# INK-USC/RE-Net

Measured on AMD Instinct MI355X. Metric: RGCN+GRU encoder triples/s at bs=1024 n_hidden=200 (full training step, both directions), higher is better.
Workload: dtype f32; 1 GPU; ICEWS18-shaped synthetic stream (seed 999), n_hidden=200, seq_len=10, batch=1024 per GPU, dropout=0.50, fwd+bwd both directions + clip + Adam; parallelism=dp1, global_batch=1024, nodes=99312, edges=288792

## Files before the change

include/renet_hip.h:

```cpp
#ifndef RENET_HIP_H
#define RENET_HIP_H

#include <stddef.h>
#include <stdint.h>

#ifdef __cplusplus
extern "C" {
#endif

#define RENET_OK 0
#define RENET_ERR_BADARG (-1)
#define RENET_ERR_UNSUPPORTED (-2)
#define RENET_ERR_WORKSPACE (-3)

#define RENET_ABI_VERSION 1
int renet_version(void);

int renet_gather_rows(const float* table, const int32_t* idx, int n, int D, float* out, void* stream);
int renet_segment_add(const float* src, const int32_t* order, const int32_t* seg_ptr,
                      const int32_t* seg_target, int U, int D, float* dst, void* stream);
int renet_segment_add2(const float* src0, const float* src1, const int32_t* order, const int32_t* seg_ptr,
                       const int32_t* seg_target, int U, int D, float* dst0, float* dst1, void* stream);

int renet_rgcn_gather(const float* x, int D, const int32_t* row_ptr, const int32_t* col,
                      const int32_t* etype, const float* scale, const float* W, int T, int type_shift,
                      int transpose_w, const float* addend, float drop_p, uint64_t seed, int relu,
                      float* out, int N, const int32_t* heavy_rows, int n_heavy, int heavy_thresh,
                      int src_limit, int addend_rows, void* stream);

int renet_rgcn_gather_items(const float* x, int D, const int32_t* it_src, const int32_t* it_type,
                            const int32_t* grp_ptr, int n_groups, const int32_t* row_ptr, const int32_t* col,
                            const int32_t* etype, const float* scale, const float* W, int T, int type_shift,
                            int transpose_w, const float* addend, float drop_p, uint64_t seed, int relu,
                            float* out, int N, const int32_t* heavy_rows, int n_heavy, int src_limit,
                            int addend_rows, int pruned, void* stream);

int renet_rgcn_gather_items_table(const float* table, int table_rows, int D, const int32_t* it_src_t,
                                  const int32_t* it_type_t, const int32_t* grp_ptr, int n_groups,
                                  const int32_t* row_ptr, const int32_t* col_t, const int32_t* etype,
                                  const int32_t* row_map, const float* scale, const float* W, int T, int type_shift,
                                  const float* addend_table, float drop_p, uint64_t seed, int relu, float* out, int N,
                                  const int32_t* heavy_rows, int n_heavy, void* stream);

int renet_rgcn_gather_items_bf16(const float* x, int D, const int32_t* it_src, const int32_t* it_type,
                                 const int32_t* grp_ptr, int n_groups, const int32_t* row_ptr, const int32_t* col,
                                 const int32_t* etype, const float* scale, const void* W_bf16, int w_ld, int T,
                                 int type_shift, int transpose_w, const float* addend, float drop_p, uint64_t seed,
                                 int relu, float* out, int N, const int32_t* heavy_rows, int n_heavy, int src_limit,
                                 int addend_rows, int pruned, void* stream);
int renet_rgcn_gather_items_table_bf16(const void* table_bf16, int table_ld, int table_rows, int D,
                                       const int32_t* it_src_t, const int32_t* it_type_t, const int32_t* grp_ptr,
                                       int n_groups, const int32_t* row_ptr, const int32_t* col_t, const int32_t* etype,
                                       const int32_t* row_map, const float* scale, const void* W_bf16, int w_ld, int T,
                                       int type_shift, const float* addend_table, float drop_p, uint64_t seed, int relu,
                                       float* out, int N, const int32_t* heavy_rows, int n_heavy, void* stream);
int renet_compose_table_items(const int32_t* row_map, const int32_t* it_src, const int32_t* it_type, int n_items,
                              const int32_t* col, const int32_t* e_src, int E, int32_t* it_src_t,
                              int32_t* it_type_t, int32_t* col_t, int32_t* e_src_t, void* stream);

int renet_rgcn_bwd_prep(const float* g_out, const float* out, const float* norm, int relu,
                        float drop_p, uint64_t seed, int N, int D, float* gn, float* g_loop,
                        void* stream);
int renet_rgcn_bwd_prep_bounds(const float* g_out, const float* out, const float* norm, int relu,
                               float drop_p, uint64_t seed, int N, int D, float* gn, float* g_loop,
                               float* bound_part, void* stream);

size_t renet_rgcn_bwd_w_workspace(int n_chunks, int D);
int renet_rgcn_bwd_w(const float* x, const float* gn, const int32_t* e_src, const int32_t* e_dst,
                     const int32_t* chunk_ptr, const int32_t* chunk_type, int n_chunks,
                     const int32_t* type_chunk_ptr, int T, int type_shift, int D, float* dW, float beta,
                     float* workspace, size_t workspace_bytes, void* stream);
int renet_rgcn_bwd_w64(const float* x, const float* gn, const int32_t* e_src, const int32_t* e_dst,
                       const int32_t* chunk_ptr, const int32_t* chunk_type, int n_chunks,
                       const int32_t* type_chunk_ptr, int T, int type_shift, int D, float* dW, float beta,
                       float* workspace, size_t workspace_bytes, void* stream);

size_t renet_gemm_workspace(int M, int N, int split_k);
int renet_gemm_f32(int ta, int tb, int M, int N, int K, float alpha, const float* A, int lda,
                   const float* B, int ldb, float beta, float* C, int ldc, const float* bias,
                   int split_k, float* workspace, size_t workspace_bytes, void* stream);

int renet_gemm_f32_split(int ta, int tb, int M, int N, int K, float alpha, const float* A, int lda,
                         const float* B, int ldb, float beta, float* C, int ldc, const float* bias,
                         int split_k, float* workspace, size_t workspace_bytes, void* stream);

int renet_gemm_split_plan(int ta, int tb, int M, int N, int K, const float* A, int lda, const float* B, int ldb,
                          int split_k, int* plan);

int renet_maxabs_blocks(int rows, int cols, int ld);
int renet_maxabs_partials(const float* x, int rows, int cols, int ld, float* part, void* stream);
int renet_maxabs_partials_multi(const void* jobs, int n_jobs, void* stream);
int renet_gemm_f32_h3(int ta, int tb, int M, int N, int K, float alpha, const float* A, int lda, const float* B,
                      int ldb, float beta, float* C, int ldc, const float* bias, int split_k, float* workspace,
                      size_t workspace_bytes, const float* maxA, int nA, const float* maxB, int nB, void* stream);

int renet_gemm_bf16(int ta, int tb, int M, int N, int K, float alpha, const float* A, int lda,
                    const float* B, int ldb, float beta, float* C, int ldc, const float* bias,
                    int split_k, float* workspace, size_t workspace_bytes, void* stream);

size_t renet_bf16_bytes(int R, int C);
int renet_pack_bf16(const float* X, int R, int C, int ldx, void* out, void* stream);
int renet_gemm_bf16s(int a_tr, int b_tr, int M, int N, int K, float alpha, const void* Ap, int lda, const void* Bp,
                     int ldb, float beta, float* C, int ldc, const float* bias, int split_k, float* workspace,
                     size_t workspace_bytes, void* stream);
int renet_bf16_zero_padding(void* P, int rows, int C, int ld, int rows_alloc, void* stream);
int renet_seq_assemble_fwd_bf16(const float* h2, const float* ent, const float* rel, const float* glob,
                                const int32_t* subj_row, const int32_t* row_ent, const int32_t* row_rel,
                                const int32_t* glob_row, int S, int D, float drop_p, uint64_t seed_x,
                                uint64_t seed_xr, void* X, int ldx, void* Xr, int ldxr, int rows_alloc,
                                void* stream);
int renet_softmax_ce_bf16(const float* logits, const int32_t* target, int B, int C, int ld, float grad_scale,
                          float* row_loss, void* dlogits_bf16, int ld16, int rows16, void* stream);
int renet_gru_bwd_layouts_bf16out(int n, const float* const* dh_last, const int32_t* const* step_off, const int* L,
                                  int H, const float* const* Whh, const float* const* saved, void* const* dGi16,
                                  void* const* dGh16, int out_ld, float* workspace, size_t workspace_bytes,
                                  void* stream);
int renet_colsum_bf16(const void* X, int M, int N, int ldx, float* out, float beta, float* workspace,
                      size_t workspace_bytes, void* stream);
int renet_scale_bf16_by_device_scalar(void* x, size_t n, const float* scale, void* stream);

size_t renet_planes_elems(int R, int C);
int renet_pack_planes(const float* X, int R, int C, int ldx, int ones_col, void* out, void* stream);
int renet_gemm_planes(int a_tr, int b_tr, int M, int N, int K, float alpha, const float* alpha_dev, const void* Ap,
                      int lda, size_t a_plane, const void* Bp, int ldb, size_t b_plane, float beta, float* C, int ldc,
                      const float* bias, float* col_out, int split_k, float* workspace, size_t workspace_bytes,
                      void* stream);
int renet_softmax_ce_planes(const float* logits, const int32_t* target, int B, int C, int ld, float grad_scale,
                            float* row_loss, void* dl_planes, size_t plane, int ld16, int rows16, void* stream);

size_t renet_colsum_workspace(int M, int N);
int renet_colsum(const float* X, int M, int N, int ldx, float* out, float beta, float* workspace,
                 size_t workspace_bytes, void* stream);

int renet_scale_by_device_scalar(float* x, size_t n, const float* scale, void* stream);
int renet_scale_by_device_scalar_bound(float* x, size_t n, const float* scale, float bound_in, float* bound_out,
                                       void* stream);

int renet_seq_assemble_fwd(const float* h2, const float* ent, const float* rel, const float* glob,
                           const int32_t* subj_row, const int32_t* row_ent, const int32_t* row_rel,
                           const int32_t* glob_row, int S, int D, float drop_p, uint64_t seed_x,
                           uint64_t seed_xr, float* X, float* Xr, void* stream);
int renet_bound_parts(size_t total4);
int renet_seq_assemble_fwd_bounds(const float* h2, const float* ent, const float* rel, const float* glob,
                                  const int32_t* subj_row, const int32_t* row_ent, const int32_t* row_rel,
                                  const int32_t* glob_row, int S, int D, float drop_p, uint64_t seed_x,
                                  uint64_t seed_xr, float* X, float* Xr, float* partX, float* partXr, void* stream);
int renet_seq_assemble_bwd(const float* dX, const float* dXr, const int32_t* step_off, int L, int S,
                           int B, int D, float drop_p, uint64_t seed_x, uint64_t seed_xr, float* dRows,
                           float* dEntSeq, float* dRelSeq, void* stream);

size_t renet_gru_workspace(int B, int H);
int renet_gru_fwd(const float* Gi, const int32_t* step_off, int L, int H, const float* Whh,
                  const float* bhh, float* h_last, int out_rows, float* saved, float* workspace,
                  size_t workspace_bytes, void* stream);
int renet_gru_bwd(const float* dh_last, const int32_t* step_off, int L, int H, const float* Whh,
                  const float* saved, float* dGi, float* dGh, float* workspace,
                  size_t workspace_bytes, void* stream);
int renet_gru_fwd_multi(int n, const float* const* Gi, const int32_t* step_off, int L, int H,
                        const float* const* Whh, const float* const* bhh, float* const* h_last, int out_rows,
                        float* const* saved, float* workspace, size_t workspace_bytes, void* stream);
int renet_gru_bwd_multi(int n, const float* const* dh_last, const int32_t* step_off, int L, int H,
                        const float* const* Whh, const float* const* saved, float* const* dGi,
                        float* const* dGh, float* workspace, size_t workspace_bytes, void* stream);
int renet_gru_fwd_layouts(int n, const float* const* Gi, const int32_t* const* step_off, const int* L, int H,
                          const float* const* Whh, const float* const* bhh, float* const* h_last,
                          const int* out_rows, float* const* saved, float* workspace, size_t workspace_bytes,
                          void* stream);
int renet_gru_bwd_layouts(int n, const float* const* dh_last, const int32_t* const* step_off, const int* L, int H,
                          const float* const* Whh, const float* const* saved, float* const* dGi,
                          float* const* dGh, float* workspace, size_t workspace_bytes, void* stream);
int renet_gru_bound_parts(int max_rows);
int renet_gru_bwd_layouts_bounds(int n, const float* const* dh_last, const int32_t* const* step_off, const int* L, int H,
                                 const float* const* Whh, const float* const* saved, float* const* dGi,
                                 float* const* dGh, float* const* bounds, float* workspace, size_t workspace_bytes,
                                 void* stream);
int renet_gru_fwd_layouts_f32(int n, const float* const* Gi, const int32_t* const* step_off, const int* L, int H,
                              const float* const* Whh, const float* const* bhh, float* const* h_last,
                              const int* out_rows, float* const* saved, float* workspace, size_t workspace_bytes,
                              void* stream);
int renet_gru_bwd_layouts_f32(int n, const float* const* dh_last, const int32_t* const* step_off, const int* L, int H,
                              const float* const* Whh, const float* const* saved, float* const* dGi,
                              float* const* dGh, float* workspace, size_t workspace_bytes, void* stream);
int renet_gru_fwd_layouts_bf16(int n, const float* const* Gi, const int32_t* const* step_off, const int* L, int H,
                               const float* const* Whh, const float* const* bhh, float* const* h_last,
                               const int* out_rows, float* const* saved, float* workspace, size_t workspace_bytes,
                               void* stream);
int renet_gru_bwd_layouts_bf16(int n, const float* const* dh_last, const int32_t* const* step_off, const int* L, int H,
                               const float* const* Whh, const float* const* saved, float* const* dGi,
                               float* const* dGh, float* workspace, size_t workspace_bytes, void* stream);

int renet_concat3_fwd(const float* a, const int32_t* ia, const float* hmid, const float* c,
                      const int32_t* ic, int B, int D, float drop_p, uint64_t seed, float* feat,
                      void* stream);
int renet_concat3_fwd_bounds(const float* a, const int32_t* ia, const float* hmid, const float* c,
                             const int32_t* ic, int B, int D, float drop_p, uint64_t seed, float* feat,
                             float* bound_part, void* stream);
int renet_concat3_bwd(const float* dfeat, int B, int D, int parts, float drop_p, uint64_t seed,
                      float* da_rows, float* dhmid, float* dc_rows, void* stream);
int renet_dropout(const float* x, size_t n, float drop_p, uint64_t seed, float* y, void* stream);
int renet_softmax_ce(const float* logits, const int32_t* target, int B, int C, int ld,
                     float grad_scale, float* row_loss, float* dlogits, void* stream);

int renet_segment_pool_fwd(const float* h, const int32_t* seg_ptr, int G, int D, int is_max,
                           float* out, int32_t* argmax, void* stream);
int renet_segment_pool_bwd(const float* dout, const int32_t* seg_ptr, const int32_t* argmax, int G,
                           int D, int is_max, int N, float* dh, void* stream);

size_t renet_adam_workspace(size_t n);
int renet_adam_step(float* p, float* g, float* m, float* v, size_t n, float lr, float beta1, float beta2,
                    float eps, float weight_decay, float max_norm, int step, int zero_grad, float* workspace,
                    size_t workspace_bytes, float* grad_norm_out, void* stream);
int renet_adam_step_scaled(float* p, float* g, float* m, float* v, size_t n, float lr, float beta1, float beta2,
                           float eps, float weight_decay, float max_norm, float grad_scale, int step,
                           int zero_grad, float* workspace, size_t workspace_bytes, float* grad_norm_out,
                           void* stream);

int renet_sumsq_partials(const float* g, size_t n, float* partial, int n_slots, void* stream);
int renet_adam_step_presummed(float* p, float* g, float* m, float* v, size_t n, float lr, float beta1, float beta2,
                              float eps, float weight_decay, float max_norm, float grad_scale, int step, int zero_grad,
                              const float* partial, int n_partial, float* grad_norm_out, void* stream);

int renet_joint_softmax(float* logits, int ld, int n, int R, int N, const float* logits_r, int ld_r,
                        const float* prob_e, void* stream);
size_t renet_topk_workspace(int n);
int renet_topk_positive(const float* x, size_t ldx, int n, int M, int k, float* out_val, int64_t* out_idx,
                        void* workspace, size_t workspace_bytes, void* stream);

typedef struct {
    const int32_t *q_s, *q_r, *q_o;
    const int32_t* h_first[2];
    const int32_t* h_count[2];
    const int32_t* snap_t[2];
    const int32_t* snap_ptr[2];
    const int32_t* nbr_o[2];
    const int32_t* times;
    const int32_t* trip_ptr;
    const int32_t *trip_s, *trip_r, *trip_o;
    const int32_t* glob_times;
    int T, n_glob, n_facts, num_ent, num_rels;
} RenetStoreDev;

typedef struct {
    int32_t *node_ent, *node_slot, *row_ptr, *col, *etype;
    float* norm;
    int32_t *heavy_rows, *e_src, *e_dst, *chunk_ptr, *chunk_type, *type_chunk_ptr;
    int32_t *e_src2, *e_dst2, *chunk_ptr2, *chunk_type2, *type_chunk_ptr2;
    int32_t *it_src, *it_type, *grp_ptr;
    int32_t *subj_row, *row_seq, *row_ent, *row_rel, *glob_row;
    int32_t *s_sorted, *r_sorted, *rel_label, *ent_label, *perm, *step_off;
    int32_t* plan_order[4];
    int32_t* plan_seg[4];
    int32_t* plan_target[4];
    int32_t* counts;
    int cap_nodes, cap_edges;
    int32_t* seg_ptr;
} RenetBatchOut;

enum {
    RENET_BB_NNZ = 0, RENET_BB_S, RENET_BB_L, RENET_BB_TB, RENET_BB_FACTS, RENET_BB_N, RENET_BB_NA, RENET_BB_E2,
    RENET_BB_E, RENET_BB_NHEAVY, RENET_BB_NHEAVY_OUT, RENET_BB_NCHUNKS, RENET_BB_NCHUNKS2, RENET_BB_NITEMS,
    RENET_BB_NGROUPS, RENET_BB_NGROUPS_OUT, RENET_BB_NSEG0, RENET_BB_NSEG1, RENET_BB_NSEG2, RENET_BB_NSEG3,
    RENET_BB_ERR, RENET_BB_EOUT,
    RENET_BB_STEP_OFF = 24,
    RENET_BB_NCOUNTS = 64
};
enum { RENET_BB_ERR_TIME = 1, RENET_BB_ERR_GLOB = 2, RENET_BB_ERR_NODES = 4, RENET_BB_ERR_EDGES = 8 };

size_t renet_build_batch_workspace(const RenetStoreDev* store, int B, int cap_nodes, int cap_edges);
int renet_build_batch_both(const RenetStoreDev* store, const int32_t* idx_dev, int B, int seq_len, int heavy_thresh,
                           int group_budget, int chunk, const RenetBatchOut* out, void* workspace,
                           size_t workspace_bytes, void* stream);

typedef struct {
    const int32_t* node_ptr;
    const int32_t* node_ent_all;
    const int32_t* trip_ptr;
    const int32_t *trip_ls, *trip_r, *trip_lo;
    int T, n_nodes, n_facts, num_ent, num_rels;
} RenetFullStoreDev;

size_t renet_build_full_graphs_workspace(const RenetFullStoreDev* store, int G, int cap_nodes, int cap_edges);
int renet_build_full_graphs(const RenetFullStoreDev* store, const int32_t* tidx_dev, int G, int heavy_thresh,
                            int group_items, int chunk, RenetBatchOut* out, void* workspace, size_t workspace_bytes,
                            void* stream);

typedef struct { const int32_t *order, *seg_ptr, *target; int num_segments; } RenetSegPlan;
typedef struct {
    int D, num_ent, T, C2;
    float drop_p;
    const float *ent, *rel;
    const float *w1, *loop1, *w2, *loop2;
    const float *wih, *whh, *bih, *bhh;
    const float *wih_r, *whh_r, *bih_r, *bhh_r;
    const float *lin_w, *lin_b;
    const float *linr_w, *linr_b;
    float *g_ent, *g_rel, *g_w1, *g_loop1, *g_w2, *g_loop2, *g_wih, *g_whh, *g_bih, *g_bhh, *g_wih_r, *g_whh_r, *g_bih_r,
          *g_bhh_r, *g_lin_w, *g_lin_b, *g_linr_w, *g_linr_b;
    const float* glob;
    const void* lin_w_planes;
    size_t lin_w_plane;
    int lin_w_ld;
} RenetStepModel;
// ... 62 lines not shown
```

re-net_amd/csrc/rgcn.hip:

```cpp
#include "common.h"
#include <stdlib.h>

namespace {

constexpr int kWaves = 4;
constexpr int kThreads = 64 * kWaves;

template <int SI, bool TR>
__device__ __forceinline__ void blockmul(const float4 x, const float4* __restrict__ w, float4& acc) {
    if constexpr (SI == 1) {
        const float4 w0 = w[0];
        acc.x = fmaf(x.x, w0.x, acc.x);
        acc.y = fmaf(x.y, w0.y, acc.y);
        acc.z = fmaf(x.z, w0.z, acc.z);
        acc.w = fmaf(x.w, w0.w, acc.w);
    } else if constexpr (SI == 2) {
        const float4 a = w[0], b = w[1];
        if constexpr (!TR) {
            acc.x = fmaf(x.x, a.x, fmaf(x.y, a.z, acc.x));
            acc.y = fmaf(x.x, a.y, fmaf(x.y, a.w, acc.y));
            acc.z = fmaf(x.z, b.x, fmaf(x.w, b.z, acc.z));
            acc.w = fmaf(x.z, b.y, fmaf(x.w, b.w, acc.w));
        } else {
            acc.x = fmaf(x.x, a.x, fmaf(x.y, a.y, acc.x));
// ... 611 lines not shown
#pragma unroll
    for (int q = 0; q < NCH; ++q) off[q] = (uint32_t)(lane + 64 * q) < (uint32_t)CH ? (uint32_t)(lane + 64 * q) * 16u : kOob;
    float4 acc[NCH][SI];
#pragma unroll
    for (int q = 0; q < NCH; ++q)
#pragma unroll
        for (int i = 0; i < SI; ++i) acc[q][i] = make_float4(0.f, 0.f, 0.f, 0.f);

    for (int eb = e0; eb < e1; eb += 64) {
        const int my_e = eb + lane;
        int my_s = 0, my_d = 0;
        if (my_e < e1) { my_s = e_src[my_e]; my_d = e_dst[my_e]; }
        asm volatile("" : "+v"(my_s), "+v"(my_d));
        const int cnt = min(64, e1 - eb);
        for (int k0 = 0; k0 < cnt; k0 += UNR) {
            float4 xv[UNR][NCH], gv[UNR][NCH];
#pragma unroll
            for (int u = 0; u < UNR; ++u) {
                const int kk = min(k0 + u, 63);
                const bool ok = (k0 + u) < cnt;
                const uint32_t so = ok ? (uint32_t)__builtin_amdgcn_readlane(my_s, kk) * ROWB : 0u;
                const uint32_t dof = ok ? (uint32_t)__builtin_amdgcn_readlane(my_d, kk) * ROWB : 0u;
#pragma unroll
                for (int q = 0; q < NCH; ++q) {
                    if constexpr (BIG) {
                        const int ch = lane + 64 * q;
                        const bool on = ok && ch < CH;
                        const size_t sr = (size_t)__builtin_amdgcn_readlane(my_s, kk) * CH + ch;
                        const size_t dr = (size_t)__builtin_amdgcn_readlane(my_d, kk) * CH + ch;
                        const float4 z = make_float4(0.f, 0.f, 0.f, 0.f);
                        xv[u][q] = on ? reinterpret_cast<const float4*>(x)[sr] : z;
                        gv[u][q] = on ? reinterpret_cast<const float4*>(gmat)[dr] : z;
                    } else {
                        xv[u][q] = buf_load4s(rx, ok ? off[q] : kOob, so);
                        gv[u][q] = buf_load4s(rg, ok ? off[q] : kOob, dof);
                    }
                }
            }
#pragma unroll
            for (int u = 0; u < UNR; ++u) {
#pragma unroll
                for (int q = 0; q < NCH; ++q) {
                    if constexpr (SI == 1) {
                        acc[q][0].x = fmaf(xv[u][q].x, gv[u][q].x, acc[q][0].x);
                        acc[q][0].y = fmaf(xv[u][q].y, gv[u][q].y, acc[q][0].y);
                        acc[q][0].z = fmaf(xv[u][q].z, gv[u][q].z, acc[q][0].z);
                        acc[q][0].w = fmaf(xv[u][q].w, gv[u][q].w, acc[q][0].w);
                    } else if constexpr (SI == 2) {
                        acc[q][0].x = fmaf(xv[u][q].x, gv[u][q].x, acc[q][0].x);
                        acc[q][0].y = fmaf(xv[u][q].x, gv[u][q].y, acc[q][0].y);
                        acc[q][0].z = fmaf(xv[u][q].y, gv[u][q].x, acc[q][0].z);
                        acc[q][0].w = fmaf(xv[u][q].y, gv[u][q].y, acc[q][0].w);
                        acc[q][1].x = fmaf(xv[u][q].z, gv[u][q].z, acc[q][1].x);
                        acc[q][1].y = fmaf(xv[u][q].z, gv[u][q].w, acc[q][1].y);
                        acc[q][1].z = fmaf(xv[u][q].w, gv[u][q].z, acc[q][1].z);
                        acc[q][1].w = fmaf(xv[u][q].w, gv[u][q].w, acc[q][1].w);
                    } else {
                        const float xs[4] = {xv[u][q].x, xv[u][q].y, xv[u][q].z, xv[u][q].w};
#pragma unroll
                        for (int i = 0; i < 4; ++i) {
                            acc[q][i].x = fmaf(xs[i], gv[u][q].x, acc[q][i].x);
                            acc[q][i].y = fmaf(xs[i], gv[u][q].y, acc[q][i].y);
                            acc[q][i].z = fmaf(xs[i], gv[u][q].z, acc[q][i].z);
                            acc[q][i].w = fmaf(xs[i], gv[u][q].w, acc[q][i].w);
                        }
                    }
                }
            }
        }
    }
#pragma unroll
    for (int q = 0; q < NCH; ++q) {
        const int ch = lane + 64 * q;
        if (ch < CH) {
#pragma unroll
            for (int i = 0; i < SI; ++i) red[wave][ch * SI + i] = acc[q][i];
        }
    }
    __syncthreads();
    if (!live) return;
    const int ty = chunk_type[c];
    if (wave != 0 && chunk_type[c - 1] == ty) return;
    int run = 1;
    while (wave + run < kBwdWGroup && c + run < n_chunks && chunk_type[c + run] == ty) ++run;
#pragma unroll
    for (int q = 0; q < NCH; ++q) {
        const int ch = lane + 64 * q;
        if (ch < CH) {
#pragma unroll
            for (int i = 0; i < SI; ++i) {
                float4 r = red[wave][ch * SI + i];
                for (int w = 1; w < run; ++w) r = f4_add(r, red[wave + w][ch * SI + i]);
                partial[(size_t)c * WROW4 + ch * SI + i] = r;
            }
        }
    }
}

constexpr int kRedWaves = 16;
__global__ __launch_bounds__(kRedWaves * 64) void rgcn_bwd_w_reduce_kernel(
    const float4* __restrict__ partial, const int32_t* __restrict__ type_chunk_ptr, int WROW4,
    int T, int shift, float beta, float4* __restrict__ dW) {
    __shared__ float4 red[kRedWaves][64];
    const int t = blockIdx.x;
    const int lane = threadIdx.x & 63, wave = threadIdx.x >> 6;
    const int colq = blockIdx.y * 64 + lane;
    const int c0 = type_chunk_ptr[t], c1 = type_chunk_ptr[t + 1];
    float4 s = make_float4(0.f, 0.f, 0.f, 0.f);
    if (colq < WROW4 && c1 > c0) {
        if (wave == 0) s = partial[(size_t)c0 * WROW4 + colq];
        const int g0 = c0 / kBwdWGroup + 1;
        const int g1 = (c1 + kBwdWGroup - 1) / kBwdWGroup;
        float4 s1 = make_float4(0.f, 0.f, 0.f, 0.f), s2 = s1, s3 = s1;
        int gq = g0 + wave;
        for (; gq + 3 * kRedWaves < g1; gq += 4 * kRedWaves) {
            const float4 v0 = partial[(size_t)gq * kBwdWGroup * WROW4 + colq];
            const float4 v1 = partial[(size_t)(gq + kRedWaves) * kBwdWGroup * WROW4 + colq];
            const float4 v2 = partial[(size_t)(gq + 2 * kRedWaves) * kBwdWGroup * WROW4 + colq];
            const float4 v3 = partial[(size_t)(gq + 3 * kRedWaves) * kBwdWGroup * WROW4 + colq];
            s = f4_add(s, v0); s1 = f4_add(s1, v1); s2 = f4_add(s2, v2); s3 = f4_add(s3, v3);
        }
        for (; gq < g1; gq += kRedWaves) s = f4_add(s, partial[(size_t)gq * kBwdWGroup * WROW4 + colq]);
        s = f4_add(f4_add(s, s1), f4_add(s2, s3));
    }
    red[wave][lane] = s;
    __syncthreads();
    if (wave == 0 && colq < WROW4) {
        float4 r = red[0][lane];
#pragma unroll
        for (int w = 1; w < kRedWaves; ++w) r = f4_add(r, red[w][lane]);
        int to = t + shift;
        if (to >= T) to -= T;
        float4* o = dW + (size_t)to * WROW4 + colq;
        if (beta != 0.f) {
            const float4 p = *o;
            r = make_float4(r.x + beta * p.x, r.y + beta * p.y, r.z + beta * p.z, r.w + beta * p.w);
        }
        *o = r;
    }
}

__global__ __launch_bounds__(256) void gather_rows_kernel(const float4* __restrict__ table,
                                                          const int32_t* __restrict__ idx, int n, int CH,
                                                          float4* __restrict__ out) {
    const size_t total = (size_t)n * CH;
    for (size_t i = (size_t)blockIdx.x * blockDim.x + threadIdx.x; i < total;
         i += (size_t)gridDim.x * blockDim.x) {
        const int r = (int)(i / CH), c = (int)(i % CH);
        out[i] = table[(size_t)idx[r] * CH + c];
    }
}

constexpr int kSegWaves = 16, kSegShort = 16, kSegUnr = 8;
__global__ __launch_bounds__(kSegWaves * 64) void segment_add_kernel(const float4* __restrict__ src0,
                                                                     const float4* __restrict__ src1,
                                                                     const int32_t* __restrict__ order,
                                                                     const int32_t* __restrict__ seg_ptr,
                                                                     const int32_t* __restrict__ seg_target,
                                                                     int U, int CH, float4* __restrict__ dst0,
                                                                     float4* __restrict__ dst1) {
    const float4* __restrict__ src = blockIdx.y ? src1 : src0;
    float4* __restrict__ dst = blockIdx.y ? dst1 : dst0;
    __shared__ float4 red[kSegWaves][128];
    const int lane = threadIdx.x & 63;
    const int wave = __builtin_amdgcn_readfirstlane(threadIdx.x >> 6);
    const int nwg = gridDim.x;
    {
        const int u = blockIdx.x + wave * nwg;
        const int k0 = u < U ? seg_ptr[u] : 0, k1 = u < U ? seg_ptr[u + 1] : 0;
        const int len = k1 - k0;
        if (len > 0 && len <= kSegShort) {
            const size_t tgt = (size_t)seg_target[u] * CH;
            for (int ch = lane; ch < CH; ch += 64) {
                float4 s = make_float4(0.f, 0.f, 0.f, 0.f);
                for (int k = k0; k < k1; k += kSegUnr) {
                    float4 v[kSegUnr];
#pragma unroll
                    for (int j = 0; j < kSegUnr; ++j) v[j] = src[(size_t)order[min(k + j, k1 - 1)] * CH + ch];
#pragma unroll
                    for (int j = 0; j < kSegUnr; ++j)
                        if (k + j < k1) s = f4_add(s, v[j]);
                }
                dst[tgt + ch] = f4_add(dst[tgt + ch], s);
            }
        }
    }
    for (int j = 0; j < kSegWaves; ++j) {
        const int u = blockIdx.x + j * nwg;
        if (u >= U) break;
        const int k0 = seg_ptr[u], k1 = seg_ptr[u + 1];
        if (k1 - k0 <= kSegShort) continue;
        const size_t tgt = (size_t)seg_target[u] * CH;
        for (int ch = lane; ch < CH; ch += 64) {
            float4 s = make_float4(0.f, 0.f, 0.f, 0.f);
            for (int k = k0 + wave * kSegUnr; k < k1; k += kSegWaves * kSegUnr) {
                float4 v[kSegUnr];
#pragma unroll
                for (int q = 0; q < kSegUnr; ++q) v[q] = src[(size_t)order[min(k + q, k1 - 1)] * CH + ch];
#pragma unroll
                for (int q = 0; q < kSegUnr; ++q)
                    if (k + q < k1) s = f4_add(s, v[q]);
            }
            red[wave][ch] = s;
        }
        __syncthreads();
        if (wave == 0) {
            for (int ch = lane; ch < CH; ch += 64) {
                float4 r = red[0][ch];
#pragma unroll
                for (int w = 1; w < kSegWaves; ++w) r = f4_add(r, red[w][ch]);
                dst[tgt + ch] = f4_add(dst[tgt + ch], r);
            }
        }
        __syncthreads();
    }
}

__global__ __launch_bounds__(256) void compose_table_items_kernel(const int32_t* __restrict__ row_map,
                                                                  const int32_t* __restrict__ it_src,
                                                                  const int32_t* __restrict__ it_type, int n_items,
                                                                  const int32_t* __restrict__ col,
                                                                  const int32_t* __restrict__ e_src, int E,
                                                                  int32_t* __restrict__ it_src_t,
                                                                  int32_t* __restrict__ it_type_t,
                                                                  int32_t* __restrict__ col_t,
                                                                  int32_t* __restrict__ e_src_t) {
    const int total = n_items + 2 * E;
    for (int i = blockIdx.x * blockDim.x + threadIdx.x; i < total; i += gridDim.x * blockDim.x) {
        if (i < n_items) {
            const int s = it_src[i], t = it_type[i];
            if (t >= 0) { it_src_t[i] = row_map[s]; it_type_t[i] = t; }
            else if (t == -1) { it_src_t[i] = s; it_type_t[i] = -3 - row_map[s]; }
            else { it_src_t[i] = s; it_type_t[i] = t; }
        } else if (i < n_items + E) {
            col_t[i - n_items] = row_map[col[i - n_items]];
        } else {
            e_src_t[i - n_items - E] = row_map[e_src[i - n_items - E]];
        }
    }
}

}

extern "C" {

int renet_version(void) { return RENET_ABI_VERSION; }

int renet_gather_rows(const float* table, const int32_t* idx, int n, int D, float* out, void* stream) {
    if (n < 0 || D <= 0 || (D & 3)) return RENET_ERR_BADARG;
    if (n == 0) return RENET_OK;
    const int CH = D / 4;
    const size_t total = (size_t)n * CH;
    int blocks = (int)min((size_t)2048, (total + 255) / 256);
    RENET_LAUNCH(gather_rows_kernel, dim3(blocks), dim3(256), 0, (hipStream_t)stream,
                       (const float4*)table, idx, n, CH, (float4*)out);
    RENET_LAUNCH_CHECK();
    return RENET_OK;
}

static int seg_grid(int U) { return U <= 512 ? U : max(512, (U + kSegWaves - 1) / kSegWaves); }

int renet_segment_add(const float* src, const int32_t* order, const int32_t* seg_ptr,
                      const int32_t* seg_target, int U, int D, float* dst, void* stream) {
    if (U < 0 || D <= 0 || (D & 3)) return RENET_ERR_BADARG;
    if (U == 0) return RENET_OK;
    if (D > 512) return RENET_ERR_UNSUPPORTED;
    RENET_LAUNCH(segment_add_kernel, dim3(seg_grid(U)), dim3(kSegWaves * 64), 0,
                       (hipStream_t)stream, (const float4*)src, (const float4*)src, order, seg_ptr, seg_target, U, D / 4,
                       (float4*)dst, (float4*)dst);
    RENET_LAUNCH_CHECK();
    return RENET_OK;
}

int renet_segment_add2(const float* src0, const float* src1, const int32_t* order, const int32_t* seg_ptr,
                       const int32_t* seg_target, int U, int D, float* dst0, float* dst1, void* stream) {
    if (U < 0 || D <= 0 || (D & 3)) return RENET_ERR_BADARG;
    if (U == 0) return RENET_OK;
    if (D > 512) return RENET_ERR_UNSUPPORTED;
    RENET_LAUNCH(segment_add_kernel, dim3(seg_grid(U), 2), dim3(kSegWaves * 64), 0,
                       (hipStream_t)stream, (const float4*)src0, (const float4*)src1, order, seg_ptr, seg_target, U, D / 4,
                       (float4*)dst0, (float4*)dst1);
    RENET_LAUNCH_CHECK();
    return RENET_OK;
}

int renet_rgcn_gather(const float* x, int D, const int32_t* row_ptr, const int32_t* col,
                      const int32_t* etype, const float* scale, const float* W, int T, int type_shift,
                      int transpose_w, const float* addend, float drop_p, uint64_t seed, int relu,
                      float* out, int N, const int32_t* heavy_rows, int n_heavy, int heavy_thresh,
                      int src_limit, int addend_rows, void* stream) {
    if (!renet_dim_ok(D)) return RENET_ERR_UNSUPPORTED;
    if (n_heavy < 0 || (n_heavy > 0 && (!heavy_rows || heavy_thresh < 1))) return RENET_ERR_BADARG;
    if (N < 0 || T <= 0 || type_shift < 0 || type_shift >= T || drop_p < 0.f || drop_p >= 1.f)
        return RENET_ERR_BADARG;
    if (N == 0) return RENET_OK;
    GatherArgs a;
    a.x = x; a.row_ptr = row_ptr; a.col = col; a.etype = etype; a.scale = scale; a.W = W;
    a.addend = addend; a.out = out; a.N = N; a.T = T; a.shift = type_shift; a.relu = relu;
    a.heavy = heavy_rows; a.n_heavy = n_heavy;
    a.src_limit = src_limit > 0 ? src_limit : 0x7fffffff;
    a.addend_rows = addend_rows > 0 ? addend_rows : 0x7fffffff;
    a.heavy_thresh = n_heavy > 0 ? heavy_thresh : 0x7fffffff;
    a.drop = make_drop(drop_p, seed);
    hipStream_t st = (hipStream_t)stream;
    switch (D) {
        case 100: return launch_gather<1, 1, 4>(a, transpose_w != 0, st);
        case 200: return launch_gather<2, 1, 4>(a, transpose_w != 0, st);
        default: return launch_gather<4, 2, 2>(a, transpose_w != 0, st);
    }
}

static int gather_items_impl(int mx, int x_ld, int w_ld, const float* x, int x_rows, int D, const int32_t* it_src, const int32_t* it_type,
                             const int32_t* grp_ptr, int n_groups, const int32_t* row_ptr, const int32_t* col,
                             const int32_t* etype, const float* scale, const float* W, int T, int type_shift,
                             int transpose_w, const float* addend, float drop_p, uint64_t seed, int relu,
                             float* out, int N, const int32_t* heavy_rows, int n_heavy, int src_limit,
                             int addend_rows, int pruned, const int32_t* row_map, void* stream) {
    if (!renet_dim_ok(D)) return RENET_ERR_UNSUPPORTED;
    if (n_heavy < 0 || (n_heavy > 0 && !heavy_rows) || n_groups < 0) return RENET_ERR_BADARG;
    if (N < 0 || T <= 0 || type_shift < 0 || type_shift >= T || drop_p < 0.f || drop_p >= 1.f)
        return RENET_ERR_BADARG;
    if (N == 0 || (n_groups == 0 && n_heavy == 0)) return RENET_OK;
    if ((size_t)max(N, x_rows) * D * sizeof(float) >= ((size_t)1 << 31) ||
        (size_t)T * D * (D / 100) * sizeof(float) >= ((size_t)1 << 31))
        return RENET_ERR_UNSUPPORTED;
    ItemArgs a;
    a.g.x = x; a.g.row_ptr = row_ptr; a.g.col = col; a.g.etype = etype; a.g.scale = scale; a.g.W = W;
    a.g.addend = addend; a.g.out = out; a.g.N = N; a.g.T = T; a.g.shift = type_shift; a.g.relu = relu;
    a.g.heavy = heavy_rows; a.g.n_heavy = n_heavy; a.g.heavy_thresh = 0;
    a.g.src_limit = src_limit > 0 ? src_limit : 0x7fffffff;
    a.g.addend_rows = addend_rows > 0 ? addend_rows : 0x7fffffff;
    a.g.row_map = row_map;
    a.g.drop = make_drop(drop_p, seed);
    a.it_src = it_src; a.it_type = it_type; a.grp_ptr = grp_ptr; a.n_groups = n_groups;
    hipStream_t st = (hipStream_t)stream;
    const bool tr = transpose_w != 0, pr = pruned != 0;
    a.g.x_rowb = mx == 2 ? (uint32_t)x_ld * 2u : (uint32_t)D * 4u;
    a.g.w_rowb = mx >= 1 ? (uint32_t)w_ld * 2u : (uint32_t)D * (D / 100) * 4u;
    if (mx < 0 || mx > 2 || (mx >= 1 && w_ld < D * (D / 100)) || (mx == 2 && x_ld < D)) return RENET_ERR_BADARG;
    if (mx == 1) {
        switch (D) {
            case 100: return launch_gather_items<1, 1, 6, 1>(a, tr, pr, st);
            case 200: return launch_gather_items<2, 1, 3, 1>(a, tr, pr, st);
            default: return launch_gather_items<4, 2, 2, 1>(a, tr, pr, st);
        }
    }
    if (mx == 2) {
        switch (D) {
            case 100: return launch_gather_items<1, 1, 6, 2>(a, tr, pr, st);
            case 200: return launch_gather_items<2, 1, 3, 2>(a, tr, pr, st);
            default: return launch_gather_items<4, 2, 2, 2>(a, tr, pr, st);
        }
    }
    const int unr = gather_unr();
    switch (D) {
        case 100:
            if (unr == 8) return launch_gather_items<1, 1, 8>(a, tr, pr, st);
            if (unr == 4) return launch_gather_items<1, 1, 4>(a, tr, pr, st);
            return launch_gather_items<1, 1, 6>(a, tr, pr, st);
        case 200:
            if (unr == 2) return launch_gather_items<2, 1, 2>(a, tr, pr, st);
            if (unr == 4) return launch_gather_items<2, 1, 4>(a, tr, pr, st);
            if (unr == 6) return launch_gather_items<2, 1, 6>(a, tr, pr, st);
            if (unr == 8) return launch_gather_items<2, 1, 8>(a, tr, pr, st);
            return launch_gather_items<2, 1, 3>(a, tr, pr, st);
        default:
            if (unr == 3) return launch_gather_items<4, 2, 3>(a, tr, pr, st);
            if (unr == 4) return launch_gather_items<4, 2, 4>(a, tr, pr, st);
            return launch_gather_items<4, 2, 2>(a, tr, pr, st);
    }
}

int renet_rgcn_gather_items(const float* x, int D, const int32_t* it_src, const int32_t* it_type,
                            const int32_t* grp_ptr, int n_groups, const int32_t* row_ptr, const int32_t* col,
                            const int32_t* etype, const float* scale, const float* W, int T, int type_shift,
                            int transpose_w, const float* addend, float drop_p, uint64_t seed, int relu,
                            float* out, int N, const int32_t* heavy_rows, int n_heavy, int src_limit,
                            int addend_rows, int pruned, void* stream) {
    return gather_items_impl(0, 0, 0, x, N, D, it_src, it_type, grp_ptr, n_groups, row_ptr, col, etype, scale, W, T,
                             type_shift, transpose_w, addend, drop_p, seed, relu, out, N, heavy_rows, n_heavy, src_limit,
                             addend_rows, pruned, nullptr, stream);
}

int renet_rgcn_gather_items_bf16(const float* x, int D, const int32_t* it_src, const int32_t* it_type,
                                 const int32_t* grp_ptr, int n_groups, const int32_t* row_ptr, const int32_t* col,
                                 const int32_t* etype, const float* scale, const void* W_bf16, int w_ld, int T,
                                 int type_shift, int transpose_w, const float* addend, float drop_p, uint64_t seed,
                                 int relu, float* out, int N, const int32_t* heavy_rows, int n_heavy, int src_limit,
                                 int addend_rows, int pruned, void* stream) {
    return gather_items_impl(1, 0, w_ld, x, N, D, it_src, it_type, grp_ptr, n_groups, row_ptr, col, etype, scale,
                             (const float*)W_bf16, T, type_shift, transpose_w, addend, drop_p, seed, relu, out, N,
                             heavy_rows, n_heavy, src_limit, addend_rows, pruned, nullptr, stream);
}

int renet_rgcn_gather_items_table(const float* table, int table_rows, int D, const int32_t* it_src_t,
                                  const int32_t* it_type_t, const int32_t* grp_ptr, int n_groups,
                                  const int32_t* row_ptr, const int32_t* col_t, const int32_t* etype,
                                  const int32_t* row_map, const float* scale, const float* W, int T, int type_shift,
                                  const float* addend_table, float drop_p, uint64_t seed, int relu, float* out, int N,
                                  const int32_t* heavy_rows, int n_heavy, void* stream) {
    if (!row_map || table_rows <= 0) return RENET_ERR_BADARG;
    return gather_items_impl(0, 0, 0, table, table_rows, D, it_src_t, it_type_t, grp_ptr, n_groups, row_ptr, col_t, etype,
                             scale, W, T, type_shift, 0, addend_table, drop_p, seed, relu, out, N, heavy_rows, n_heavy, 0, 0,
                             0, row_map, stream);
}

int renet_rgcn_gather_items_table_bf16(const void* table_bf16, int table_ld, int table_rows, int D,
                                       const int32_t* it_src_t, const int32_t* it_type_t, const int32_t* grp_ptr,
                                       int n_groups, const int32_t* row_ptr, const int32_t* col_t, const int32_t* etype,
                                       const int32_t* row_map, const float* scale, const void* W_bf16, int w_ld, int T,
                                       int type_shift, const float* addend_table, float drop_p, uint64_t seed, int relu,
                                       float* out, int N, const int32_t* heavy_rows, int n_heavy, void* stream) {
    if (!row_map || table_rows <= 0) return RENET_ERR_BADARG;
    return gather_items_impl(2, table_ld, w_ld, (const float*)table_bf16, table_rows, D, it_src_t, it_type_t, grp_ptr,
                             n_groups, row_ptr, col_t, etype, scale, (const float*)W_bf16, T, type_shift, 0, addend_table,
                             drop_p, seed, relu, out, N, heavy_rows, n_heavy, 0, 0, 0, row_map, stream);
}

int renet_compose_table_items(const int32_t* row_map, const int32_t* it_src, const int32_t* it_type, int n_items,
                              const int32_t* col, const int32_t* e_src, int E, int32_t* it_src_t,
                              int32_t* it_type_t, int32_t* col_t, int32_t* e_src_t, void* stream) {
    if (n_items < 0 || E < 0 || !row_map) return RENET_ERR_BADARG;
    const int total = n_items + 2 * E;
    if (total == 0) return RENET_OK;
    RENET_LAUNCH(compose_table_items_kernel, dim3(min(2048, (total + 255) / 256)), dim3(256), 0, (hipStream_t)stream,
                 row_map, it_src, it_type, n_items, col, e_src, E, it_src_t, it_type_t, col_t, e_src_t);
    RENET_LAUNCH_CHECK();
    return RENET_OK;
}

static int bwd_prep_impl(const float* g_out, const float* out, const float* norm, int relu, float drop_p,
                         uint64_t seed, int N, int D, float* gn, float* g_loop, float* bound_part, void* stream) {
    if (N < 0 || D <= 0 || (D & 3) || drop_p < 0.f || drop_p >= 1.f) return RENET_ERR_BADARG;
    if (N == 0) return bound_part ? RENET_ERR_BADARG : RENET_OK;
// ... 88 lines not shown
```

re-net_amd/csrc/seq.hip:

```cpp
#include "common.h"

namespace {

__device__ __forceinline__ float sq_max4(float m, const float4& v) {
    return fmaxf(fmaxf(m, fmaxf(fabsf(v.x), fabsf(v.y))), fmaxf(fabsf(v.z), fabsf(v.w)));
}
__device__ __forceinline__ void sq_block_max_write(float m, float* __restrict__ part, float* red ) {
#pragma unroll
    for (int off = 32; off >= 1; off >>= 1) m = fmaxf(m, __shfl_xor(m, off));
    if ((threadIdx.x & 63) == 0) red[threadIdx.x >> 6] = m;
    __syncthreads();
    if (threadIdx.x == 0) part[blockIdx.x] = fmaxf(fmaxf(red[0], red[1]), fmaxf(red[2], red[3]));
    __syncthreads();
}

__global__ __launch_bounds__(256) void seq_assemble_fwd_kernel(
    const float4* __restrict__ h2, const float4* __restrict__ ent, const float4* __restrict__ rel,
    const float4* __restrict__ glob, const int32_t* __restrict__ subj_row,
    const int32_t* __restrict__ row_ent, const int32_t* __restrict__ row_rel,
    const int32_t* __restrict__ glob_row, int S, int CH, DropCfg dx, DropCfg dxr,
    float4* __restrict__ X, float4* __restrict__ Xr, float* __restrict__ partX, float* __restrict__ partXr) {
    __shared__ float red[4];
    float mx = 0.f, mxr = 0.f;
    const size_t total = (size_t)S * 4 * CH;
    for (size_t i = (size_t)blockIdx.x * blockDim.x + threadIdx.x; i < total;
         i += (size_t)gridDim.x * blockDim.x) {
        const int p = (int)(i / (4 * CH));
        const int c = (int)(i - (size_t)p * 4 * CH);
        const int part = c / CH, cc = c - part * CH;
        float4 v;
        if (part == 0) v = h2[(size_t)subj_row[p] * CH + cc];
        else if (part == 1) v = ent[(size_t)row_ent[p] * CH + cc];
        else if (part == 2) v = rel[(size_t)row_rel[p] * CH + cc];
        else v = glob[(size_t)glob_row[p] * CH + cc];
        const float4 o = f4_mul(v, renet_drop4(dx, i));
        X[i] = o;
        mx = sq_max4(mx, o);
        if (part != 2) {
            const int cr = (part == 3 ? 2 : part) * CH + cc;
            const size_t ir = (size_t)p * 3 * CH + cr;
            const float4 orr = f4_mul(v, renet_drop4(dxr, ir));
            Xr[ir] = orr;
            mxr = sq_max4(mxr, orr);
        }
    }
    if (partX) {
        sq_block_max_write(mx, partX, red);
        sq_block_max_write(mxr, partXr, red);
    }
}

typedef float sq_f32x2 __attribute__((ext_vector_type(2)));
typedef __bf16 sq_bf16x2 __attribute__((ext_vector_type(2)));
__device__ __forceinline__ uint2 sq_pack4(float4 v) {
    const sq_bf16x2 lo = __builtin_convertvector(sq_f32x2{v.x, v.y}, sq_bf16x2);
    const sq_bf16x2 hi = __builtin_convertvector(sq_f32x2{v.z, v.w}, sq_bf16x2);
    uint2 u;
    u.x = __builtin_bit_cast(unsigned, lo);
    u.y = __builtin_bit_cast(unsigned, hi);
    return u;
}
__global__ __launch_bounds__(256) void seq_assemble_fwd_bf16_kernel(
    const float4* __restrict__ h2, const float4* __restrict__ ent, const float4* __restrict__ rel,
    const float4* __restrict__ glob, const int32_t* __restrict__ subj_row,
    const int32_t* __restrict__ row_ent, const int32_t* __restrict__ row_rel,
    const int32_t* __restrict__ glob_row, int S, int CH, DropCfg dx, DropCfg dxr,
    __bf16* __restrict__ X, int ldx, __bf16* __restrict__ Xr, int ldxr) {
    const size_t total = (size_t)S * 4 * CH;
    for (size_t i = (size_t)blockIdx.x * blockDim.x + threadIdx.x; i < total;
         i += (size_t)gridDim.x * blockDim.x) {
        const int p = (int)(i / (4 * CH));
        const int c = (int)(i - (size_t)p * 4 * CH);
        const int part = c / CH, cc = c - part * CH;
        float4 v;
        if (part == 0) v = h2[(size_t)subj_row[p] * CH + cc];
        else if (part == 1) v = ent[(size_t)row_ent[p] * CH + cc];
        else if (part == 2) v = rel[(size_t)row_rel[p] * CH + cc];
        else v = glob[(size_t)glob_row[p] * CH + cc];
        *reinterpret_cast<uint2*>(X + (size_t)p * ldx + c * 4) = sq_pack4(f4_mul(v, renet_drop4(dx, i)));
        if (part != 2) {
            const int cr = (part == 3 ? 2 : part) * CH + cc;
            const size_t ir = (size_t)p * 3 * CH + cr;
            *reinterpret_cast<uint2*>(Xr + (size_t)p * ldxr + cr * 4) = sq_pack4(f4_mul(v, renet_drop4(dxr, ir)));
        }
    }
}

__global__ __launch_bounds__(256) void seq_assemble_bwd_rows_kernel(const float4* __restrict__ dX,
                                                                    const float4* __restrict__ dXr, int S,
                                                                    int CH, DropCfg dx, DropCfg dxr,
                                                                    float4* __restrict__ dRows) {
    const size_t total = (size_t)S * CH;
    for (size_t i = (size_t)blockIdx.x * blockDim.x + threadIdx.x; i < total;
         i += (size_t)gridDim.x * blockDim.x) {
        const int p = (int)(i / CH), cc = (int)(i - (size_t)p * CH);
        const size_t bx = (size_t)p * 4 * CH, br = (size_t)p * 3 * CH;
        const float4 a = f4_mul(dX[bx + cc], renet_drop4(dx, bx + cc));
        const float4 b = f4_mul(dXr[br + cc], renet_drop4(dxr, br + cc));
        dRows[i] = f4_add(a, b);
    }
}

__global__ __launch_bounds__(256) void seq_assemble_bwd_seq_kernel(const float4* __restrict__ dX,
                                                                   const float4* __restrict__ dXr,
                                                                   const int32_t* __restrict__ off, int L,
                                                                   int B, int CH, DropCfg dx, DropCfg dxr,
                                                                   float4* __restrict__ dEntSeq,
                                                                   float4* __restrict__ dRelSeq) {
    const size_t total = (size_t)B * CH;
    for (size_t t = (size_t)blockIdx.x * blockDim.x + threadIdx.x; t < total;
         t += (size_t)gridDim.x * blockDim.x) {
        const int i = (int)(t / CH), cc = (int)(t - (size_t)i * CH);
        float4 se = make_float4(0.f, 0.f, 0.f, 0.f), sr = se;
        for (int j = 0; j < L; ++j) {
            const int o0 = off[j], o1 = off[j + 1];
            if (i >= o1 - o0) break;
            const size_t p = (size_t)(o0 + i);
            const size_t bx = p * 4 * CH, br = p * 3 * CH;
            se = f4_add(se, f4_mul(dX[bx + CH + cc], renet_drop4(dx, bx + CH + cc)));
            se = f4_add(se, f4_mul(dXr[br + CH + cc], renet_drop4(dxr, br + CH + cc)));
            sr = f4_add(sr, f4_mul(dX[bx + 2 * CH + cc], renet_drop4(dx, bx + 2 * CH + cc)));
        }
        dEntSeq[t] = se;
        dRelSeq[t] = sr;
    }
}

__global__ __launch_bounds__(256) void concat3_fwd_kernel(const float4* __restrict__ a,
                                                          const int32_t* __restrict__ ia,
                                                          const float4* __restrict__ hmid,
                                                          const float4* __restrict__ c,
                                                          const int32_t* __restrict__ ic, int B, int CH,
                                                          int parts, DropCfg d, float4* __restrict__ feat,
                                                          float* __restrict__ bound_part) {
    __shared__ float red[4];
    float mx = 0.f;
    const size_t total = (size_t)B * parts * CH;
    for (size_t i = (size_t)blockIdx.x * blockDim.x + threadIdx.x; i < total;
         i += (size_t)gridDim.x * blockDim.x) {
        const int b = (int)(i / (parts * CH));
        const int q = (int)(i - (size_t)b * parts * CH);
        const int part = q / CH, cc = q - part * CH;
        float4 v;
        if (part == 0) v = a[(size_t)ia[b] * CH + cc];
        else if (part == 1) v = hmid[(size_t)b * CH + cc];
        else v = c[(size_t)ic[b] * CH + cc];
        const float4 o = f4_mul(v, renet_drop4(d, i));
        feat[i] = o;
        mx = sq_max4(mx, o);
    }
    if (bound_part) sq_block_max_write(mx, bound_part, red);
}

__global__ __launch_bounds__(256) void concat3_bwd_kernel(const float4* __restrict__ dfeat, int B, int CH,
                                                          int parts, DropCfg d, float4* __restrict__ da,
                                                          float4* __restrict__ dh, float4* __restrict__ dc) {
    const size_t total = (size_t)B * parts * CH;
    for (size_t i = (size_t)blockIdx.x * blockDim.x + threadIdx.x; i < total;
         i += (size_t)gridDim.x * blockDim.x) {
        const int b = (int)(i / (parts * CH));
        const int q = (int)(i - (size_t)b * parts * CH);
        const int part = q / CH, cc = q - part * CH;
        const float4 v = f4_mul(dfeat[i], renet_drop4(d, i));
        const size_t o = (size_t)b * CH + cc;
        if (part == 0) da[o] = v;
        else if (part == 1) dh[o] = v;
        else dc[o] = v;
    }
}

__device__ __forceinline__ float wave_max(float v) {
#pragma unroll
    for (int o = 32; o > 0; o >>= 1) v = fmaxf(v, __shfl_xor(v, o));
    return v;
}
__device__ __forceinline__ float wave_sum(float v) {
#pragma unroll
    for (int o = 32; o > 0; o >>= 1) v += __shfl_xor(v, o);
    return v;
}

__global__ __launch_bounds__(256) void softmax_ce_kernel(const float* logits,
                                                         const int32_t* __restrict__ target, int C, int ld,
                                                         float grad_scale, float* __restrict__ row_loss,
                                                         float* dlogits, __bf16* __restrict__ dl16, int ld16) {
    __shared__ float red[4];
    const int b = blockIdx.x;
    const int lane = threadIdx.x & 63, wave = threadIdx.x >> 6;
    const float* x = logits + (size_t)b * ld;
    float m = -INFINITY;
    for (int c = threadIdx.x; c < C; c += 256) m = fmaxf(m, x[c]);
    m = wave_max(m);
    if (lane == 0) red[wave] = m;
    __syncthreads();
    m = fmaxf(fmaxf(red[0], red[1]), fmaxf(red[2], red[3]));
    __syncthreads();
    float s = 0.f;
    for (int c = threadIdx.x; c < C; c += 256) s += expf(x[c] - m);
    s = wave_sum(s);
    if (lane == 0) red[wave] = s;
    __syncthreads();
    s = (red[0] + red[1]) + (red[2] + red[3]);
    const int t = target[b];
    float xt = x[t];
    asm volatile("" : "+v"(xt) :: "memory");
    __syncthreads();
    if (threadIdx.x == 0) row_loss[b] = logf(s) + m - xt;
    if (dlogits) {
        float* dx = dlogits + (size_t)b * ld;
        const float inv = 1.f / s;
        for (int c = threadIdx.x; c < C; c += 256) {
            const float p = expf(x[c] - m) * inv;
            dx[c] = (p - (c == t ? 1.f : 0.f)) * grad_scale;
        }
    }
    if (dl16) {
        __bf16* dx = dl16 + (size_t)b * ld16;
        const float inv = 1.f / s;
        const int C16 = min((C + 63) & ~63, ld16);
        for (int c = threadIdx.x; c < C16; c += 256)
            dx[c] = c < C ? (__bf16)((expf(x[c] - m) * inv - (c == t ? 1.f : 0.f)) * grad_scale) : (__bf16)0.f;
    }
}

template <int NQ>
__global__ __launch_bounds__(512, 4) void softmax_ce_reg_kernel(const float* logits, const int32_t* __restrict__ target,
                                                                int C, int ld, float grad_scale,
                                                                float* __restrict__ row_loss, float* dlogits) {
    __shared__ float red_m[8], red_s[8];
    const int b = blockIdx.x;
    const int lane = threadIdx.x & 63, wave = threadIdx.x >> 6;
    const int t = target[b];
    const __amdgpu_buffer_rsrc_t rin = __builtin_amdgcn_make_buffer_rsrc(
        const_cast<float*>(logits + (size_t)b * ld), (short)0, C * 4, 0x00020000);
    const int voff = (int)threadIdx.x * 4;
    float v[NQ];
#pragma unroll
    for (int q = 0; q < NQ; ++q)
        v[q] = __uint_as_float(__builtin_amdgcn_raw_buffer_load_b32(rin, voff, 2048 * q, 0));
    float m = -INFINITY, xt = 0.f;
    const int tq = t >> 9;
    const bool mine = (int)threadIdx.x == (t & 511);
#pragma unroll
    for (int q = 0; q < NQ; ++q) {
        v[q] = (int)threadIdx.x < C - 512 * q ? v[q] : -INFINITY;
        m = fmaxf(m, v[q]);
        xt = (mine && q == tq) ? v[q] : xt;
    }
    m = wave_max(m);
    if (lane == 0) red_m[wave] = m;
    __syncthreads();
    m = red_m[0];
#pragma unroll
    for (int w = 1; w < 8; ++w) m = fmaxf(m, red_m[w]);
    float s = 0.f;
#pragma unroll
    for (int q = 0; q < NQ; ++q) {
        v[q] = expf(v[q] - m);
        s += v[q];
        if ((q & 7) == 7) __builtin_amdgcn_sched_barrier(0);
    }
    s = wave_sum(s);
    if (lane == 0) red_s[wave] = s;
    __syncthreads();
    s = 0.f;
#pragma unroll
    for (int w = 0; w < 8; ++w) s += red_s[w];
    if (mine) row_loss[b] = logf(s) + m - xt;
    if (dlogits) {
        const __amdgpu_buffer_rsrc_t rout = __builtin_amdgcn_make_buffer_rsrc(dlogits + (size_t)b * ld, (short)0, C * 4,
                                                                             0x00020000);
        const float inv = 1.f / s;
#pragma unroll
        for (int q = 0; q < NQ; ++q) {
            const float o = (v[q] * inv - ((mine && q == tq) ? 1.f : 0.f)) * grad_scale;
            __builtin_amdgcn_raw_buffer_store_b32(__float_as_uint(o), rout, voff, 2048 * q, 0);
        }
    }
}

// ... 327 lines not shown

__global__ __launch_bounds__(256) void zero_kernel(float4* __restrict__ x, size_t n4, float* __restrict__ xt, int tail) {
    const float4 z = make_float4(0.f, 0.f, 0.f, 0.f);
    for (size_t i = (size_t)blockIdx.x * 256 + threadIdx.x; i < n4; i += (size_t)gridDim.x * 256) x[i] = z;
    if (blockIdx.x == 0 && (int)threadIdx.x < tail) xt[threadIdx.x] = 0.f;
}

__global__ __launch_bounds__(256) void add_inplace_kernel(float4* __restrict__ x, const float4* __restrict__ y, size_t n4,
                                                          float* __restrict__ xt, const float* __restrict__ yt, int tail) {
    for (size_t i = (size_t)blockIdx.x * 256 + threadIdx.x; i < n4; i += (size_t)gridDim.x * 256) x[i] = f4_add(x[i], y[i]);
    if (blockIdx.x == 0 && (int)threadIdx.x < tail) xt[threadIdx.x] += yt[threadIdx.x];
}

__global__ __launch_bounds__(256) void segment_pool_fwd_kernel(const float* __restrict__ h,
                                                               const int32_t* __restrict__ seg_ptr, int D,
                                                               int is_max, float* __restrict__ out,
                                                               int32_t* __restrict__ argmax) {
    __shared__ float rv[4][64];
    __shared__ int ri[4][64];
    const int g = blockIdx.x;
    const int lane = threadIdx.x & 63, wave = threadIdx.x >> 6;
    const int c = blockIdx.y * 64 + lane;
    const int r0 = seg_ptr[g], r1 = seg_ptr[g + 1];
    float best = is_max ? -INFINITY : 0.f;
    int bi = r0;
    if (c < D) {
        for (int r = r0 + wave; r < r1; r += 4) {
            const float v = h[(size_t)r * D + c];
            if (is_max) { if (v > best) { best = v; bi = r; } }
            else best += v;
        }
    }
    rv[wave][lane] = best; ri[wave][lane] = bi;
    __syncthreads();
    if (wave == 0 && c < D) {
        if (is_max) {
            for (int w = 1; w < 4; ++w) {
                const float v = rv[w][lane];
                const int i = ri[w][lane];
                if (v > best || (v == best && i < bi)) { best = v; bi = i; }
            }
            out[(size_t)g * D + c] = best;
            argmax[(size_t)g * D + c] = bi;
        } else {
            const float s = (rv[0][lane] + rv[1][lane]) + (rv[2][lane] + rv[3][lane]);
            out[(size_t)g * D + c] = s / (float)max(r1 - r0, 1);
        }
    }
}

__global__ __launch_bounds__(256) void segment_pool_bwd_kernel(const float* __restrict__ dout,
                                                               const int32_t* __restrict__ seg_ptr,
                                                               const int32_t* __restrict__ argmax, int D,
                                                               int is_max, float* __restrict__ dh) {
    const int g = blockIdx.x;
    const int r0 = seg_ptr[g], r1 = seg_ptr[g + 1];
    const int n = (r1 - r0) * D;
    for (int i = threadIdx.x; i < n; i += 256) {
        const int r = r0 + i / D, c = i % D;
        const float go = dout[(size_t)g * D + c];
        float v;
        if (is_max) v = (argmax[(size_t)g * D + c] == r) ? go : 0.f;
        else v = go / (float)(r1 - r0);
        dh[(size_t)r * D + c] = v;
    }
}

__global__ __launch_bounds__(256) void dropout_kernel(const float4* __restrict__ x, size_t n4, DropCfg d,
                                                      float4* __restrict__ y) {
    for (size_t i = (size_t)blockIdx.x * blockDim.x + threadIdx.x; i < n4; i += (size_t)gridDim.x * blockDim.x)
        y[i] = f4_mul(x[i], renet_drop4(d, i));
}

inline int grid_for(size_t total) { return (int)max((size_t)1, min((size_t)2048, (total + 255) / 256)); }

}

extern "C" {

int renet_seq_assemble_fwd(const float* h2, const float* ent, const float* rel, const float* glob,
                           const int32_t* subj_row, const int32_t* row_ent, const int32_t* row_rel,
                           const int32_t* glob_row, int S, int D, float drop_p, uint64_t seed_x,
                           uint64_t seed_xr, float* X, float* Xr, void* stream) {
    if (S < 0 || D <= 0 || (D & 3) || drop_p < 0.f || drop_p >= 1.f) return RENET_ERR_BADARG;
    if (S == 0) return RENET_OK;
    const int CH = D / 4;
    RENET_LAUNCH(seq_assemble_fwd_kernel, dim3(grid_for((size_t)S * 4 * CH)), dim3(256), 0,
                       (hipStream_t)stream, (const float4*)h2, (const float4*)ent, (const float4*)rel,
                       (const float4*)glob, subj_row, row_ent, row_rel, glob_row, S, CH,
                       make_drop(drop_p, seed_x), make_drop(drop_p, seed_xr), (float4*)X, (float4*)Xr,
                       (float*)nullptr, (float*)nullptr);
    RENET_LAUNCH_CHECK();
    return RENET_OK;
}

int renet_bound_parts(size_t total4) { return (int)max((size_t)1, min((size_t)1024, (total4 + 255) / 256)); }

int renet_seq_assemble_fwd_bounds(const float* h2, const float* ent, const float* rel, const float* glob,
                                  const int32_t* subj_row, const int32_t* row_ent, const int32_t* row_rel,
                                  const int32_t* glob_row, int S, int D, float drop_p, uint64_t seed_x,
                                  uint64_t seed_xr, float* X, float* Xr, float* partX, float* partXr, void* stream) {
    if (S <= 0 || D <= 0 || (D & 3) || drop_p < 0.f || drop_p >= 1.f || !partX || !partXr) return RENET_ERR_BADARG;
    const int CH = D / 4;
    RENET_LAUNCH(seq_assemble_fwd_kernel, dim3(renet_bound_parts((size_t)S * 4 * CH)), dim3(256), 0,
                       (hipStream_t)stream, (const float4*)h2, (const float4*)ent, (const float4*)rel,
                       (const float4*)glob, subj_row, row_ent, row_rel, glob_row, S, CH,
                       make_drop(drop_p, seed_x), make_drop(drop_p, seed_xr), (float4*)X, (float4*)Xr, partX, partXr);
    RENET_LAUNCH_CHECK();
    return RENET_OK;
}

static int zero_bf16_padding(__bf16* P, int rows, int C, int ld, int rows_alloc, hipStream_t st) {
    const int c16 = min((C + 63) & ~63, ld), r16 = min((rows + 63) & ~63, rows_alloc);
    if (c16 > C && rows > 0) {
        hipError_t e = hipMemset2DAsync(P + C, (size_t)ld * sizeof(__bf16), 0, (size_t)(c16 - C) * sizeof(__bf16),
                                        (size_t)rows, st);
        if (e != hipSuccess) return (int)e;
    }
    if (r16 > rows) {
        hipError_t e = hipMemsetAsync(P + (size_t)rows * ld, 0, (size_t)(r16 - rows) * ld * sizeof(__bf16), st);
        if (e != hipSuccess) return (int)e;
    }
    return RENET_OK;
}

int renet_seq_assemble_fwd_bf16(const float* h2, const float* ent, const float* rel, const float* glob,
                                const int32_t* subj_row, const int32_t* row_ent, const int32_t* row_rel,
                                const int32_t* glob_row, int S, int D, float drop_p, uint64_t seed_x,
                                uint64_t seed_xr, void* X, int ldx, void* Xr, int ldxr, int rows_alloc,
                                void* stream) {
    if (S < 0 || D <= 0 || (D & 3) || drop_p < 0.f || drop_p >= 1.f || ldx < 4 * D || ldxr < 3 * D || (ldx & 3) ||
        (ldxr & 3) || rows_alloc < S) return RENET_ERR_BADARG;
    hipStream_t st = (hipStream_t)stream;
    int e = zero_bf16_padding((__bf16*)X, S, 4 * D, ldx, rows_alloc, st);
    if (e != RENET_OK) return e;
    e = zero_bf16_padding((__bf16*)Xr, S, 3 * D, ldxr, rows_alloc, st);
    if (e != RENET_OK) return e;
    if (S == 0) return RENET_OK;
    const int CH = D / 4;
    RENET_LAUNCH(seq_assemble_fwd_bf16_kernel, dim3(grid_for((size_t)S * 4 * CH)), dim3(256), 0, st,
                       (const float4*)h2, (const float4*)ent, (const float4*)rel, (const float4*)glob, subj_row,
                       row_ent, row_rel, glob_row, S, CH, make_drop(drop_p, seed_x), make_drop(drop_p, seed_xr),
                       (__bf16*)X, ldx, (__bf16*)Xr, ldxr);
    RENET_LAUNCH_CHECK();
    return RENET_OK;
}

int renet_seq_assemble_bwd(const float* dX, const float* dXr, const int32_t* step_off, int L, int S,
                           int B, int D, float drop_p, uint64_t seed_x, uint64_t seed_xr, float* dRows,
                           float* dEntSeq, float* dRelSeq, void* stream) {
    if (S < 0 || B < 0 || L < 0 || D <= 0 || (D & 3) || drop_p < 0.f || drop_p >= 1.f) return RENET_ERR_BADARG;
    const int CH = D / 4;
    const DropCfg dx = make_drop(drop_p, seed_x), dxr = make_drop(drop_p, seed_xr);
    if (S > 0) {
        RENET_LAUNCH(seq_assemble_bwd_rows_kernel, dim3(grid_for((size_t)S * CH)), dim3(256), 0,
                           (hipStream_t)stream, (const float4*)dX, (const float4*)dXr, S, CH, dx, dxr,
                           (float4*)dRows);
        RENET_LAUNCH_CHECK();
    }
    if (B > 0) {
        RENET_LAUNCH(seq_assemble_bwd_seq_kernel, dim3(grid_for((size_t)B * CH)), dim3(256), 0,
                           (hipStream_t)stream, (const float4*)dX, (const float4*)dXr, step_off, L, B, CH, dx,
                           dxr, (float4*)dEntSeq, (float4*)dRelSeq);
        RENET_LAUNCH_CHECK();
    }
    return RENET_OK;
}

static int concat3_fwd_impl(const float* a, const int32_t* ia, const float* hmid, const float* c,
                            const int32_t* ic, int B, int D, float drop_p, uint64_t seed, float* feat,
                            float* bound_part, void* stream) {
    if (B < 0 || D <= 0 || (D & 3) || drop_p < 0.f || drop_p >= 1.f) return RENET_ERR_BADARG;
    if (B == 0) return bound_part ? RENET_ERR_BADARG : RENET_OK;
    const int CH = D / 4, parts = c ? 3 : 2;
    RENET_LAUNCH(concat3_fwd_kernel, dim3(bound_part ? renet_bound_parts((size_t)B * parts * CH)
                                                     : grid_for((size_t)B * parts * CH)), dim3(256), 0,
                       (hipStream_t)stream, (const float4*)a, ia, (const float4*)hmid, (const float4*)c, ic,
                       B, CH, parts, make_drop(drop_p, seed), (float4*)feat, bound_part);
    RENET_LAUNCH_CHECK();
    return RENET_OK;
}

int renet_concat3_fwd(const float* a, const int32_t* ia, const float* hmid, const float* c,
                      const int32_t* ic, int B, int D, float drop_p, uint64_t seed, float* feat,
                      void* stream) {
    return concat3_fwd_impl(a, ia, hmid, c, ic, B, D, drop_p, seed, feat, nullptr, stream);
}

int renet_concat3_fwd_bounds(const float* a, const int32_t* ia, const float* hmid, const float* c,
                             const int32_t* ic, int B, int D, float drop_p, uint64_t seed, float* feat,
                             float* bound_part, void* stream) {
    if (!bound_part) return RENET_ERR_BADARG;
    return concat3_fwd_impl(a, ia, hmid, c, ic, B, D, drop_p, seed, feat, bound_part, stream);
}

int renet_concat3_bwd(const float* dfeat, int B, int D, int parts, float drop_p, uint64_t seed,
                      float* da_rows, float* dhmid, float* dc_rows, void* stream) {
    if (B < 0 || D <= 0 || (D & 3) || (parts != 2 && parts != 3) || drop_p < 0.f || drop_p >= 1.f)
        return RENET_ERR_BADARG;
    if (B == 0) return RENET_OK;
    const int CH = D / 4;
    RENET_LAUNCH(concat3_bwd_kernel, dim3(grid_for((size_t)B * parts * CH)), dim3(256), 0,
                       (hipStream_t)stream, (const float4*)dfeat, B, CH, parts, make_drop(drop_p, seed),
                       (float4*)da_rows, (float4*)dhmid, (float4*)dc_rows);
    RENET_LAUNCH_CHECK();
    return RENET_OK;
}

int renet_dropout(const float* x, size_t n, float drop_p, uint64_t seed, float* y, void* stream) {
    if ((n & 3) || drop_p < 0.f || drop_p >= 1.f) return RENET_ERR_BADARG;
    if (n == 0) return RENET_OK;
    RENET_LAUNCH(dropout_kernel, dim3(grid_for(n / 4)), dim3(256), 0, (hipStream_t)stream,
                       (const float4*)x, n / 4, make_drop(drop_p, seed), (float4*)y);
    RENET_LAUNCH_CHECK();
    return RENET_OK;
}

static int softmax_ce_impl(const float* logits, const int32_t* target, int B, int C, int ld, float grad_scale,
                           float* row_loss, float* dlogits, __bf16* dl16, int ld16, void* stream);

int renet_softmax_ce(const float* logits, const int32_t* target, int B, int C, int ld,
                     float grad_scale, float* row_loss, float* dlogits, void* stream) {
    return softmax_ce_impl(logits, target, B, C, ld, grad_scale, row_loss, dlogits, nullptr, 0, stream);
}

int renet_softmax_ce_bf16(const float* logits, const int32_t* target, int B, int C, int ld, float grad_scale,
                          float* row_loss, void* dlogits_bf16, int ld16, int rows16, void* stream) {
    if (!dlogits_bf16 || ld16 < C || (ld16 & 1) || rows16 < B) return RENET_ERR_BADARG;
    if (rows16 > B) {
        hipError_t e = hipMemsetAsync((__bf16*)dlogits_bf16 + (size_t)B * ld16, 0,
                                      (size_t)(rows16 - B) * ld16 * sizeof(__bf16), (hipStream_t)stream);
        if (e != hipSuccess) return (int)e;
    }
    return softmax_ce_impl(logits, target, B, C, ld, grad_scale, row_loss, nullptr, (__bf16*)dlogits_bf16, ld16, stream);
}

static int softmax_ce_impl(const float* logits, const int32_t* target, int B, int C, int ld, float grad_scale,
                           float* row_loss, float* dlogits, __bf16* dl16, int ld16, void* stream) {
    if (B < 0 || C <= 0 || ld < C) return RENET_ERR_BADARG;
    if (B == 0) return RENET_OK;
    const size_t lds = (size_t)C * sizeof(float);
    if (!dl16 && C >= 4096 && C <= 48 * 512) {
        const dim3 grid(B), blk(512);
        hipStream_t st = (hipStream_t)stream;
        if (C <= 16 * 512) RENET_LAUNCH((softmax_ce_reg_kernel<16>), grid, blk, 0, st, logits, target, C, ld, grad_scale, row_loss, dlogits);
        else if (C <= 32 * 512) RENET_LAUNCH((softmax_ce_reg_kernel<32>), grid, blk, 0, st, logits, target, C, ld, grad_scale, row_loss, dlogits);
        else RENET_LAUNCH((softmax_ce_reg_kernel<48>), grid, blk, 0, st, logits, target, C, ld, grad_scale, row_loss, dlogits);
    } else if (lds <= 128 * 1024 && C >= 4096) {
        static bool attr_set = false;
        if (!attr_set) {
            hipError_t e = hipFuncSetAttribute((const void*)softmax_ce_lds_kernel,
                                               hipFuncAttributeMaxDynamicSharedMemorySize, 128 * 1024);
            if (e != hipSuccess) return (int)e;
            attr_set = true;
        }
        RENET_LAUNCH(softmax_ce_lds_kernel, dim3(B), dim3(1024), lds, (hipStream_t)stream, logits, target, C, ld,
                     grad_scale, row_loss, dlogits, dl16, ld16);
    } else {
        RENET_LAUNCH(softmax_ce_kernel, dim3(B), dim3(256), 0, (hipStream_t)stream, logits, target, C, ld,
                     grad_scale, row_loss, dlogits, dl16, ld16);
    }
    RENET_LAUNCH_CHECK();
    return RENET_OK;
}

int renet_softmax_ce_planes(const float* logits, const int32_t* target, int B, int C, int ld, float grad_scale,
                            float* row_loss, void* dl_planes, size_t plane, int ld16, int rows16, void* stream) {
    if (B < 0 || C <= 0 || ld < C || !dl_planes || ld16 < C || (ld16 & 15) || rows16 < ((B + 15) & ~15)) return RENET_ERR_BADARG;
    if (plane < (size_t)rows16 * ld16) return RENET_ERR_BADARG;
    if (B == 0) return RENET_OK;
    hipStream_t st = (hipStream_t)stream;
    __bf16* P = (__bf16*)dl_planes;
    if ((B & 15) != 0) {
        for (int p = 0; p < 3; ++p) {
            hipError_t e = hipMemsetAsync(P + (size_t)p * plane + (size_t)(B >> 4) * ld16 * 16, 0,
                                          (size_t)ld16 * 16 * sizeof(__bf16), st);
            if (e != hipSuccess) return (int)e;
        }
    }
    const bool aligned = (ld & 3) == 0 && (reinterpret_cast<uintptr_t>(logits) & 15) == 0 &&
                         (reinterpret_cast<uintptr_t>(dl_planes) & 7) == 0 && (plane & 3) == 0;
    static const bool rows4 = !renet_env_flag("RENET_SOFTMAX_ROWS", false);
    if (aligned && rows4 && C >= 2048 && ld16 <= 12 * 2048 && (reinterpret_cast<uintptr_t>(dl_planes) & 15) == 0 &&
        (plane & 7) == 0) {
        const int quads = (B + 3) / 4;
        const dim3 grid((unsigned)((quads + 31) & ~31)), blk(512);
        if (ld16 <= 4 * 2048) RENET_LAUNCH((softmax_ce_planes4_kernel<4>), grid, blk, 0, st, logits, target, B, C, ld, grad_scale, row_loss, P, plane, ld16);
        else if (ld16 <= 8 * 2048) RENET_LAUNCH((softmax_ce_planes4_kernel<8>), grid, blk, 0, st, logits, target, B, C, ld, grad_scale, row_loss, P, plane, ld16);
        else RENET_LAUNCH((softmax_ce_planes4_kernel<12>), grid, blk, 0, st, logits, target, B, C, ld, grad_scale, row_loss, P, plane, ld16);
    } else if (aligned && C >= 2048 && ld16 <= 12 * 2048) {
        const dim3 grid((unsigned)((B + 127) & ~127)), blk(512);
        if (ld16 <= 4 * 2048) RENET_LAUNCH((softmax_ce_planes_kernel<4>), grid, blk, 0, st, logits, target, B, C, ld, grad_scale, row_loss, P, plane, ld16);
        else if (ld16 <= 8 * 2048) RENET_LAUNCH((softmax_ce_planes_kernel<8>), grid, blk, 0, st, logits, target, B, C, ld, grad_scale, row_loss, P, plane, ld16);
        else RENET_LAUNCH((softmax_ce_planes_kernel<12>), grid, blk, 0, st, logits, target, B, C, ld, grad_scale, row_loss, P, plane, ld16);
    } else {
        RENET_LAUNCH(softmax_ce_planes_generic_kernel, dim3(B), dim3(256), 0, st, logits, target, C, ld, grad_scale,
                     row_loss, P, plane, ld16);
    }
    RENET_LAUNCH_CHECK();
    return RENET_OK;
}

int renet_zero(float* x, size_t n, void* stream) {
    if (n == 0) return RENET_OK;
    if (!x || (reinterpret_cast<uintptr_t>(x) & 15)) return RENET_ERR_BADARG;
    const size_t n4 = n / 4;
    const int blocks = (int)max((size_t)1, min((size_t)2048, (n4 + 255) / 256));
    RENET_LAUNCH(zero_kernel, dim3(blocks), dim3(256), 0, (hipStream_t)stream, (float4*)x, n4, x + n4 * 4, (int)(n & 3));
    RENET_LAUNCH_CHECK();
    return RENET_OK;
}

int renet_add_inplace(float* x, const float* y, size_t n, void* stream) {
    if (n == 0) return RENET_OK;
    if (!x || !y || ((reinterpret_cast<uintptr_t>(x) | reinterpret_cast<uintptr_t>(y)) & 15)) return RENET_ERR_BADARG;
    const size_t n4 = n / 4;
// ... 30 lines not shown
```

re-net_amd/csrc/step.cpp:

```cpp
#include <hip/hip_runtime.h>
#include <algorithm>
#include <cstdint>
#include <cstdlib>
#include <vector>
#include "../../include/renet_hip.h"

namespace {

int auto_split_k(int m, int n, int k) {
    const long tiles = (long)((m + 127) / 128) * ((n + 127) / 128);
    const int ktiles = (k + 31) / 32;
    if (tiles >= 256 || ktiles < 8) return 1;
    const int smax = std::max(1, std::min(128, ktiles / 4));
    const double per_slice = (double)m * (double)n * 2.7e-6;
    int best = 1;
    double best_t = -1.0;
    for (int s = 1; s <= smax; ++s) {
        const long rounds = (tiles * s + 511) / 512;
        const double t = (double)rounds * ((double)ktiles / (double)s + 6.0) + (s > 1 ? per_slice * s : 0.0);
        if (best_t < 0.0 || t < best_t - 1e-9) { best = s; best_t = t; }
    }
    return best;
}

int auto_split_k_planes(int m, int n, int k) {
    const long tiles = (long)((m + 255) / 256) * ((n + 127) / 128);
    const int ktiles = (k + 31) / 32;
    if (tiles >= 128 || ktiles < 8) return 1;
    const int smax = std::max(1, std::min(64, ktiles / 4));
    const double per_slice = (double)m * (double)n * 2.7e-6;
    int best = 1;
    double best_t = -1.0;
    for (int s = 1; s <= smax; ++s) {
        const long rounds = (tiles * s + 255) / 256;
        const double t = (double)rounds * ((double)ktiles / (double)s + 6.0) + (s > 1 ? per_slice * s : 0.0);
        if (best_t < 0.0 || t < best_t - 1e-9) { best = s; best_t = t; }
    }
    return best;
}

inline size_t up(size_t x) { return (x + 255) & ~(size_t)255; }
inline size_t fbytes(size_t rows, size_t cols) { return up(rows * cols * sizeof(float)); }

struct Lay {
    size_t out1, out2, X, Xr, sv0, sv1, feat1, feat2, dl1, dl2, featp1;
    size_t ew, gi0, gi1, hs0, hs1, logits, featp;
    size_t dfeat1, dfeat2, da1, da2, dh1, dh2, dc1, dgi0, dgi1, dgh0, dgh1, dX, dXr, d_rows, d_ent_seq, d_rel_seq, d_h2, gn2,
        gl2, dhN, gn1, gl1, dh1N, gs;
    size_t gru_ws, gemm_ws_main, gemm_ws_side, bwdw_ws, colsum_ws;
    size_t gru_ws_bytes, gemm_ws_bytes, bwdw_ws_bytes, colsum_ws_bytes;
    size_t dl_plane, dl_ld, dl_rows, featp_plane, featp_ld, featp1_plane, featp1_ld, logits_ld;
    size_t total;
};

bool use_planes(const RenetStepModel& m) { return m.lin_w_planes != nullptr; }

Lay layout(const RenetStepModel& m, const RenetStepBatch& b) {
    Lay L{};
    size_t o = 0;
    auto take = [&](size_t bytes) { const size_t at = o; o += up(bytes); return at; };
    const size_t D = m.D, N = b.N, nA = b.nA, S = b.S, B = b.B, NE = m.num_ent, C2 = m.C2;
    const bool pl = use_planes(m);
    L.out1 = take(fbytes(N, D));
    L.out2 = take(fbytes(nA, D));
    L.X = take(fbytes(S, 4 * D));
    L.Xr = take(fbytes(S, 3 * D));
    L.sv0 = take(fbytes(S, 5 * D));
    L.sv1 = take(fbytes(S, 5 * D));
    L.feat1 = take(fbytes(B, 3 * D));
    L.feat2 = take(fbytes(B, 2 * D));
    L.dl2 = take(fbytes(B, C2));
    if (pl) {
        L.dl_rows = (B + 255) & ~(size_t)255;
        L.dl_ld = (NE + 255) & ~(size_t)255;
        L.dl_plane = L.dl_rows * L.dl_ld;
        L.dl1 = take(3 * L.dl_plane * 2);
        L.featp_ld = (3 * D + 255) & ~(size_t)255;
        L.featp_plane = L.dl_rows * L.featp_ld;
        L.featp1_ld = (3 * D + 1 + 255) & ~(size_t)255;
        L.featp1_plane = L.dl_rows * L.featp1_ld;
        L.featp1 = take(3 * L.featp1_plane * 2);
        L.logits_ld = (NE + 3) & ~(size_t)3;
        L.logits = take(fbytes(B, L.logits_ld));
    } else {
        L.dl1 = take(fbytes(B, NE));
        L.logits_ld = NE;
    }
    L.ew = take(fbytes(NE, D));
    L.gi0 = take(fbytes(S, 3 * D));
    L.gi1 = take(fbytes(S, 3 * D));
    L.hs0 = take(fbytes(B, D));
    L.hs1 = take(fbytes(B, D));
    L.dfeat1 = take(fbytes(B, 3 * D));
    L.dfeat2 = take(fbytes(B, 2 * D));
    L.da1 = take(fbytes(B, D));
    L.da2 = take(fbytes(B, D));
    L.dh1 = take(fbytes(B, D));
    L.dh2 = take(fbytes(B, D));
    L.dc1 = take(fbytes(B, D));
    L.dgi0 = take(fbytes(S, 3 * D));
    L.dgi1 = take(fbytes(S, 3 * D));
    L.dgh0 = take(fbytes(S, 3 * D));
    L.dgh1 = take(fbytes(S, 3 * D));
    L.dX = take(fbytes(S, 4 * D));
    L.dXr = take(fbytes(S, 3 * D));
    L.d_rows = take(fbytes(S, D));
    L.d_ent_seq = take(fbytes(B, D));
    L.d_rel_seq = take(fbytes(B, D));
    L.d_h2 = take(fbytes(nA, D));
    L.gn2 = take(fbytes(nA, D));
    L.gl2 = take(fbytes(nA, D));
    L.dhN = take(fbytes(N, D));
    L.gn1 = take(fbytes(N, D));
    L.gl1 = take(fbytes(N, D));
    L.dh1N = take(fbytes(N, D));
    L.gs = take(fbytes(NE, D));
    const int bmax = b.L > 0 ? b.step_off_host[1] - b.step_off_host[0] : 0;
    L.gru_ws_bytes = 2 * renet_gru_workspace(bmax, m.D);
    L.gru_ws = take(std::max<size_t>(L.gru_ws_bytes, 4));
    size_t need = 4;
    auto g_ = [&](int mm, int nn, int kk) { need = std::max(need, renet_gemm_workspace(mm, nn, auto_split_k(mm, nn, kk))); };
    const int Di = m.D, Si = b.S, Bi = b.B, NEi = m.num_ent, nAi = b.nA, C2i = m.C2;
    g_(NEi, Di, Di); g_(nAi, Di, Di); g_(Si, 3 * Di, 4 * Di); g_(Si, 3 * Di, 3 * Di); g_(Bi, NEi, 3 * Di); g_(Bi, C2i, 2 * Di);
    g_(Bi, 3 * Di, NEi); g_(NEi, 3 * Di, Bi); g_(Bi, 2 * Di, C2i); g_(C2i, 2 * Di, Bi);
    g_(3 * Di, 4 * Di, Si); g_(3 * Di, 3 * Di, Si); g_(3 * Di, Di, Si); g_(Si, 3 * Di, 3 * Di); g_(Si, 2 * Di, 3 * Di);
    g_(Di, Di, nAi); g_(Di, Di, NEi);
    if (pl) {
        need = std::max(need, renet_gemm_workspace(Bi, 3 * Di, auto_split_k_planes(Bi, 3 * Di, NEi)));
        need = std::max(need, renet_gemm_workspace(NEi, 3 * Di + 1, auto_split_k_planes(NEi, 3 * Di + 1, Bi)));
        need = std::max(need, renet_gemm_workspace(Bi, NEi, auto_split_k_planes(Bi, NEi, 3 * Di)));
    }
    L.gemm_ws_bytes = need;
    L.gemm_ws_main = take(need);
    L.gemm_ws_side = take(need);
    L.bwdw_ws_bytes = std::max<size_t>(renet_rgcn_bwd_w_workspace(std::max(b.n_chunks, b.n_chunks2), m.D), 4);
    L.bwdw_ws = take(L.bwdw_ws_bytes);
    size_t cs = 4;
    cs = std::max(cs, renet_colsum_workspace(Bi, NEi));
    cs = std::max(cs, renet_colsum_workspace(Bi, C2i));
    cs = std::max(cs, renet_colsum_workspace(Si, 3 * Di));
    L.colsum_ws_bytes = cs;
    L.colsum_ws = take(cs);
    L.total = o;
    return L;
}

bool args_ok(const RenetStepModel* m, const RenetStepBatch* b) {
    if (!m || !b) return false;
    if (!(m->D == 100 || m->D == 200 || m->D == 400) || m->num_ent < 1 || m->T < 2 || m->C2 < 1) return false;
    if (b->N < 1 || b->nA < 1 || b->nA > b->N || b->S < 1 || b->B < 1 || b->L < 1 || !b->step_off_host) return false;
    const size_t big = (size_t)std::max(b->N, m->num_ent) * m->D * 4;
    return big < ((size_t)1 << 31);
}

hipEvent_t step_event(int i) {
    thread_local std::vector<hipEvent_t> ev;
    while ((int)ev.size() <= i) {
        hipEvent_t e = nullptr;
        if (hipEventCreateWithFlags(&e, hipEventDisableTiming) != hipSuccess) return nullptr;
        ev.push_back(e);
    }
    return ev[i];
}

struct Streams {
    hipStream_t main, side;
    int next_ev = 0, rc = 0;
    bool two() const { return side != main; }
    void order(hipStream_t first, hipStream_t then) {
        if (!two() || rc) return;
        hipEvent_t e = step_event(next_ev++ & 7);
        if (!e) { rc = (int)hipErrorOutOfMemory; return; }
        hipError_t x = hipEventRecord(e, first);
        if (x == hipSuccess) x = hipStreamWaitEvent(then, e, 0);
        if (x != hipSuccess) rc = (int)x;
    }
    void fork() { order(main, side); }
    void join() { order(side, main); }
};

#define CK(call)                      \
    do {                              \
        const int rc__ = (call);      \
        ++launches;                   \
        if (rc__ != 0) return rc__;   \
    } while (0)

int gemm(hipStream_t st, float* ws, size_t ws_bytes, int ta, int tb, int M, int N, int K, const float* A, int lda, const float* B,
         int ldb, float beta, float* C, int ldc, const float* bias) {
    const int sk = auto_split_k(M, N, K);
    return renet_gemm_f32_split(ta, tb, M, N, K, 1.f, A, lda, B, ldb, beta, C, ldc, bias, sk, sk > 1 ? ws : nullptr,
                                sk > 1 ? ws_bytes : 0, st);
}

}

extern "C" {

size_t renet_step_workspace(const RenetStepModel* m, const RenetStepBatch* b) {
    if (!args_ok(m, b)) return 0;
    return layout(*m, *b).total;
}

int renet_step_forward(const RenetStepModel* mp, const RenetStepBatch* bp, const RenetStepRun* r, float* row_loss,
                       int* n_launches) {
    if (!args_ok(mp, bp) || !r || !r->workspace || !row_loss) return RENET_ERR_BADARG;
    const RenetStepModel& m = *mp;
    const RenetStepBatch& b = *bp;
    const Lay L = layout(m, b);
    if (r->workspace_bytes < L.total) return RENET_ERR_WORKSPACE;
    char* W = (char*)r->workspace;
    auto F = [&](size_t off) { return (float*)(W + off); };
    Streams s{(hipStream_t)r->stream, (hipStream_t)(r->side_stream ? r->side_stream : r->stream)};
    int launches = 0;
    const int D = m.D, N = b.N, nA = b.nA, S = b.S, B = b.B, NE = m.num_ent, T = m.T;
    const float p = m.drop_p;
    const bool pruned = nA < N;
    float* wsm = F(L.gemm_ws_main);
    float* wss = F(L.gemm_ws_side);

    CK(gemm(s.main, wsm, L.gemm_ws_bytes, 0, 0, NE, D, D, m.ent, D, m.loop1, D, 0.f, F(L.ew), D, nullptr));
    CK(renet_rgcn_gather_items_table(m.ent, NE, D, b.it_src_t, b.it_type_t, b.grp_ptr, b.n_groups, b.row_ptr, b.col_t, b.etype,
                                     b.node_ent, b.norm, m.w1, T, 0, F(L.ew), p, r->seed_rgcn1, 1, F(L.out1), N,
                                     b.n_heavy ? b.heavy_rows : nullptr, b.n_heavy, s.main));
    CK(gemm(s.main, wsm, L.gemm_ws_bytes, 0, 0, nA, D, D, F(L.out1), D, m.loop2, D, 0.f, F(L.out2), D, nullptr));
    CK(renet_rgcn_gather_items(F(L.out1), D, b.it_src, b.it_type, b.grp_ptr, pruned ? b.n_groups_out : b.n_groups, b.row_ptr,
                               b.col, b.etype, b.norm, m.w2, T, 0, 0, F(L.out2), p, r->seed_rgcn2, 0, F(L.out2), nA,
                               pruned ? (b.n_heavy_out ? b.heavy_rows_out : nullptr) : (b.n_heavy ? b.heavy_rows : nullptr),
                               pruned ? b.n_heavy_out : b.n_heavy, 0, 0, pruned ? 1 : 0, s.main));
    CK(renet_seq_assemble_fwd(F(L.out2), m.ent, m.rel, m.glob, b.subj_row, b.row_ent, b.row_rel, b.glob_row, S, D, p, r->seed_x,
                              r->seed_xr, F(L.X), F(L.Xr), s.main));
    s.fork();
    CK(gemm(s.side, wss, L.gemm_ws_bytes, 0, 1, S, 3 * D, 3 * D, F(L.Xr), 3 * D, m.wih_r, 3 * D, 0.f, F(L.gi1), 3 * D, m.bih_r));
    CK(gemm(s.main, wsm, L.gemm_ws_bytes, 0, 1, S, 3 * D, 4 * D, F(L.X), 4 * D, m.wih, 4 * D, 0.f, F(L.gi0), 3 * D, m.bih));
    s.join();
    {
        const float* gi[2] = {F(L.gi0), F(L.gi1)};
        const int32_t* so[2] = {b.step_off_host, b.step_off_host};
        const int ls[2] = {b.L, b.L};
        const float* whh[2] = {m.whh, m.whh_r};
        const float* bhh[2] = {m.bhh, m.bhh_r};
        float* hl[2] = {F(L.hs0), F(L.hs1)};
        const int bmax = b.step_off_host[1] - b.step_off_host[0];
        const int rows[2] = {std::max(B, bmax), std::max(B, bmax)};
        float* sv[2] = {F(L.sv0), F(L.sv1)};
        if (rows[0] != B) return RENET_ERR_BADARG;
        CK(renet_gru_fwd_layouts(2, gi, so, ls, D, whh, bhh, hl, rows, sv, F(L.gru_ws), L.gru_ws_bytes, s.main));
    }
    s.fork();
    CK(renet_concat3_fwd(m.ent, b.s_idx, F(L.hs1), nullptr, nullptr, B, D, p, r->seed_head2, F(L.feat2), s.side));
    CK(gemm(s.side, wss, L.gemm_ws_bytes, 0, 1, B, m.C2, 2 * D, F(L.feat2), 2 * D, m.linr_w, 2 * D, 0.f, F(L.dl2), m.C2, m.linr_b));
    CK(renet_softmax_ce(F(L.dl2), b.rel_label, B, m.C2, m.C2, r->scale_rel, row_loss + B, F(L.dl2), s.side));
    CK(renet_concat3_fwd(m.ent, b.s_idx, F(L.hs0), m.rel, b.r_idx, B, D, p, r->seed_head1, F(L.feat1), s.main));
    if (use_planes(m)) {
        CK(renet_pack_planes(F(L.feat1), B, 3 * D, 3 * D, 1, W + L.featp1, s.main));
        const int sk = auto_split_k_planes(B, NE, 3 * D);
        CK(renet_gemm_planes(0, 0, B, NE, 3 * D, 1.f, nullptr, W + L.featp1, (int)L.featp1_ld, L.featp1_plane, m.lin_w_planes,
                             m.lin_w_ld, m.lin_w_plane, 0.f, F(L.logits), (int)L.logits_ld, m.lin_b, nullptr, sk,
                             sk > 1 ? wsm : nullptr, sk > 1 ? L.gemm_ws_bytes : 0, s.main));
        CK(renet_softmax_ce_planes(F(L.logits), b.ent_label, B, NE, (int)L.logits_ld, r->scale_ent, row_loss, W + L.dl1, L.dl_plane,
                                   (int)L.dl_ld, (int)L.dl_rows, s.main));
    } else {
        CK(gemm(s.main, wsm, L.gemm_ws_bytes, 0, 1, B, NE, 3 * D, F(L.feat1), 3 * D, m.lin_w, 3 * D, 0.f, F(L.dl1), NE, m.lin_b));
        CK(renet_softmax_ce(F(L.dl1), b.ent_label, B, NE, NE, r->scale_ent, row_loss, F(L.dl1), s.main));
    }
    s.join();
    if (n_launches) *n_launches = launches;
    return s.rc;
}

int renet_step_backward(const RenetStepModel* mp, const RenetStepBatch* bp, const RenetStepRun* r, const float* g,
                        int defer_side, void* ev_head_done, void* ev_gru_done, int* n_launches) {
    if (!args_ok(mp, bp) || !r || !r->workspace || !g) return RENET_ERR_BADARG;
    const RenetStepModel& m = *mp;
    const RenetStepBatch& b = *bp;
    const Lay L = layout(m, b);
    if (r->workspace_bytes < L.total) return RENET_ERR_WORKSPACE;
    char* W = (char*)r->workspace;
    auto F = [&](size_t off) { return (float*)(W + off); };
    Streams s{(hipStream_t)r->stream, (hipStream_t)(r->side_stream ? r->side_stream : r->stream)};
    int launches = 0;
    const int D = m.D, N = b.N, nA = b.nA, S = b.S, B = b.B, NE = m.num_ent, T = m.T, C2 = m.C2;
    const float p = m.drop_p;
    const bool pruned = nA < N;
    const bool pl = use_planes(m);
    float* wsm = F(L.gemm_ws_main);
    float* wss = F(L.gemm_ws_side);
    float* csw = L.colsum_ws_bytes > 4 ? F(L.colsum_ws) : nullptr;
    auto colsum = [&](const float* X, int M_, int N_, float* out, hipStream_t st) {
        const size_t need = renet_colsum_workspace(M_, N_);
        return renet_colsum(X, M_, N_, N_, out, 1.f, need ? csw : nullptr, need, st);
    };

    if (!pl) CK(renet_scale_by_device_scalar(F(L.dl1), (size_t)B * NE, g, s.main));
    s.fork();
    CK(renet_scale_by_device_scalar(F(L.dl2), (size_t)B * C2, g, s.side));
    CK(gemm(s.side, wss, L.gemm_ws_bytes, 0, 0, B, 2 * D, C2, F(L.dl2), C2, m.linr_w, 2 * D, 0.f, F(L.dfeat2), 2 * D, nullptr));
    CK(gemm(s.side, wss, L.gemm_ws_bytes, 1, 0, C2, 2 * D, B, F(L.dl2), C2, F(L.feat2), 2 * D, 1.f, m.g_linr_w, 2 * D, nullptr));
    CK(colsum(F(L.dl2), B, C2, m.g_linr_b, s.side));
    CK(renet_concat3_bwd(F(L.dfeat2), B, D, 2, p, r->seed_head2, F(L.da2), F(L.dh2), nullptr, s.side));
    if (pl) {
        const int sk1 = auto_split_k_planes(B, 3 * D, NE);
        CK(renet_gemm_planes(0, 1, B, 3 * D, NE, 1.f, g, W + L.dl1, (int)L.dl_ld, L.dl_plane, m.lin_w_planes, m.lin_w_ld,
                             m.lin_w_plane, 0.f, F(L.dfeat1), 3 * D, nullptr, nullptr, sk1, sk1 > 1 ? wsm : nullptr,
                             sk1 > 1 ? L.gemm_ws_bytes : 0, s.main));
        const int sk2 = auto_split_k_planes(NE, 3 * D + 1, B);
        CK(renet_gemm_planes(1, 1, NE, 3 * D + 1, B, 1.f, g, W + L.dl1, (int)L.dl_ld, L.dl_plane, W + L.featp1, (int)L.featp1_ld,
                             L.featp1_plane, 1.f, m.g_lin_w, 3 * D, nullptr, m.g_lin_b, sk2, sk2 > 1 ? wsm : nullptr,
                             sk2 > 1 ? L.gemm_ws_bytes : 0, s.main));
    } else {
        CK(colsum(F(L.dl1), B, NE, m.g_lin_b, s.side));
        CK(gemm(s.main, wsm, L.gemm_ws_bytes, 0, 0, B, 3 * D, NE, F(L.dl1), NE, m.lin_w, 3 * D, 0.f, F(L.dfeat1), 3 * D, nullptr));
        CK(gemm(s.main, wsm, L.gemm_ws_bytes, 1, 0, NE, 3 * D, B, F(L.dl1), NE, F(L.feat1), 3 * D, 1.f, m.g_lin_w, 3 * D, nullptr));
    }
    CK(renet_concat3_bwd(F(L.dfeat1), B, D, 3, p, r->seed_head1, F(L.da1), F(L.dh1), F(L.dc1), s.main));
    s.join();
    if (ev_head_done) {
        const hipError_t e = hipEventRecord((hipEvent_t)ev_head_done, s.main);
        if (e != hipSuccess) return (int)e;
    }
    CK(renet_add_inplace(F(L.da1), F(L.da2), (size_t)B * D, s.main));
    CK(renet_segment_add(F(L.da1), b.plan_s.order, b.plan_s.seg_ptr, b.plan_s.target, b.plan_s.num_segments, D, m.g_ent, s.main));
    CK(renet_segment_add(F(L.dc1), b.plan_r.order, b.plan_r.seg_ptr, b.plan_r.target, b.plan_r.num_segments, D, m.g_rel, s.main));

    {
        const float* dhl[2] = {F(L.dh1), F(L.dh2)};
        const int32_t* so[2] = {b.step_off_host, b.step_off_host};
        const int ls[2] = {b.L, b.L};
        const float* whh[2] = {m.whh, m.whh_r};
        const float* sv[2] = {F(L.sv0), F(L.sv1)};
        float* dgi[2] = {F(L.dgi0), F(L.dgi1)};
        float* dgh[2] = {F(L.dgh0), F(L.dgh1)};
        CK(renet_gru_bwd_layouts(2, dhl, so, ls, D, whh, sv, dgi, dgh, F(L.gru_ws), L.gru_ws_bytes, s.main));
    }
    auto gru_param_grads = [&]() -> int {
        const float* xs[2] = {F(L.X), F(L.Xr)};
        const int in[2] = {4 * D, 3 * D};
        const size_t dgi[2] = {L.dgi0, L.dgi1}, dgh[2] = {L.dgh0, L.dgh1}, sv[2] = {L.sv0, L.sv1};
        float* gwih[2] = {m.g_wih, m.g_wih_r};
        float* gwhh[2] = {m.g_whh, m.g_whh_r};
        float* gbih[2] = {m.g_bih, m.g_bih_r};
        float* gbhh[2] = {m.g_bhh, m.g_bhh_r};
        for (int k = 0; k < 2; ++k) {
            CK(gemm(s.side, wss, L.gemm_ws_bytes, 1, 0, 3 * D, in[k], S, F(dgi[k]), 3 * D, xs[k], in[k], 1.f, gwih[k], in[k], nullptr));
            CK(gemm(s.side, wss, L.gemm_ws_bytes, 1, 0, 3 * D, D, S, F(dgh[k]), 3 * D, F(sv[k]) + 4 * D, 5 * D, 1.f, gwhh[k], D, nullptr));
            CK(colsum(F(dgi[k]), S, 3 * D, gbih[k], s.side));
            CK(colsum(F(dgh[k]), S, 3 * D, gbhh[k], s.side));
        }
        return 0;
    };
    auto gru_done = [&]() -> int {
        if (!ev_gru_done) return 0;
        return (int)hipEventRecord((hipEvent_t)ev_gru_done, s.side);
    };
    {
        s.fork();
        int rc_ = gru_param_grads();
        if (!rc_) rc_ = gru_done();
        if (rc_) return rc_;
    }
    CK(gemm(s.main, wsm, L.gemm_ws_bytes, 0, 0, S, 3 * D, 3 * D, F(L.dgi0), 3 * D, m.wih, 4 * D, 0.f, F(L.dX), 4 * D, nullptr));
    CK(gemm(s.main, wsm, L.gemm_ws_bytes, 0, 0, S, 2 * D, 3 * D, F(L.dgi1), 3 * D, m.wih_r, 3 * D, 0.f, F(L.dXr), 3 * D, nullptr));

    CK(renet_seq_assemble_bwd(F(L.dX), F(L.dXr), b.step_off, b.L, S, B, D, p, r->seed_x, r->seed_xr, F(L.d_rows), F(L.d_ent_seq),
                              F(L.d_rel_seq), s.main));
    CK(renet_zero(F(L.d_h2), (size_t)nA * D, s.main));
    CK(renet_segment_add(F(L.d_rows), b.plan_subj_row.order, b.plan_subj_row.seg_ptr, b.plan_subj_row.target,
                         b.plan_subj_row.num_segments, D, F(L.d_h2), s.main));
    CK(renet_segment_add(F(L.d_ent_seq), b.plan_s.order, b.plan_s.seg_ptr, b.plan_s.target, b.plan_s.num_segments, D, m.g_ent, s.main));
    CK(renet_segment_add(F(L.d_rel_seq), b.plan_r.order, b.plan_r.seg_ptr, b.plan_r.target, b.plan_r.num_segments, D, m.g_rel, s.main));

    const int pair_shift = (T / 2) % T;
    CK(renet_rgcn_bwd_prep(F(L.d_h2), F(L.out2), b.norm, 0, p, r->seed_rgcn2, nA, D, F(L.gn2), F(L.gl2), s.main));
    CK(renet_rgcn_gather_items(F(L.gn2), D, b.it_src, b.it_type, b.grp_ptr, b.n_groups, b.row_ptr, b.col, b.etype, nullptr, m.w2, T,
                               pair_shift, 1, nullptr, 0.f, 0, 0, F(L.dhN), N, b.n_heavy ? b.heavy_rows : nullptr, b.n_heavy,
                               pruned ? nA : 0, 0, pruned ? 1 : 0, s.main));
    CK(gemm(s.main, wsm, L.gemm_ws_bytes, 0, 1, nA, D, D, F(L.gl2), D, m.loop2, D, 1.f, F(L.dhN), D, nullptr));
    s.fork();
    if (pruned)
        CK(renet_rgcn_bwd_w(F(L.out1), F(L.gn2), b.e_src2, b.e_dst2, b.chunk_ptr2, b.chunk_type2, b.n_chunks2, b.type_chunk_ptr2, T,
                            0, D, m.g_w2, 1.f, F(L.bwdw_ws), renet_rgcn_bwd_w_workspace(b.n_chunks2, D), s.side));
    else
        CK(renet_rgcn_bwd_w(F(L.out1), F(L.gn2), b.e_src, b.e_dst, b.chunk_ptr, b.chunk_type, b.n_chunks, b.type_chunk_ptr, T, 0, D,
                            m.g_w2, 1.f, F(L.bwdw_ws), renet_rgcn_bwd_w_workspace(b.n_chunks, D), s.side));
    CK(gemm(s.side, wss, L.gemm_ws_bytes, 1, 0, D, D, nA, F(L.out1), D, F(L.gl2), D, 1.f, m.g_loop2, D, nullptr));

    CK(renet_rgcn_bwd_prep(F(L.dhN), F(L.out1), b.norm, 1, p, r->seed_rgcn1, N, D, F(L.gn1), F(L.gl1), s.main));
    CK(renet_rgcn_gather_items(F(L.gn1), D, b.it_src, b.it_type, b.grp_ptr, b.n_groups, b.row_ptr, b.col, b.etype, nullptr, m.w1, T,
                               pair_shift, 1, nullptr, 0.f, 0, 0, F(L.dh1N), N, b.n_heavy ? b.heavy_rows : nullptr, b.n_heavy, 0, 0,
                               0, s.main));
    s.fork();
    CK(renet_rgcn_bwd_w(m.ent, F(L.gn1), b.e_src_t, b.e_dst, b.chunk_ptr, b.chunk_type, b.n_chunks, b.type_chunk_ptr, T, 0, D,
                        m.g_w1, 1.f, F(L.bwdw_ws), renet_rgcn_bwd_w_workspace(b.n_chunks, D), s.side));
    CK(renet_zero(F(L.gs), (size_t)NE * D, s.main));
    CK(renet_segment_add2(F(L.dh1N), F(L.gl1), b.plan_node_ent.order, b.plan_node_ent.seg_ptr, b.plan_node_ent.target,
                          b.plan_node_ent.num_segments, D, m.g_ent, F(L.gs), s.main));
    CK(gemm(s.main, wsm, L.gemm_ws_bytes, 0, 1, NE, D, D, F(L.gs), D, m.loop1, D, 1.f, m.g_ent, D, nullptr));
    CK(gemm(s.main, wsm, L.gemm_ws_bytes, 1, 0, D, D, NE, m.ent, D, F(L.gs), D, 1.f, m.g_loop1, D, nullptr));
    if (!defer_side) s.join();
    if (n_launches) *n_launches = launches;
    return s.rc;
}

}
```

re-net_amd/ops.py:

```python
import contextlib
import threading
import functools
import ctypes
import os

import numpy as np
import torch
from torch.autograd import Function

import renet_hip as K

_seed_state = {'counter': 0}

SIDE_STREAM = os.environ.get('RENET_SIDE_STREAM', '1') != '0'
_side_streams = {}


class _Side(object):
    def __init__(self, device):
        self.on = SIDE_STREAM and device.type == 'cuda' and K._timer is None
        if self.on:
            key = device.index if device.index is not None else torch.cuda.current_device()
            if key not in _side_streams:
                _side_streams[key] = torch.cuda.Stream(device=device)
# ... 20 lines not shown
    if not sd.on:
        return None
    for t in tensors:
        if isinstance(t, torch.Tensor) and t.is_cuda:
            t.record_stream(sd.side)
    _deferred.append((sd.main, sd.side, (list(tensors), list(keep))))
    return sd


def join_deferred():
    while _deferred:
        main, side, keep = _deferred.pop()
        main.wait_stream(side)
        del keep


def _rank():
    import torch.distributed as dist
    return dist.get_rank() if (dist.is_available() and dist.is_initialized()) else 0


SHARED_GRAPH_SEEDS = False
_shared_tls = threading.local()


@contextlib.contextmanager
def shared_graph_seeds(flag):
    old = getattr(_shared_tls, 'flag', None)
    _shared_tls.flag = bool(flag)
    try:
        yield
    finally:
        _shared_tls.flag = old


def next_seed(graph_site=False):
    _seed_state['counter'] += 1
    scoped = getattr(_shared_tls, 'flag', None)
    shared = SHARED_GRAPH_SEEDS if scoped is None else scoped
    rank = 0 if (graph_site and shared) else _rank()
    x = torch.initial_seed() * 0x9E3779B1 + (rank + 1) * 0xC2B2AE3D27D4EB4F + _seed_state['counter'] * 0x85EBCA77
    return x & 0x7FFFFFFFFFFFFFFF


def reset_seed_counter(value=0):
    _seed_state['counter'] = int(value)


def _c(t):
    return t if t.is_contiguous() else t.contiguous()


INPLACE_GRADS = True

_grad_done_hooks = {}
_hook_tokens = {'next': 0}


_hook_wanted = {}


def register_grad_done_hook(params, callback, wanted=None):
    _hook_tokens['next'] += 1
    token = _hook_tokens['next']
    for p in params:
        _grad_done_hooks.setdefault(id(p), {})[token] = callback
    _hook_wanted[token] = wanted
    return token


def hooks_wanted(param):
    cbs = _grad_done_hooks.get(id(param))
    if not cbs:
        return False
    for token in cbs:
        w = _hook_wanted.get(token)
        if w is None or w():
            return True
    return False


def unregister_grad_done_hook(token):
    _hook_wanted.pop(token, None)
    for pid in list(_grad_done_hooks):
        _grad_done_hooks[pid].pop(token, None)
        if not _grad_done_hooks[pid]:
            del _grad_done_hooks[pid]


def grad_done(param):
    cbs = _grad_done_hooks.get(id(param))
    if cbs:
        for cb in list(cbs.values()):
            cb(param)

debug_tap = None


def _fwd_mode(fwd):
    @functools.wraps(fwd)
    def forward(ctx, *a, **k):
        ctx.gemm_mode = K.current_mode()
        return fwd(ctx, *a, **k)
    return forward


def _bwd_mode(bwd):
    @functools.wraps(bwd)
    def backward(ctx, *g):
        with K.gemm_mode(getattr(ctx, 'gemm_mode', None)):
            return bwd(ctx, *g)
    return backward


def grad_target(t):
    if not INPLACE_GRADS or t is None:
        return None
    base = t if t.is_leaf else getattr(t, '_base', None)
    if base is None or not base.is_leaf or not base.requires_grad or base.grad is None:
        return None
    if not base.grad.is_contiguous() or base.grad.shape != base.shape:
        return None
    if t is base:
        return base.grad
    if t.dim() == 2 and base.dim() == 2 and t.is_contiguous() and t.shape[1] == base.shape[1]:
        off = t.storage_offset() - base.storage_offset()
        if off >= 0 and off % base.shape[1] == 0:
            r0 = off // base.shape[1]
            return base.grad[r0:r0 + t.shape[0]]
    return None


def _gemm_grad(a, b, tgt):
    if tgt is not None:
        K.gemm(a, b, ta=True, out=tgt, beta=1.0)
        return None
    return K.gemm(a, b, ta=True)


def _colsum_grad(x, tgt):
    if tgt is not None:
        K.colsum(x, out=tgt, beta=1.0)
        return None
    return K.colsum(x)


def _segment_grad(src, plan, tgt, shape):
    if tgt is not None:
        K.segment_add(src, plan, tgt)
        return None
    d = torch.zeros(shape, device=src.device, dtype=torch.float32)
    K.segment_add(src, plan, d)
    return d


class GatherRowsFn(Function):

    @staticmethod
    @_fwd_mode
    def forward(ctx, table, idx, plan):
        ctx.plan, ctx.shape, ctx.src = plan, table.shape, table
        return K.gather_rows(_c(table), idx)

    @staticmethod
    @_bwd_mode
    def backward(ctx, g):
        return _segment_grad(_c(g), ctx.plan, grad_target(ctx.src), ctx.shape), None, None


class RGCNLayerFn(Function):

    @staticmethod
    @_fwd_mode
    def forward(ctx, h, weight, loop_weight, g, reverse, relu, drop_p, seed, n_out):
        ctx.src_w, ctx.src_loop = weight, loop_weight
        h, weight, loop_weight = _c(h), _c(weight), _c(loop_weight)
        n = h.shape[0]
        n_out = n if (n_out is None or n_out >= n) else int(n_out)
        pruned = n_out < n
        shift = g.num_types // 2 if reverse else 0
        h_op = K.operand(h[:n_out])
        out = K.gemm(h_op, loop_weight)
        K.rgcn_gather_items(h, g, weight, shift, False, out, drop_p, seed, relu, out, use_norm=True, pruned=pruned,
                            w16=K.gather_weight_bf16(weight))
        ctx.g, ctx.relu, ctx.drop_p, ctx.seed, ctx.shift, ctx.n_out = g, relu, drop_p, seed, shift, n_out
        ctx.h_op = h_op if K.is_handle(h_op) else None
        ctx.save_for_backward(h, weight, loop_weight, out)
        return out

    @staticmethod
    @_bwd_mode
    def backward(ctx, g_out):
        h, weight, loop_weight, out = ctx.saved_tensors
        g, n_out = ctx.g, ctx.n_out
        tgt_loop, tgt_w = grad_target(ctx.src_loop), grad_target(ctx.src_w)
        g_out = _c(g_out)
        n, d = h.shape
        pruned = n_out < n
        gn = torch.empty(n_out, d, device=h.device, dtype=torch.float32)
        g_loop = torch.empty(n_out, d, device=h.device, dtype=torch.float32)
        K.rgcn_bwd_prep(g_out, out, g.norm, ctx.relu, ctx.drop_p, ctx.seed, gn, g_loop)
        dh = torch.empty(n, d, device=h.device, dtype=torch.float32)
        pair_shift = (ctx.shift + g.num_types // 2) % g.num_types
        K.rgcn_gather_items(gn, g, weight, pair_shift, True, None, 0.0, 0, False, dh, use_norm=False, pruned=pruned,
                            src_limit=n_out if pruned else 0, w16=K.gather_weight_bf16(weight))
        gl_op = K.operand(g_loop)
        h_op = ctx.h_op if ctx.h_op is not None else h[:n_out]
        K.gemm(gl_op, loop_weight, tb=True, out=dh[:n_out], beta=1.0)
        acc = tgt_w is not None
        d_w = tgt_w if acc else torch.empty_like(weight)

        def weight_grads():
            if pruned:
                K.rgcn_bwd_w(h, gn, g.e_src2, g.e_dst2, g.chunk_ptr2, g.chunk_type2, g.n_chunks2, g.type_chunk_ptr2,
                             g.num_types, ctx.shift, d_w, beta=1.0 if acc else 0.0)
            else:
                K.rgcn_bwd_w(h, gn, g.e_src, g.e_dst, g.chunk_ptr, g.chunk_type, g.n_chunks, g.type_chunk_ptr,
                             g.num_types, ctx.shift, d_w, beta=1.0 if acc else 0.0)
            return _gemm_grad(h_op, gl_op, tgt_loop)
        sd = _deferred_scope(h.device, (h, gn, g_loop, getattr(gl_op, 'p', None), getattr(gl_op, 'part', None),
                                        getattr(h_op, 'p', None), getattr(h_op, 'part', None), getattr(h_op, 't', None),
                                        getattr(gl_op, 't', None)), keep=(g, h_op, gl_op, weight_grads)) \
            if (acc and tgt_loop is not None and K.current_mode() != 'bf16s') else None
        if sd is not None:
            if isinstance(gl_op, K.F32Op):
                gl_op.bound()
            if isinstance(h_op, K.F32Op):
                h_op.bound()
            sd.side.wait_stream(sd.main)
            with sd():
                weight_grads()
            d_loop = None
        else:
            d_loop = weight_grads()
        return dh, None if acc else d_w, d_loop, None, None, None, None, None, None


class TableRows(object):
    __slots__ = ('table', 'idx', 'plan')

    def __init__(self, table, idx, plan):
        self.table, self.idx, self.plan = table, idx, plan

    def materialise(self):
        return GatherRowsFn.apply(self.table, self.idx, self.plan)


class RGCNTableLayerFn(Function):

    @staticmethod
    @_fwd_mode
    def forward(ctx, table, weight, loop_weight, g, reverse, relu, drop_p, seed):
        ctx.src_tab, ctx.src_w, ctx.src_loop = table, weight, loop_weight
        table, weight, loop_weight = _c(table), _c(weight), _c(loop_weight)
        shift = g.num_types // 2 if reverse else 0
        ew = K.gemm(table, loop_weight)
        out = torch.empty(g.N, table.shape[1], device=table.device, dtype=torch.float32)
        K.rgcn_gather_items_table(table, g, weight, shift, ew, drop_p, seed, relu, out,
                                  table16=K.gather_weight_bf16(table), w16=K.gather_weight_bf16(weight))
        ctx.g, ctx.relu, ctx.drop_p, ctx.seed, ctx.shift = g, relu, drop_p, seed, shift
        ctx.save_for_backward(table, weight, loop_weight, out)
        return out

    @staticmethod
    @_bwd_mode
    def backward(ctx, g_out):
        table, weight, loop_weight, out = ctx.saved_tensors
        g = ctx.g
        tgt_tab, tgt_loop, tgt_w = grad_target(ctx.src_tab), grad_target(ctx.src_loop), grad_target(ctx.src_w)
        g_out = _c(g_out)
        n, d = out.shape
        dev = out.device
        gn = torch.empty(n, d, device=dev, dtype=torch.float32)
        g_loop = torch.empty(n, d, device=dev, dtype=torch.float32)
        K.rgcn_bwd_prep(g_out, out, g.norm, ctx.relu, ctx.drop_p, ctx.seed, gn, g_loop)
        dh = torch.empty(n, d, device=dev, dtype=torch.float32)
        pair_shift = (ctx.shift + g.num_types // 2) % g.num_types
        K.rgcn_gather_items(gn, g, weight, pair_shift, True, None, 0.0, 0, False, dh, use_norm=False,
                            w16=K.gather_weight_bf16(weight))
        acc = tgt_w is not None
        d_w = tgt_w if acc else torch.empty_like(weight)
        e_src_t = g.table_items()[3]
        sd = _deferred_scope(dev, (gn, e_src_t), keep=(g, table)) if acc else None
        with (sd() if sd is not None else contextlib.nullcontext()):
            K.rgcn_bwd_w(table, gn, e_src_t, g.e_dst, g.chunk_ptr, g.chunk_type, g.n_chunks, g.type_chunk_ptr,
                         g.num_types, ctx.shift, d_w, beta=1.0 if acc else 0.0)
        gs = torch.zeros(table.shape, device=dev, dtype=torch.float32)
        d_tab = tgt_tab if tgt_tab is not None else torch.zeros(table.shape, device=dev, dtype=torch.float32)
        K.segment_add2(dh, g_loop, g.plan_node_ent, d_tab, gs)
        gs_op = K.operand(gs)
        K.gemm(gs_op, loop_weight, tb=True, out=d_tab, beta=1.0)
        d_loop = _gemm_grad(table, gs_op, tgt_loop)
        return (None if tgt_tab is not None else d_tab), None if acc else d_w, d_loop, None, None, None, None, None


class SeqAssembleFn(Function):

    @staticmethod
    @_fwd_mode
    def forward(ctx, h2, ent, rel, glob, g, drop_p, seed_x, seed_xr, _lazy_bf16=False):
        ctx.src_ent, ctx.src_rel = ent, rel
        h2, ent, rel, glob = _c(h2), _c(ent), _c(rel), _c(glob)
        if _lazy_bf16 and K.current_mode() == 'bf16s':
            mx, mxr = K.seq_assemble_fwd_bf16(h2, ent, rel, glob, g.subj_row, g.row_ent, g.row_rel, g.glob_row,
                                              drop_p, seed_x, seed_xr)
            x, xr = K.lazy_shell(mx, h2.device), K.lazy_shell(mxr, h2.device)
        else:
            x, xr = K.seq_assemble_fwd(h2, ent, rel, glob, g.subj_row, g.row_ent, g.row_rel, g.glob_row,
                                       drop_p, seed_x, seed_xr)
        ctx.g, ctx.drop_p, ctx.seeds = g, drop_p, (seed_x, seed_xr)
        ctx.shapes = (h2.shape, ent.shape, rel.shape)
        return x, xr

    @staticmethod
    @_bwd_mode
    def backward(ctx, dx, dxr):
        g = ctx.g
        d = ctx.shapes[0][1]
        tgt_ent, tgt_rel = grad_target(ctx.src_ent), grad_target(ctx.src_rel)
        d_rows, d_ent_seq, d_rel_seq = K.seq_assemble_bwd(_c(dx), _c(dxr), g.step_off, g.L, g.B, d, ctx.drop_p,
                                                          *ctx.seeds)
        d_h2 = _segment_grad(d_rows, g.plan_subj_row, None, ctx.shapes[0])
        d_ent = _segment_grad(d_ent_seq, g.plan_s, tgt_ent, ctx.shapes[1])
        d_rel = _segment_grad(d_rel_seq, g.plan_r, tgt_rel, ctx.shapes[2])
        return d_h2, d_ent, d_rel, None, None, None, None, None, None


class GRUFn(Function):

    @staticmethod
    @_fwd_mode
    def forward(ctx, x, w_ih, w_hh, b_ih, b_hh, step_off, total_rows):
        x, w_ih, w_hh, b_ih, b_hh = _c(x), _c(w_ih), _c(w_hh), _c(b_ih), _c(b_hh)
        hdim = w_hh.shape[1]
        gi = K.gemm(x, w_ih, tb=True, bias=b_ih)
        full, saved = K.gru_fwd(gi, step_off, hdim, w_hh, b_hh, out_rows=total_rows)
        nnz = int(step_off[1] - step_off[0]) if len(step_off) > 1 else 0
        ctx.step_off, ctx.nnz, ctx.hdim = step_off, nnz, hdim
        ctx.save_for_backward(x, w_ih, w_hh, saved)
        return full.unsqueeze(0)

    @staticmethod
    @_bwd_mode
    def backward(ctx, dh):
        x, w_ih, w_hh, saved = ctx.saved_tensors
        hdim, nnz = ctx.hdim, ctx.nnz
        dh_last = _c(dh[0, :nnz])
        d_gi, d_gh = K.gru_bwd(dh_last, ctx.step_off, hdim, w_hh, saved)
        s = x.shape[0]
        dx = K.gemm(d_gi, w_ih)
        d_wih = K.gemm(d_gi, x, ta=True)
        d_bih = K.colsum(d_gi)
        h_prev = saved[:, 4 * hdim:]
        d_whh = K.gemm(d_gh, h_prev, ta=True)
        d_bhh = K.colsum(d_gh)
        return dx, d_wih, d_whh, d_bih, d_bhh, None, None


class MultiGRUFn(Function):

    @staticmethod
    @_fwd_mode
    def forward(ctx, step_offs, total_rows, live_cols, *ts):
        n = len(ts) // 5
        ctx.live_cols = live_cols
        ctx.src_w = [(ts[5 * k + 1], ts[5 * k + 2]) for k in range(n)]
        ctx.src_b = [(ts[5 * k + 3], ts[5 * k + 4]) for k in range(n)]
        ts = [_c(t) for t in ts]
        xs, w_ihs, w_hhs = ts[0::5], ts[1::5], ts[2::5]
        b_ihs, b_hhs = ts[3::5], ts[4::5]
        hdim = w_hhs[0].shape[1]
        x_ops = [K.operand(x) for x in xs]
        sd = _Side(xs[0].device)
        gis = [None] * n
        with sd():
            for k in range(1, n, 2):
                gis[k] = K.gemm(x_ops[k], w_ihs[k], tb=True, bias=b_ihs[k])
        for k in range(0, n, 2):
            gis[k] = K.gemm(x_ops[k], w_ihs[k], tb=True, bias=b_ihs[k])
        sd.join()
        ctx.x_ops = x_ops if any(K.is_handle(x) for x in x_ops) else None
        hs, svs = K.gru_fwd_layouts(gis, step_offs, hdim, w_hhs, b_hhs, total_rows)
        ctx.step_offs, ctx.hdim, ctx.n = step_offs, hdim, n
        ctx.nnz = [int(o[1] - o[0]) if len(o) > 1 else 0 for o in step_offs]
        ctx.save_for_backward(*(list(xs) + list(w_ihs) + list(w_hhs) + list(svs)))
        if debug_tap is not None:
            for k, h in enumerate(hs):
                debug_tap('h_n' if k % 2 == 0 else 'q_n', h)
        return tuple(h.unsqueeze(0) for h in hs)

    @staticmethod
    @_bwd_mode
    def backward(ctx, *dhs):
        n, hdim = ctx.n, ctx.hdim
        sv_ = ctx.saved_tensors
        xs, w_ihs, w_hhs, svs = sv_[:n], sv_[n:2 * n], sv_[2 * n:3 * n], sv_[3 * n:4 * n]
        d_gis, d_ghs = K.gru_bwd_layouts([_c(dh[0, :nz]) for dh, nz in zip(dhs, ctx.nnz)], ctx.step_offs, hdim,
                                         list(w_hhs), list(svs), out_bf16=(K.current_mode() == 'bf16s'))
        def param_grads(k, dgi_op):
            t_ih, t_hh = (grad_target(t) for t in ctx.src_w[k])
            t_bi, t_bh = (grad_target(t) for t in ctx.src_b[k])
            dgi, dgh, xx, s_ = d_gis[k], d_ghs[k], xs[k], svs[k]
            x_op = ctx.x_ops[k] if ctx.x_ops is not None else xx
            dwi = _gemm_grad(dgi_op, x_op, t_ih)
            dgh_op = K.operand_like(dgh, dgi_op)
            hp_op = K.operand(s_[:, 4 * hdim:], bound=K.const_bound(1.0, s_.device))
            return [dwi, _gemm_grad(dgh_op, hp_op, t_hh), _colsum_grad(dgi, t_bi), _colsum_grad(dgh, t_bh)]

        def input_grad(k, dgi_op):
            xx = xs[k]
            live = ctx.live_cols[k] if ctx.live_cols is not None else None
            if live is not None and live < xx.shape[1]:
                dxx = torch.empty_like(xx)
                K.gemm(dgi_op, w_ihs[k][:, :live], out=dxx[:, :live])
                dxx[:, live:].zero_()
                return dxx
            return K.gemm(dgi_op, w_ihs[k])

        def problem(k):
            dgi_op = K.operand(d_gis[k])
            return [input_grad(k, dgi_op)] + param_grads(k, dgi_op)

        all_in_place = all(grad_target(t) is not None for k in range(n) for t in ctx.src_w[k] + ctx.src_b[k])
        sd0 = _Side(d_gis[0].device if not isinstance(d_gis[0], K.BF16Mat) else d_gis[0].p.device)
        if DEFER_WEIGHT_GRADS and sd0.on and all_in_place and K.current_mode() != 'bf16s':
            ops_ = [K.operand(d_gis[k]) for k in range(n)]
            if K.current_mode() == 'f16x3':
                for o in ops_:
                    o.bound()
            sd = _Side(sd0.main.device)
            res = [None] * n
            with sd():
                for k in range(n):
                    param_grads(k, ops_[k])
                _gru_grads_done(ctx)
            live_ops = ops_ + (list(ctx.x_ops) if ctx.x_ops is not None else [])
            for t in list(d_gis) + list(d_ghs) + list(xs) + list(svs) + \
                    [getattr(o, 'part', None) for o in live_ops] + [getattr(o, 't', None) for o in live_ops]:
                if isinstance(t, torch.Tensor) and t.is_cuda:
                    t.record_stream(sd.side)
            for k in range(n):
                res[k] = [input_grad(k, ops_[k]), None, None, None, None]
            _deferred.append((sd.main, sd.side, (list(d_gis), list(d_ghs), list(xs), list(svs), live_ops)))
            out = [None, None, None]
            for k in range(n):
                out += res[k]
            return tuple(out)

        keys = [id(ctx.src_w[k][0]) for k in range(n)]
        uniq = list(dict.fromkeys(keys))
        on_side = [len(uniq) > 1 and keys[k] == uniq[1] for k in range(n)]
        res = [None] * n
        sd = sd0
        with sd():
            for k in range(n):
                if on_side[k]:
                    res[k] = problem(k)
        for k in range(n):
            if not on_side[k]:
                res[k] = problem(k)
        sd.join()
        if all_in_place:
            _gru_grads_done(ctx)
        out = [None, None, None]
        for k in range(n):
            out += res[k]
        return tuple(out)


def _gru_grads_done(ctx):
    if not _grad_done_hooks:
        return
    for k in range(len(ctx.src_w)):
        for t in list(ctx.src_w[k]) + list(ctx.src_b[k]):
            grad_done(t)


# ... 34 lines not shown
        return K.scale_by_device_scalar(dlogits, g, bound_in=float(grad_scale))
    K.scale_by_device_scalar(dlogits, g)
    return None


def _head_backward(dlogits, feat, feat_op, weight, t_w, t_b, bias_side=None, bound=None, g=None):
    if isinstance(dlogits, K.PlanesMat):
        w_pl = K.weight_planes(weight)
        dfeat = K.gemm_planes(dlogits, w_pl, alpha_dev=g)
        acc = t_w is not None and t_b is not None
        d_w = t_w if acc else torch.empty_like(weight)
        d_b = t_b if acc else torch.empty(weight.shape[0], device=weight.device, dtype=torch.float32)
        K.gemm_planes(dlogits, feat_op, ta=True, out=d_w, col_out=d_b, alpha_dev=g, beta=1.0 if acc else 0.0)
        return dfeat, (None if acc else d_w), (None if acc else d_b)
    dl_op = K.operand(dlogits, bound=bound)
    f_op = feat_op if feat_op is not None else feat

    if bias_side is not None:
        with bias_side():
            d_b = _colsum_grad(dlogits, t_b)
    dfeat = K.gemm(dl_op, weight)
    d_w = _gemm_grad(dl_op, f_op, t_w)
    if bias_side is None:
        d_b = _colsum_grad(dlogits, t_b)
    return dfeat, d_w, d_b


def _consume_ce_gradient(ctx):
    if ctx.consumed:
        raise RuntimeError('%s: the saved (softmax - onehot) buffers were scaled in place by the first backward pass; a '
                           'second pass over the same graph is not supported' % type(ctx).__name__)
    ctx.consumed = True


def _scatter_head_rows(da_rows, dc_rows, plan_a, plan_c, t_a, t_c, a_shape, c_shape):
    d_a = _segment_grad(da_rows, plan_a, t_a, a_shape)
    return d_a, (_segment_grad(dc_rows, plan_c, t_c, c_shape) if dc_rows is not None else None)


class HeadCEFn(Function):

    @staticmethod
    @_fwd_mode
    def forward(ctx, a, ia, hmid, c, ic, weight, bias, target, plan_a, plan_c, drop_p, seed, loss_scale=1.0):
        ctx.srcs = (a, c, weight, bias)
        a, hmid, weight, bias = _c(a), _c(hmid), _c(weight), _c(bias)
        c = _c(c) if c is not None else None
        b, d = hmid.shape
        need_grad = any(ctx.needs_input_grad)
        ctx.grad_scale = float(loss_scale) / b
        row_loss, feat, logits, ctx.dl_bf16, feat_op = _head_forward(a, ia, hmid, c, ic, weight, bias, target, drop_p,
                                                                     seed, ctx.grad_scale, need_grad)
        ctx.meta = (d, 3 if c is not None else 2, drop_p, seed, plan_a, plan_c, a.shape,
                    c.shape if c is not None else None)
        if need_grad:
            ctx.save_for_backward(feat, logits, weight)
            ctx.consumed = False
            ctx.feat_op = feat_op
        return row_loss.mean() if loss_scale == 1.0 else row_loss.mean() * float(loss_scale)

    @staticmethod
    @_bwd_mode
    def backward(ctx, g):
        feat, dlogits, weight = ctx.saved_tensors
        d, parts, drop_p, seed, plan_a, plan_c, a_shape, c_shape = ctx.meta
        t_a, t_c, t_w, t_b = [grad_target(t) for t in ctx.srcs]
        _consume_ce_gradient(ctx)
        if ctx.dl_bf16 is not None:
            dlogits = ctx.dl_bf16
        bound = _scale_ce_gradient(dlogits, g, ctx.grad_scale)
        sd = _Side(feat.device)
        dfeat, d_w, d_b = _head_backward(dlogits, feat, ctx.feat_op, weight, t_w, t_b, bias_side=sd, bound=bound, g=g)
        sd.join()
        if t_w is not None and t_b is not None:
            grad_done(ctx.srcs[2])
            grad_done(ctx.srcs[3])
        da_rows, dh, dc_rows = K.concat3_bwd(dfeat, d, parts, drop_p, seed)
        d_a, d_c = _scatter_head_rows(da_rows, dc_rows, plan_a, plan_c, t_a, t_c, a_shape, c_shape)
        return d_a, None, dh, d_c, None, d_w, d_b, None, None, None, None, None, None


_loss_weights = {}


def _loss_weight_vector(b, w1, w2, device):
    key = (b, float(w1), float(w2), str(device))
    v = _loss_weights.get(key)
    if v is None:
        if len(_loss_weights) > 16:
            _loss_weights.clear()
        v = torch.cat((torch.full((b,), float(w1)), torch.full((b,), float(w2)))).to(device)
        _loss_weights[key] = v
    return v


class DualHeadCEFn(Function):

    @staticmethod
    @_fwd_mode
    def forward(ctx, a, ia, h1, c, ic, w1, b1, target1, h2, w2, b2, target2, plan_a, plan_c, drop_p, seed1, seed2,
                loss_scale=1.0, rel_weight=0.1, row_tap=None):
        ctx.srcs = (a, c, w1, b1, w2, b2)
        a, h1, h2, c, w1, b1, w2, b2 = (_c(t) for t in (a, h1, h2, c, w1, b1, w2, b2))
        b, d = h1.shape
        need_grad = any(ctx.needs_input_grad)
        s1, s2 = float(loss_scale) / b, float(loss_scale) * float(rel_weight) / b
        rl = torch.empty(2 * b, device=h1.device, dtype=torch.float32)
        def head2():
            return _head_forward(a, ia, h2, None, None, w2, b2, target2, drop_p, seed2, s2, need_grad, row_loss=rl[b:])
        sd = _Side(h1.device)
        if debug_tap is None:
            with sd():
                _, feat2, lg2, dl2, fop2 = head2()
        _, feat1, lg1, dl1, fop1 = _head_forward(a, ia, h1, c, ic, w1, b1, target1, drop_p, seed1, s1, need_grad,
                                                 row_loss=rl[:b])
        if debug_tap is not None:
            _, feat2, lg2, dl2, fop2 = head2()
        sd.join()
        ctx.meta = (d, drop_p, seed1, seed2, plan_a, plan_c, a.shape, c.shape)
        ctx.grad_scales = (s1, s2)
        if need_grad:
            ctx.save_for_backward(feat1, lg1, w1, feat2, lg2, w2)
            ctx.consumed = False
            ctx.bf16 = (dl1, fop1, dl2, fop2)
        if row_tap is not None:
            row_tap.append((rl.detach(), s1, s2))
        return torch.dot(rl, _loss_weight_vector(b, s1, s2, h1.device))

    @staticmethod
    @_bwd_mode
    def backward(ctx, g):
        feat1, dl1, w1, feat2, dl2, w2 = ctx.saved_tensors
        d, drop_p, seed1, seed2, plan_a, plan_c, a_shape, c_shape = ctx.meta
        t_a, t_c, t_w1, t_b1, t_w2, t_b2 = [grad_target(t) for t in ctx.srcs]
        _consume_ce_gradient(ctx)
        b1_, fop1, b2_, fop2 = ctx.bf16
        dl1 = b1_ if b1_ is not None else dl1
        dl2 = b2_ if b2_ is not None else dl2
        bound1 = _scale_ce_gradient(dl1, g, ctx.grad_scales[0])
        sd = _Side(feat1.device)
        with sd():
            bound2 = _scale_ce_gradient(dl2, g, ctx.grad_scales[1])
            dfeat2, d_w2, d_b2 = _head_backward(dl2, feat2, fop2, w2, t_w2, t_b2, bound=bound2, g=g)
            da2, dh2, _ = K.concat3_bwd(dfeat2, d, 2, drop_p, seed2)
        dfeat1, d_w1, d_b1 = _head_backward(dl1, feat1, fop1, w1, t_w1, t_b1, bias_side=sd, bound=bound1, g=g)
        da1, dh1, dc1 = K.concat3_bwd(dfeat1, d, 3, drop_p, seed1)
        sd.join()
        if t_w1 is not None and t_b1 is not None:
            grad_done(ctx.srcs[2])
            grad_done(ctx.srcs[3])
        if t_w2 is not None and t_b2 is not None:
            grad_done(ctx.srcs[4])
            grad_done(ctx.srcs[5])
        da1.add_(da2)
        d_a, d_c = _scatter_head_rows(da1, dc1, plan_a, plan_c, t_a, t_c, a_shape, c_shape)
        return (d_a, None, dh1, d_c, None, d_w1, d_b1, None, dh2, d_w2, d_b2, None) + (None,) * 8


class SegmentPoolFn(Function):

    @staticmethod
    @_fwd_mode
    def forward(ctx, h, seg_ptr, num_graphs, is_max):
        h = _c(h)
        out, arg = K.segment_pool_fwd(h, seg_ptr, num_graphs, is_max)
        ctx.meta = (seg_ptr, arg, num_graphs, is_max, h.shape[0])
        return out

    @staticmethod
    @_bwd_mode
    def backward(ctx, dout):
        seg_ptr, arg, num_graphs, is_max, n = ctx.meta
        return K.segment_pool_bwd(_c(dout), seg_ptr, arg, num_graphs, is_max, n), None, None, None


class DropoutFn(Function):

    @staticmethod
    @_fwd_mode
    def forward(ctx, x, drop_p, seed):
        ctx.meta = (drop_p, seed)
        return K.dropout(_c(x), drop_p, seed)

    @staticmethod
    @_bwd_mode
    def backward(ctx, g):
        return K.dropout(_c(g), *ctx.meta), None, None


class LinearFn(Function):

    @staticmethod
    @_fwd_mode
    def forward(ctx, x, weight, bias):
        x, weight = _c(x), _c(weight)
        ctx.save_for_backward(x, weight)
        return K.gemm(x, weight, tb=True, bias=_c(bias))

    @staticmethod
    @_bwd_mode
    def backward(ctx, g):
        x, weight = ctx.saved_tensors
        g = _c(g)
        return (K.gemm(g, weight), K.gemm(g, x, ta=True), K.colsum(g))


def host_offsets(step_off):
    arr = np.ascontiguousarray(step_off, dtype=np.int32)
    return (ctypes.c_int32 * len(arr))(*arr.tolist())
```

re-net_amd/renet_hip.py:

```python
import contextlib
import ctypes
import functools
import os
import threading
import weakref

import torch

_HERE = os.path.dirname(os.path.abspath(__file__))
LIB_PATH = os.environ.get('RENET_HIP_LIB', os.path.join(_HERE, 'csrc', 'librenet_hip.so'))

_lib = None

c_int = ctypes.c_int
c_float = ctypes.c_float
c_void_p = ctypes.c_void_p
c_size_t = ctypes.c_size_t
c_u64 = ctypes.c_uint64

_GEMM_ARGS = [c_int, c_int, c_int, c_int, c_int, c_float, c_void_p, c_int, c_void_p, c_int,
              c_float, c_void_p, c_int, c_void_p, c_int, c_void_p, c_size_t, c_void_p]
_RGCN_BWD_W_ARGS = [c_void_p, c_void_p, c_void_p, c_void_p, c_void_p, c_void_p, c_int,
                    c_void_p, c_int, c_int, c_int, c_void_p, c_float, c_void_p, c_size_t, c_void_p]
_GRU_FWD_LAYOUTS_ARGS = [c_int, c_void_p, c_void_p, c_void_p, c_int, c_void_p, c_void_p, c_void_p,
                         c_void_p, c_void_p, c_void_p, c_size_t, c_void_p]
_GRU_BWD_LAYOUTS_ARGS = [c_int, c_void_p, c_void_p, c_void_p, c_int, c_void_p, c_void_p, c_void_p,
                         c_void_p, c_void_p, c_size_t, c_void_p]

_SIGNATURES = {
    'renet_version': (c_int, []),
    'renet_gather_rows': (c_int, [c_void_p, c_void_p, c_int, c_int, c_void_p, c_void_p]),
    'renet_segment_add': (c_int, [c_void_p, c_void_p, c_void_p, c_void_p, c_int, c_int, c_void_p, c_void_p]),
    'renet_segment_add2': (c_int, [c_void_p, c_void_p, c_void_p, c_void_p, c_void_p, c_int, c_int, c_void_p, c_void_p,
                                   c_void_p]),
    'renet_rgcn_gather': (c_int, [c_void_p, c_int, c_void_p, c_void_p, c_void_p, c_void_p, c_void_p, c_int,
                                  c_int, c_int, c_void_p, c_float, c_u64, c_int, c_void_p, c_int, c_void_p,
                                  c_int, c_int, c_int, c_int, c_void_p]),
    'renet_rgcn_gather_items': (c_int, [c_void_p, c_int, c_void_p, c_void_p, c_void_p, c_int, c_void_p, c_void_p,
                                        c_void_p, c_void_p, c_void_p, c_int, c_int, c_int, c_void_p, c_float, c_u64,
                                        c_int, c_void_p, c_int, c_void_p, c_int, c_int, c_int, c_int, c_void_p]),
    'renet_rgcn_gather_items_bf16': (c_int, [c_void_p, c_int, c_void_p, c_void_p, c_void_p, c_int, c_void_p, c_void_p,
                                             c_void_p, c_void_p, c_void_p, c_int, c_int, c_int, c_int, c_void_p,
                                             c_float, c_u64, c_int, c_void_p, c_int, c_void_p, c_int, c_int, c_int,
                                             c_int, c_void_p]),
    'renet_rgcn_gather_items_table_bf16': (c_int, [c_void_p, c_int, c_int, c_int, c_void_p, c_void_p, c_void_p, c_int,
                                                   c_void_p, c_void_p, c_void_p, c_void_p, c_void_p, c_void_p, c_int,
                                                   c_int, c_int, c_void_p, c_float, c_u64, c_int, c_void_p, c_int,
                                                   c_void_p, c_int, c_void_p]),
    'renet_rgcn_gather_items_table': (c_int, [c_void_p, c_int, c_int, c_void_p, c_void_p, c_void_p, c_int, c_void_p,
                                              c_void_p, c_void_p, c_void_p, c_void_p, c_void_p, c_int, c_int, c_void_p,
                                              c_float, c_u64, c_int, c_void_p, c_int, c_void_p, c_int, c_void_p]),
    'renet_compose_table_items': (c_int, [c_void_p, c_void_p, c_void_p, c_int, c_void_p, c_void_p, c_int, c_void_p,
                                          c_void_p, c_void_p, c_void_p, c_void_p]),
    'renet_rgcn_bwd_prep': (c_int, [c_void_p, c_void_p, c_void_p, c_int, c_float, c_u64, c_int, c_int,
                                    c_void_p, c_void_p, c_void_p]),
    'renet_rgcn_bwd_prep_bounds': (c_int, [c_void_p, c_void_p, c_void_p, c_int, c_float, c_u64, c_int, c_int,
                                           c_void_p, c_void_p, c_void_p, c_void_p]),
    'renet_bound_parts': (c_int, [c_size_t]),
    'renet_rgcn_bwd_w_workspace': (c_size_t, [c_int, c_int]),
    'renet_rgcn_bwd_w': (c_int, _RGCN_BWD_W_ARGS),
    'renet_rgcn_bwd_w64': (c_int, _RGCN_BWD_W_ARGS),
    'renet_gemm_workspace': (c_size_t, [c_int, c_int, c_int]),
    'renet_gemm_f32': (c_int, _GEMM_ARGS),
    'renet_gemm_f32_split': (c_int, _GEMM_ARGS),
    'renet_gemm_bf16': (c_int, _GEMM_ARGS),
    'renet_gemm_split_plan': (c_int, [c_int, c_int, c_int, c_int, c_int, c_void_p, c_int, c_void_p, c_int, c_int, c_void_p]),
    'renet_maxabs_blocks': (c_int, [c_int, c_int, c_int]),
    'renet_maxabs_partials_multi': (c_int, [c_void_p, c_int, c_void_p]),
    'renet_maxabs_partials': (c_int, [c_void_p, c_int, c_int, c_int, c_void_p, c_void_p]),
    'renet_gemm_f32_h3': (c_int, [c_int, c_int, c_int, c_int, c_int, c_float, c_void_p, c_int, c_void_p, c_int,
                                  c_float, c_void_p, c_int, c_void_p, c_int, c_void_p, c_size_t, c_void_p, c_int,
                                  c_void_p, c_int, c_void_p]),
    'renet_bf16_bytes': (c_size_t, [c_int, c_int]),
    'renet_pack_bf16': (c_int, [c_void_p, c_int, c_int, c_int, c_void_p, c_void_p]),
    'renet_gemm_bf16s': (c_int, _GEMM_ARGS),
    'renet_bf16_zero_padding': (c_int, [c_void_p, c_int, c_int, c_int, c_int, c_void_p]),
    'renet_seq_assemble_fwd_bf16': (c_int, [c_void_p, c_void_p, c_void_p, c_void_p, c_void_p, c_void_p, c_void_p,
                                            c_void_p, c_int, c_int, c_float, c_u64, c_u64, c_void_p, c_int, c_void_p,
                                            c_int, c_int, c_void_p]),
    'renet_softmax_ce_bf16': (c_int, [c_void_p, c_void_p, c_int, c_int, c_int, c_float, c_void_p, c_void_p, c_int, c_int,
                                      c_void_p]),
    'renet_gru_bwd_layouts_bf16out': (c_int, [c_int, c_void_p, c_void_p, c_void_p, c_int, c_void_p, c_void_p, c_void_p,
                                              c_void_p, c_int, c_void_p, c_size_t, c_void_p]),
    'renet_colsum_bf16': (c_int, [c_void_p, c_int, c_int, c_int, c_void_p, c_float, c_void_p, c_size_t, c_void_p]),
    'renet_scale_bf16_by_device_scalar': (c_int, [c_void_p, c_size_t, c_void_p, c_void_p]),
    'renet_planes_elems': (c_size_t, [c_int, c_int]),
    'renet_pack_planes': (c_int, [c_void_p, c_int, c_int, c_int, c_int, c_void_p, c_void_p]),
    'renet_gemm_planes': (c_int, [c_int, c_int, c_int, c_int, c_int, c_float, c_void_p, c_void_p, c_int, c_size_t,
                                  c_void_p, c_int, c_size_t, c_float, c_void_p, c_int, c_void_p, c_void_p, c_int,
                                  c_void_p, c_size_t, c_void_p]),
    'renet_softmax_ce_planes': (c_int, [c_void_p, c_void_p, c_int, c_int, c_int, c_float, c_void_p, c_void_p, c_size_t,
                                        c_int, c_int, c_void_p]),
    'renet_step_workspace': (c_size_t, [c_void_p, c_void_p]),
    'renet_step_forward': (c_int, [c_void_p, c_void_p, c_void_p, c_void_p, c_void_p]),
    'renet_step_backward': (c_int, [c_void_p, c_void_p, c_void_p, c_void_p, c_int, c_void_p, c_void_p, c_void_p]),
    'renet_add_inplace': (c_int, [c_void_p, c_void_p, c_size_t, c_void_p]),
    'renet_zero': (c_int, [c_void_p, c_size_t, c_void_p]),
    'renet_colsum_workspace': (c_size_t, [c_int, c_int]),
    'renet_colsum': (c_int, [c_void_p, c_int, c_int, c_int, c_void_p, c_float, c_void_p, c_size_t, c_void_p]),
    'renet_scale_by_device_scalar': (c_int, [c_void_p, c_size_t, c_void_p, c_void_p]),
    'renet_scale_by_device_scalar_bound': (c_int, [c_void_p, c_size_t, c_void_p, c_float, c_void_p, c_void_p]),
    'renet_seq_assemble_fwd': (c_int, [c_void_p, c_void_p, c_void_p, c_void_p, c_void_p, c_void_p, c_void_p,
                                       c_void_p, c_int, c_int, c_float, c_u64, c_u64, c_void_p, c_void_p,
                                       c_void_p]),
    'renet_seq_assemble_fwd_bounds': (c_int, [c_void_p, c_void_p, c_void_p, c_void_p, c_void_p, c_void_p, c_void_p,
                                              c_void_p, c_int, c_int, c_float, c_u64, c_u64, c_void_p, c_void_p,
                                              c_void_p, c_void_p, c_void_p]),
    'renet_seq_assemble_bwd': (c_int, [c_void_p, c_void_p, c_void_p, c_int, c_int, c_int, c_int, c_float,
                                       c_u64, c_u64, c_void_p, c_void_p, c_void_p, c_void_p]),
    'renet_gru_workspace': (c_size_t, [c_int, c_int]),
    'renet_gru_fwd': (c_int, [c_void_p, c_void_p, c_int, c_int, c_void_p, c_void_p, c_void_p, c_int, c_void_p,
                              c_void_p, c_size_t, c_void_p]),
    'renet_gru_bwd': (c_int, [c_void_p, c_void_p, c_int, c_int, c_void_p, c_void_p, c_void_p, c_void_p,
                              c_void_p, c_size_t, c_void_p]),
    'renet_gru_fwd_multi': (c_int, [c_int, c_void_p, c_void_p, c_int, c_int, c_void_p, c_void_p, c_void_p,
                                    c_int, c_void_p, c_void_p, c_size_t, c_void_p]),
    'renet_gru_bwd_multi': (c_int, [c_int, c_void_p, c_void_p, c_int, c_int, c_void_p, c_void_p, c_void_p,
                                    c_void_p, c_void_p, c_size_t, c_void_p]),
    'renet_gru_fwd_layouts': (c_int, _GRU_FWD_LAYOUTS_ARGS),
    'renet_gru_bwd_layouts': (c_int, _GRU_BWD_LAYOUTS_ARGS),
    'renet_gru_bound_parts': (c_int, [c_int]),
    'renet_gru_bwd_layouts_bounds': (c_int, [c_int, c_void_p, c_void_p, c_void_p, c_int, c_void_p, c_void_p, c_void_p,
                                             c_void_p, c_void_p, c_void_p, c_size_t, c_void_p]),
    'renet_gru_fwd_layouts_f32': (c_int, _GRU_FWD_LAYOUTS_ARGS),
    'renet_gru_bwd_layouts_f32': (c_int, _GRU_BWD_LAYOUTS_ARGS),
    'renet_gru_fwd_layouts_bf16': (c_int, _GRU_FWD_LAYOUTS_ARGS),
    'renet_gru_bwd_layouts_bf16': (c_int, _GRU_BWD_LAYOUTS_ARGS),
    'renet_concat3_fwd': (c_int, [c_void_p, c_void_p, c_void_p, c_void_p, c_void_p, c_int, c_int, c_float,
                                  c_u64, c_void_p, c_void_p]),
    'renet_concat3_fwd_bounds': (c_int, [c_void_p, c_void_p, c_void_p, c_void_p, c_void_p, c_int, c_int, c_float,
                                         c_u64, c_void_p, c_void_p, c_void_p]),
    'renet_concat3_bwd': (c_int, [c_void_p, c_int, c_int, c_int, c_float, c_u64, c_void_p, c_void_p,
                                  c_void_p, c_void_p]),
    'renet_dropout': (c_int, [c_void_p, c_size_t, c_float, c_u64, c_void_p, c_void_p]),
    'renet_softmax_ce': (c_int, [c_void_p, c_void_p, c_int, c_int, c_int, c_float, c_void_p, c_void_p,
                                 c_void_p]),
    'renet_joint_softmax': (c_int, [c_void_p, c_int, c_int, c_int, c_int, c_void_p, c_int, c_void_p, c_void_p]),
    'renet_topk_workspace': (c_size_t, [c_int]),
    'renet_topk_positive': (c_int, [c_void_p, c_size_t, c_int, c_int, c_int, c_void_p, c_void_p, c_void_p, c_size_t,
                                    c_void_p]),
    'renet_build_batch_workspace': (c_size_t, [c_void_p, c_int, c_int, c_int]),
    'renet_build_batch_both': (c_int, [c_void_p, c_void_p, c_int, c_int, c_int, c_int, c_int, c_void_p, c_void_p, c_size_t,
                                       c_void_p]),
    'renet_build_full_graphs_workspace': (c_size_t, [c_void_p, c_int, c_int, c_int]),
    'renet_build_full_graphs': (c_int, [c_void_p, c_void_p, c_int, c_int, c_int, c_int, c_void_p, c_void_p, c_size_t,
                                        c_void_p]),
    'renet_adam_workspace': (c_size_t, [c_size_t]),
    'renet_adam_step': (c_int, [c_void_p, c_void_p, c_void_p, c_void_p, c_size_t, c_float, c_float, c_float, c_float,
                                c_float, c_float, c_int, c_int, c_void_p, c_size_t, c_void_p, c_void_p]),
    'renet_adam_step_scaled': (c_int, [c_void_p, c_void_p, c_void_p, c_void_p, c_size_t, c_float, c_float, c_float,
                                       c_float, c_float, c_float, c_float, c_int, c_int, c_void_p, c_size_t, c_void_p,
                                       c_void_p]),
    'renet_sumsq_partials': (c_int, [c_void_p, c_size_t, c_void_p, c_int, c_void_p]),
    'renet_adam_step_presummed': (c_int, [c_void_p, c_void_p, c_void_p, c_void_p, c_size_t, c_float, c_float, c_float,
                                          c_float, c_float, c_float, c_float, c_int, c_int, c_void_p, c_int, c_void_p,
                                          c_void_p]),
    'renet_host_filter_edges': (ctypes.c_int64, [c_void_p] * 5 + [ctypes.c_int64, ctypes.c_int64, c_void_p, c_void_p,
                                                 ctypes.c_int64, c_void_p, c_void_p, c_void_p, c_void_p]),
    'renet_host_filter_edges_sparse': (ctypes.c_int64, [c_void_p] * 7 + [ctypes.c_int64, ctypes.c_int64, c_void_p,
                                                        c_void_p, ctypes.c_int64, c_void_p, c_void_p, c_void_p,
                                                        c_void_p]),
    'renet_host_node_sets': (ctypes.c_int64, [ctypes.c_int64] + [c_void_p] * 5 + [ctypes.c_int64, ctypes.c_int64]
                             + [c_void_p] * 7),
    'renet_host_type_chunks': (ctypes.c_int64, [ctypes.c_int64, c_void_p, c_void_p, c_void_p, ctypes.c_int64,
                                                ctypes.c_int64, ctypes.c_int64] + [c_void_p] * 6),
    'renet_host_edge_layouts': (None, [ctypes.c_int64, ctypes.c_int64, c_void_p, c_void_p, c_void_p, ctypes.c_int64,
                                       ctypes.c_int64, ctypes.c_int64] + [c_void_p] * 12),
    'renet_host_segplan': (ctypes.c_int64, [c_void_p, ctypes.c_int64, ctypes.c_int64, c_void_p, c_void_p, c_void_p]),
    'renet_host_gather_items': (ctypes.c_int64, [ctypes.c_int64, c_void_p, c_void_p, c_void_p, ctypes.c_int64,
                                                 ctypes.c_int64, ctypes.c_int64] + [c_void_p] * 5),
    'renet_segment_pool_fwd': (c_int, [c_void_p, c_void_p, c_int, c_int, c_int, c_void_p, c_void_p, c_void_p]),
    'renet_segment_pool_bwd': (c_int, [c_void_p, c_void_p, c_void_p, c_int, c_int, c_int, c_int, c_void_p,
                                       c_void_p]),
}

EXPORTS = sorted(_SIGNATURES)


class RenetHipError(RuntimeError):
    pass


class _Bound(object):
    """The bound entry points (attribute per symbol)."""


def _exact_arity(fn, name, n):
    def call(*a):
        if len(a) != n:
            raise RenetHipError('%s takes %d arguments, %d given' % (name, n, len(a)))
        return fn(*a)
    call.__name__ = name
    return call


def lib():
    global _lib
    if _lib is None:
        if not os.path.isfile(LIB_PATH):
            raise RenetHipError('librenet_hip.so not built (%s); run `python re-net_amd/build.py` '
                                '-- there is no fallback path' % LIB_PATH)
        L = ctypes.CDLL(LIB_PATH)
        ns = _Bound()
        for name, (res, args) in _SIGNATURES.items():
            fn = getattr(L, name)
            fn.restype = res
            fn.argtypes = args
            setattr(ns, name, _exact_arity(fn, name, len(args)))
        if ns.renet_version() != 1:
            raise RenetHipError('ABI version mismatch')
        ns._cdll = L
        _lib = ns
    return _lib


def _check(rc, what):
    if rc != 0:
        raise RenetHipError('%s failed with code %d' % (what, rc))


def _dev_ptr(dtype, default_name, t, name=None):
    if t is None:
        return None
    if not (t.is_cuda and t.dtype == dtype and t.is_contiguous()):
        raise RenetHipError('%s must be a contiguous %s device tensor' % (name or default_name, str(dtype)[6:]))
    return t.data_ptr()


_f32 = functools.partial(_dev_ptr, torch.float32, 'tensor')
_i32 = functools.partial(_dev_ptr, torch.int32, 'index')


_raw_stream = getattr(torch._C, '_cuda_getCurrentRawStream', None)


def _stream():
    if _raw_stream is not None:
        return _raw_stream(torch.cuda.current_device())
    return torch.cuda.current_stream().cuda_stream


class KernelTimer(object):

    def __init__(self):
        self.recs = {}

    def begin(self):
        e = torch.cuda.Event(enable_timing=True)
        e.record()
        return e

    def end(self, name, e0, flops=0.0, nbytes=0.0, tag=None):
        e1 = torch.cuda.Event(enable_timing=True)
        e1.record()
        self.recs.setdefault(name, []).append((e0, e1, flops, nbytes, tag))

    def summary(self):
        torch.cuda.synchronize()
        out = {}
        for name, rs in self.recs.items():
            out[name] = {'calls': len(rs), 'ms': sum(r[0].elapsed_time(r[1]) for r in rs),
                         'flops': sum(r[2] for r in rs), 'bytes': sum(r[3] for r in rs)}
        return out

    def by_tag(self, name):
        torch.cuda.synchronize()
        out = {}
        for r in self.recs.get(name, []):
            o = out.setdefault(r[4], {'calls': 0, 'ms': 0.0, 'flops': 0.0})
            o['calls'] += 1
            o['ms'] += r[0].elapsed_time(r[1])
            o['flops'] += r[2]
        return out


_timer = None


def _timed():
    return _timer.begin() if _timer is not None else None


def _timed_end(t0, name, flops=0.0, nbytes=0.0, tag=None):
    if t0 is not None:
        _timer.end(name, t0, flops=flops, nbytes=nbytes, tag=tag)

GLUE = ('softmax_ce_planes', 'gather_rows', 'segment_add', 'segment_add2', 'compose_table_items', 'rgcn_bwd_prep', 'colsum',
        'scale_by_device_scalar', 'seq_assemble_fwd', 'seq_assemble_fwd_bf16', 'softmax_ce_bf16', 'seq_assemble_bwd',
        'concat3_fwd', 'concat3_bwd', 'dropout', 'softmax_ce', 'adam_step', 'segment_pool_fwd', 'segment_pool_bwd',
        'pack_bf16_glue')
_glue_saved = {}


def _timed_glue(name, fn):
    @functools.wraps(fn)
    def call(*a, **k):
        t = _timer
        if t is None:
            return fn(*a, **k)
        e0 = t.begin()
        try:
            return fn(*a, **k)
        finally:
            t.end('glue:' + name, e0)
    return call


def set_timer(t, glue=False):
    global _timer
    _timer = t
    g = globals()
    for name, fn in _glue_saved.items():
        g[name] = fn
    _glue_saved.clear()
    if t is not None and glue:
        for name in GLUE:
            if name in g and callable(g[name]):
                _glue_saved[name] = g[name]
                g[name] = _timed_glue(name, g[name])


def gather_rows(table, idx, out=None):
    n, d = idx.numel(), table.shape[1]
    if out is None:
        out = torch.empty(n, d, device=table.device, dtype=torch.float32)
    _check(lib().renet_gather_rows(_f32(table), _i32(idx), n, d, _f32(out), _stream()), 'gather_rows')
    return out


def segment_add(src, plan, dst):
    _check(lib().renet_segment_add(_f32(src), _i32(plan.order), _i32(plan.seg_ptr), _i32(plan.target),
                                   plan.num_segments, src.shape[1], _f32(dst), _stream()), 'segment_add')
    return dst


def segment_add2(src0, src1, plan, dst0, dst1):
    _check(lib().renet_segment_add2(_f32(src0), _f32(src1), _i32(plan.order), _i32(plan.seg_ptr), _i32(plan.target),
                                    plan.num_segments, src0.shape[1], _f32(dst0), _f32(dst1), _stream()), 'segment_add2')


def rgcn_gather(x, row_ptr, col, etype, scale, weight, type_shift, transpose_w, addend, drop_p, seed,
                relu, out, heavy_rows=None, heavy_thresh=0, src_limit=0, addend_rows=0, n_edges=None):
    n, d = x.shape[0], x.shape[1]
    t0 = _timed()
    _check(lib().renet_rgcn_gather(_f32(x), d, _i32(row_ptr), _i32(col), _i32(etype), _f32(scale),
                                   _f32(weight), weight.shape[0], type_shift, int(transpose_w),
                                   _f32(addend), float(drop_p), int(seed), int(relu), _f32(out),
                                   out.shape[0], _i32(heavy_rows) if heavy_rows is not None else None,
                                   heavy_rows.numel() if heavy_rows is not None else 0, int(heavy_thresh),
                                   int(src_limit), int(addend_rows), _stream()), 'rgcn_gather')
    if t0 is not None:
        nn = out.shape[0]
        e = col.numel() if n_edges is None else int(n_edges)
        nbytes = e * (d * 4 + 8) + nn * (d * 4 + 8) + weight.numel() * 4 + (nn * d * 4 if addend is not None else 0)
        _timed_end(t0, 'rgcn_gather' if n_edges is None else 'rgcn_gather_pruned', nbytes=float(nbytes))
    return out


def gather_bytes(n_edges, n_rows, d, weight_numel, has_addend, x_bytes=4, w_bytes=4):
    return (n_edges * (d * x_bytes + 8) + n_rows * (d * 4 + 8) + weight_numel * w_bytes +
            (n_rows * d * 4 if has_addend else 0))


def rgcn_gather_items(x, g, weight, type_shift, transpose_w, addend, drop_p, seed, relu, out, use_norm=True,
                      pruned=False, src_limit=0, addend_rows=0, w16=None):
    d = x.shape[1]
    n_rows = out.shape[0]
    prefix = n_rows < g.N
    n_groups = g.n_groups_out if prefix else g.n_groups
    heavy = g.heavy_rows_out if prefix else g.heavy_rows
    if max(x.numel(), out.numel()) * 4 >= (1 << 31):
        return rgcn_gather(x, g.row_ptr, g.col, g.etype, g.norm if use_norm else None, weight, type_shift,
                           transpose_w, addend, drop_p, seed, relu, out, heavy, g.heavy_thresh, src_limit,
                           addend_rows, n_edges=g.E_out if pruned else None)
    t0 = _timed()
    hv, nhv = (_i32(heavy), heavy.numel()) if heavy is not None else (None, 0)
    if w16 is not None:
        _check(lib().renet_rgcn_gather_items_bf16(
            _f32(x), d, _i32(g.it_src), _i32(g.it_type), _i32(g.grp_ptr), int(n_groups), _i32(g.row_ptr), _i32(g.col),
            _i32(g.etype), _f32(g.norm) if use_norm else None, w16.p.data_ptr(), w16.p.shape[1], weight.shape[0],
            int(type_shift), int(transpose_w), _f32(addend), float(drop_p), int(seed), int(relu), _f32(out), n_rows,
            hv, nhv, int(src_limit), int(addend_rows), int(pruned), _stream()), 'rgcn_gather_items_bf16')
    else:
        _check(lib().renet_rgcn_gather_items(
            _f32(x), d, _i32(g.it_src), _i32(g.it_type), _i32(g.grp_ptr), int(n_groups), _i32(g.row_ptr), _i32(g.col),
            _i32(g.etype), _f32(g.norm) if use_norm else None, _f32(weight), weight.shape[0], int(type_shift),
            int(transpose_w), _f32(addend), float(drop_p), int(seed), int(relu), _f32(out), n_rows, hv, nhv,
            int(src_limit), int(addend_rows), int(pruned), _stream()), 'rgcn_gather_items')
    if t0 is not None:
        e = g.E_out if pruned else g.E
        name = 'rgcn_gather_%s_%s' % ('bwdh' if transpose_w else 'fwd', 'pruned' if pruned else 'full')
        wb = 2 if w16 is not None else 4
        _timed_end(t0, name, nbytes=float(gather_bytes(e, n_rows, d, weight.numel(), addend is not None, 4, wb)),
                   tag=float(gather_bytes(e, n_rows, d, weight.numel(), False, 4, wb)))
    return out


def gather_weight_bf16(weight):
    if current_mode() != 'bf16s' or os.environ.get('RENET_BF16_GATHER', '1') == '0':
        return None
    if weight.numel() * 2 >= (1 << 31):
        return None
    return _as_bf16(weight)[0]


def compose_table_items(g):
    ni, e = g.it_src.numel(), g.col.numel()
    buf = torch.empty(2 * ni + 2 * e + 16, device=g.col.device, dtype=torch.int32)
    a0, a1, a2 = (ni + 3) & ~3, 2 * ((ni + 3) & ~3), 2 * ((ni + 3) & ~3) + ((e + 3) & ~3)
    it_src_t, it_type_t, col_t, e_src_t = buf[:ni], buf[a0:a0 + ni], buf[a1:a1 + e], buf[a2:a2 + e]
    _check(lib().renet_compose_table_items(_i32(g.node_ent), _i32(g.it_src), _i32(g.it_type), ni, _i32(g.col),
                                           _i32(g.e_src), e, it_src_t.data_ptr(), it_type_t.data_ptr(),
                                           col_t.data_ptr(), e_src_t.data_ptr(), _stream()), 'compose_table_items')
    return it_src_t, it_type_t, col_t, e_src_t


def rgcn_gather_items_table(table, g, weight, type_shift, addend_table, drop_p, seed, relu, out, table16=None,
                            w16=None):
    d = table.shape[1]
    n_rows = out.shape[0]
    it_src_t, it_type_t, col_t, _ = g.table_items()
    heavy = g.heavy_rows
    t0 = _timed()
    if table16 is not None and w16 is not None:
        _check(lib().renet_rgcn_gather_items_table_bf16(
            table16.p.data_ptr(), table16.p.shape[1], table.shape[0], d, _i32(it_src_t), _i32(it_type_t),
            _i32(g.grp_ptr), int(g.n_groups), _i32(g.row_ptr), _i32(col_t), _i32(g.etype), _i32(g.node_ent),
            _f32(g.norm), w16.p.data_ptr(), w16.p.shape[1], weight.shape[0], int(type_shift), _f32(addend_table),
            float(drop_p), int(seed), int(relu), _f32(out), n_rows, _i32(heavy) if heavy is not None else None,
            heavy.numel() if heavy is not None else 0, _stream()), 'rgcn_gather_items_table_bf16')
    else:
        _check(lib().renet_rgcn_gather_items_table(
            _f32(table), table.shape[0], d, _i32(it_src_t), _i32(it_type_t), _i32(g.grp_ptr), int(g.n_groups),
            _i32(g.row_ptr), _i32(col_t), _i32(g.etype), _i32(g.node_ent), _f32(g.norm), _f32(weight), weight.shape[0],
            int(type_shift), _f32(addend_table), float(drop_p), int(seed), int(relu), _f32(out), n_rows,
            _i32(heavy) if heavy is not None else None, heavy.numel() if heavy is not None else 0, _stream()),
            'rgcn_gather_items_table')
    if t0 is not None:
        eb = 2 if (table16 is not None and w16 is not None) else 4
        _timed_end(t0, 'rgcn_gather_fwd_full',
                   nbytes=float(gather_bytes(g.E, n_rows, d, weight.numel(), addend_table is not None, eb, eb)),
                   tag=float(gather_bytes(g.E, n_rows, d, weight.numel(), False, eb, eb)))
    return out


def rgcn_bwd_prep(g_out, out, norm, relu, drop_p, seed, gn, g_loop):
    n, d = g_out.shape
    args = (_f32(g_out), _f32(out), _f32(norm), int(relu), float(drop_p), int(seed), n, d, _f32(gn), _f32(g_loop))
    if _fused_bounds(g_loop):
        _call_with_bounds('rgcn_bwd_prep_bounds', args, n * (d // 4), (g_loop,))
        return
    _check(lib().renet_rgcn_bwd_prep(*args, _stream()), 'rgcn_bwd_prep')


def rgcn_bwd_w(x, gn, e_src, e_dst, chunk_ptr, chunk_type, n_chunks, type_chunk_ptr, num_types, type_shift,
               dW, beta=0.0):
    d = x.shape[1]
    big = max(x.numel(), gn.numel()) * 4 >= (1 << 31) or os.environ.get('RENET_BWDW_64') == '1'
    nbytes = lib().renet_rgcn_bwd_w_workspace(n_chunks, d)
    ws = torch.empty(max(nbytes // 4, 1), device=x.device, dtype=torch.float32)
    t0 = _timed()
    fn = lib().renet_rgcn_bwd_w64 if big else lib().renet_rgcn_bwd_w
    _check(fn(_f32(x), _f32(gn), _i32(e_src), _i32(e_dst), _i32(chunk_ptr), _i32(chunk_type), n_chunks,
              _i32(type_chunk_ptr), num_types, type_shift, d, _f32(dW), float(beta), ws.data_ptr(), nbytes, _stream()),
           'rgcn_bwd_w')
    _timed_end(t0, 'rgcn_bwd_w', nbytes=float(e_src.numel() * (2 * d * 4 + 8) + dW.numel() * 4))
    return dW


def _ld(t):
    if t.dim() != 2 or t.stride(1) != 1:
        raise RenetHipError('GEMM operands must be 2-D with unit inner stride')
    return t.stride(0)


def gemm_split_plan(ta, tb, m, n, k, lda=None, ldb=None, split_k=1, a_ptr=0, b_ptr=0):
    lda = (m if ta else k) if lda is None else lda
    ldb = (k if tb else n) if ldb is None else ldb
    out = (ctypes.c_int * 8)()
    _check(lib().renet_gemm_split_plan(int(ta), int(tb), m, n, k, a_ptr, lda, b_ptr, ldb, split_k,
                                       ctypes.cast(out, ctypes.c_void_p)), 'renet_gemm_split_plan')
    names = {0: 'fused', 1: 'two_phase_128', 2: 'two_phase_256', 3: 'weight_resident', 4: 'bf16'}
    return {'kernel': names[out[0]], 'raw': bool(out[1]), 'xcd_order': out[2], 'grid': (out[3], out[4], out[5]),
            'split_k': out[6]}


def auto_split_k(m, n, k):
    return _split_k_model(m, n, k, tile_m=128, slots=512, full=256, smax=128)


def _split_k_model(m, n, k, tile_m, slots, full, smax):
# ... 789 lines not shown
```

Before: 372,700 triples/s.

## Fuse sequence-backward row scatter with RGCN bwd prep and batch entity/relation segment adds

Replaces the chain seq_assemble_bwd(d_rows) → zero → segment_add → rgcn_bwd_prep with one kernel that reads dX/dXr, applies the dropout masks, segment-sums per subject row, and writes gn/g_loop directly. It also merges four separate entity and relation segment_add launches, plus an add_inplace, into a single two-job kernel that sums a + a_plus + b per segment. This removes intermediate d_rows/d_h2 buffers, several full-tensor passes and launches. The trade-off is more complex templated kernels with higher register and LDS use, and a separate zero-rows kernel for rows that have no segment.

```diff
diff --git a/include/renet_hip.h b/include/renet_hip.h
--- a/include/renet_hip.h
+++ b/include/renet_hip.h
@@ -21,6 +21,10 @@
                       const int32_t* seg_target, int U, int D, float* dst, void* stream);
 int renet_segment_add2(const float* src0, const float* src1, const int32_t* order, const int32_t* seg_ptr,
                        const int32_t* seg_target, int U, int D, float* dst0, float* dst1, void* stream);
+int renet_segment_add_multi(const float* a0, const float* a0_plus, const float* b0, const int32_t* order0,
+                            const int32_t* seg_ptr0, const int32_t* target0, int U0, float* dst0, const float* a1,
+                            const float* a1_plus, const float* b1, const int32_t* order1, const int32_t* seg_ptr1,
+                            const int32_t* target1, int U1, float* dst1, int D, void* stream);
 
 int renet_rgcn_gather(const float* x, int D, const int32_t* row_ptr, const int32_t* col,
                       const int32_t* etype, const float* scale, const float* W, int T, int type_shift,
@@ -148,6 +152,11 @@
 int renet_seq_assemble_bwd(const float* dX, const float* dXr, const int32_t* step_off, int L, int S,
                            int B, int D, float drop_p, uint64_t seed_x, uint64_t seed_xr, float* dRows,
                            float* dEntSeq, float* dRelSeq, void* stream);
+int renet_seq_bwd_rows_segment_prep_parts(int U);
+int renet_seq_bwd_rows_segment_prep(const float* dX, const float* dXr, int S, float seq_drop_p, uint64_t seed_x,
+                                    uint64_t seed_xr, const int32_t* order, const int32_t* seg_ptr, const int32_t* seg_target,
+                                    int U, const float* out, const float* norm, int relu, float drop_p, uint64_t seed, int nA,
+                                    int D, float* gn, float* g_loop, float* bound_part, void* stream);
 
 size_t renet_gru_workspace(int B, int H);
 int renet_gru_fwd(const float* Gi, const int32_t* step_off, int L, int H, const float* Whh,
diff --git a/re-net_amd/csrc/rgcn.hip b/re-net_amd/csrc/rgcn.hip
--- a/re-net_amd/csrc/rgcn.hip
+++ b/re-net_amd/csrc/rgcn.hip
@@ -787,6 +787,144 @@
 }
 
 constexpr int kSegWaves = 16, kSegShort = 16, kSegUnr = 8;
+
+struct SegRowsPlain {
+    const float4* p;
+    struct Raw { float4 a; };
+    __device__ __forceinline__ bool present() const { return true; }
+    __device__ __forceinline__ bool wide() const { return false; }
+    __device__ __forceinline__ Raw raw(int row, int ch, int CH) const { return Raw{p[(size_t)row * CH + ch]}; }
+    __device__ __forceinline__ float4 value(const Raw& r, int, int, int) const { return r.a; }
+};
+struct SegRowsSum {
+    const float4* p;
+    const float4* q;
+    struct Raw { float4 a, b; };
+    __device__ __forceinline__ bool present() const { return p != nullptr; }
+    __device__ __forceinline__ bool wide() const { return q != nullptr; }
+    __device__ __forceinline__ Raw raw(int row, int ch, int CH) const {
+        const size_t i = (size_t)row * CH + ch;
+        Raw r;
+        r.a = p[i];
+        r.b = q ? q[i] : r.a;
+        return r;
+    }
+    __device__ __forceinline__ float4 value(const Raw& r, int, int, int) const { return q ? f4_add(r.a, r.b) : r.a; }
+};
+struct SegRowsSeqBwd {
+    const float4* dX;
+    const float4* dXr;
+    DropCfg dx, dxr;
+    struct Raw { float4 a, b; };
+    __device__ __forceinline__ bool present() const { return true; }
+    __device__ __forceinline__ bool wide() const { return true; }
+    __device__ __forceinline__ Raw raw(int row, int ch, int CH) const {
+        return Raw{dX[(size_t)row * 4 * CH + ch], dXr[(size_t)row * 3 * CH + ch]};
+    }
+    __device__ __forceinline__ float4 value(const Raw& r, int row, int ch, int CH) const {
+#pragma clang fp contract(off)
+        const float4 ma = renet_drop4(dx, (size_t)row * 4 * CH + ch), mb = renet_drop4(dxr, (size_t)row * 3 * CH + ch);
+        const float4 t = f4_mul(r.b, mb);
+        return make_float4(__builtin_fmaf(r.a.x, ma.x, t.x), __builtin_fmaf(r.a.y, ma.y, t.y), __builtin_fmaf(r.a.z, ma.z, t.z),
+                           __builtin_fmaf(r.a.w, ma.w, t.w));
+    }
+};
+
+template <int NB, class Src>
+__device__ __forceinline__ void seg_accum(const Src& src, const int32_t* __restrict__ order, int k, int k1, int ch, int CH,
+                                          float4& s) {
+    typename Src::Raw v[NB];
+#pragma unroll
+    for (int j = 0; j < NB; ++j) v[j] = src.raw(order[min(k + j, k1 - 1)], ch, CH);
+#pragma unroll
+    for (int j = 0; j < NB; ++j)
+        if (k + j < k1) s = f4_add(s, src.value(v[j], order[min(k + j, k1 - 1)], ch, CH));
+}
+template <class Src>
+__device__ __forceinline__ void seg_accum_unr(const Src& src, const int32_t* __restrict__ order, int k, int k1, int ch, int CH,
+                                              float4& s) {
+    if (src.wide()) {
+        seg_accum<kSegUnr / 2>(src, order, k, k1, ch, CH, s);
+        __builtin_amdgcn_sched_barrier(0);
+        if (k + kSegUnr / 2 < k1) seg_accum<kSegUnr / 2>(src, order, k + kSegUnr / 2, k1, ch, CH, s);
+    } else {
+        seg_accum<kSegUnr>(src, order, k, k1, ch, CH, s);
+    }
+}
+
+template <int NS, class Src>
+struct SegAddEpi {
+    float4* dst;
+    const Src* src;
+    __device__ __forceinline__ void operator()(int v, int ch, int CH, const float4 (&s)[NS]) {
+        const size_t i = (size_t)v * CH + ch;
+        float4 d = dst[i];
+#pragma unroll
+        for (int q = 0; q < NS; ++q)
+            if (src[q].present()) d = f4_add(d, s[q]);
+        dst[i] = d;
+    }
+};
+
+template <int NS, class Src, class Epi>
+__device__ __forceinline__ void segment_walk(const Src (&src)[NS], Epi& epi, const int32_t* __restrict__ order,
+                                             const int32_t* __restrict__ seg_ptr, const int32_t* __restrict__ seg_target,
+                                             int U, int CH, int nwg) {
+    __shared__ float4 red[NS][kSegWaves][128];
+    const int lane = threadIdx.x & 63;
+    const int wave = __builtin_amdgcn_readfirstlane(threadIdx.x >> 6);
+    {
+        const int u = blockIdx.x + wave * nwg;
+        const int k0 = u < U ? seg_ptr[u] : 0, k1 = u < U ? seg_ptr[u + 1] : 0;
+        const int len = k1 - k0;
+        if (len > 0 && len <= kSegShort) {
+            const int tgt = seg_target[u];
+            for (int ch = lane; ch < CH; ch += 64) {
+                float4 s[NS];
+#pragma unroll
+                for (int q = 0; q < NS; ++q) {
+                    s[q] = make_float4(0.f, 0.f, 0.f, 0.f);
+                    if (!src[q].present()) continue;
+                    for (int k = k0; k < k1; k += kSegUnr) seg_accum_unr(src[q], order, k, k1, ch, CH, s[q]);
+                }
+                epi(tgt, ch, CH, s);
+            }
+        }
+    }
+    for (int j = 0; j < kSegWaves; ++j) {
+        const int u = blockIdx.x + j * nwg;
+        if (u >= U) break;
+        const int k0 = seg_ptr[u], k1 = seg_ptr[u + 1];
+        if (k1 - k0 <= kSegShort) continue;
+        const int tgt = seg_target[u];
+        for (int ch = lane; ch < CH; ch += 64) {
+#pragma unroll
+            for (int q = 0; q < NS; ++q) {
+                float4 s = make_float4(0.f, 0.f, 0.f, 0.f);
+                if (src[q].present()) {
+                    for (int k = k0 + wave * kSegUnr; k < k1; k += kSegWaves * kSegUnr)
+                        seg_accum_unr(src[q], order, k, k1, ch, CH, s);
+                }
+                red[q][wave][ch] = s;
+            }
+        }
+        __syncthreads();
+        if (wave == 0) {
+            for (int ch = lane; ch < CH; ch += 64) {
+                float4 r[NS];
+#pragma unroll
+                for (int q = 0; q < NS; ++q) {
+                    r[q] = red[q][0][ch];
+#pragma unroll
+                    for (int w = 1; w < kSegWaves; ++w) r[q] = f4_add(r[q], red[q][w][ch]);
+                }
+                epi(tgt, ch, CH, r);
+            }
+        }
+        __syncthreads();
+    }
+}
+
 __global__ __launch_bounds__(kSegWaves * 64) void segment_add_kernel(const float4* __restrict__ src0,
                                                                      const float4* __restrict__ src1,
                                                                      const int32_t* __restrict__ order,
@@ -794,60 +932,75 @@
                                                                      const int32_t* __restrict__ seg_target,
                                                                      int U, int CH, float4* __restrict__ dst0,
                                                                      float4* __restrict__ dst1) {
-    const float4* __restrict__ src = blockIdx.y ? src1 : src0;
-    float4* __restrict__ dst = blockIdx.y ? dst1 : dst0;
-    __shared__ float4 red[kSegWaves][128];
-    const int lane = threadIdx.x & 63;
-    const int wave = __builtin_amdgcn_readfirstlane(threadIdx.x >> 6);
-    const int nwg = gridDim.x;
-    {
-        const int u = blockIdx.x + wave * nwg;
-        const int k0 = u < U ? seg_ptr[u] : 0, k1 = u < U ? seg_ptr[u + 1] : 0;
-        const int len = k1 - k0;
-        if (len > 0 && len <= kSegShort) {
-            const size_t tgt = (size_t)seg_target[u] * CH;
-            for (int ch = lane; ch < CH; ch += 64) {
-                float4 s = make_float4(0.f, 0.f, 0.f, 0.f);
-                for (int k = k0; k < k1; k += kSegUnr) {
-                    float4 v[kSegUnr];
-#pragma unroll
-                    for (int j = 0; j < kSegUnr; ++j) v[j] = src[(size_t)order[min(k + j, k1 - 1)] * CH + ch];
-#pragma unroll
-                    for (int j = 0; j < kSegUnr; ++j)
-                        if (k + j < k1) s = f4_add(s, v[j]);
-                }
-                dst[tgt + ch] = f4_add(dst[tgt + ch], s);
-            }
-        }
-    }
-    for (int j = 0; j < kSegWaves; ++j) {
-        const int u = blockIdx.x + j * nwg;
-        if (u >= U) break;
-        const int k0 = seg_ptr[u], k1 = seg_ptr[u + 1];
-        if (k1 - k0 <= kSegShort) continue;
-        const size_t tgt = (size_t)seg_target[u] * CH;
-        for (int ch = lane; ch < CH; ch += 64) {
-            float4 s = make_float4(0.f, 0.f, 0.f, 0.f);
-            for (int k = k0 + wave * kSegUnr; k < k1; k += kSegWaves * kSegUnr) {
-                float4 v[kSegUnr];
-#pragma unroll
-                for (int q = 0; q < kSegUnr; ++q) v[q] = src[(size_t)order[min(k + q, k1 - 1)] * CH + ch];
-#pragma unroll
-                for (int q = 0; q < kSegUnr; ++q)
-                    if (k + q < k1) s = f4_add(s, v[q]);
-            }
-            red[wave][ch] = s;
-        }
+    const SegRowsPlain src[1] = {{blockIdx.y ? src1 : src0}};
+    SegAddEpi<1, SegRowsPlain> epi{blockIdx.y ? dst1 : dst0, src};
+    segment_walk<1>(src, epi, order, seg_ptr, seg_target, U, CH, (int)gridDim.x);
+}
+
+struct SegJob {
+    const float4 *a, *a2, *b;
+    const int32_t *order, *seg_ptr, *target;
+    float4* dst;
+    int U, nwg;
+};
+__global__ __launch_bounds__(kSegWaves * 64) void segment_add_multi_kernel(SegJob j0, SegJob j1, int CH) {
+    const SegJob j = blockIdx.y ? j1 : j0;
+    if ((int)blockIdx.x >= j.nwg) return;
+    const SegRowsSum src[2] = {{j.a, j.a2}, {j.b, nullptr}};
+    SegAddEpi<2, SegRowsSum> epi{j.dst, src};
+    segment_walk<2>(src, epi, j.order, j.seg_ptr, j.target, j.U, CH, j.nwg);
+}
+
+struct SegPrepEpi {
+    const float4* out;
+    const float* norm;
+    DropCfg drop;
+    float4* gn;
+    float4* g_loop;
+    float mx;
+    __device__ __forceinline__ void operator()(int v, int ch, int CH, const float4 (&s)[1]) {
+        const size_t i = (size_t)v * CH + ch;
+        float4 g = make_float4(0.f + s[0].x, 0.f + s[0].y, 0.f + s[0].z, 0.f + s[0].w);
+        if (out) {
+            const float4 o = nt_load4(out + i);
+            g.x = o.x > 0.f ? g.x : 0.f; g.y = o.y > 0.f ? g.y : 0.f;
+            g.z = o.z > 0.f ? g.z : 0.f; g.w = o.w > 0.f ? g.w : 0.f;
+        }
+        gn[i] = f4_scale(g, norm[v]);
+        const float4 gl = f4_mul(g, renet_drop4(drop, i));
+        nt_store4(g_loop + i, gl);
+        mx = fmaxf(fmaxf(mx, fmaxf(fabsf(gl.x), fabsf(gl.y))), fmaxf(fabsf(gl.z), fabsf(gl.w)));
+    }
+};
+__global__ __launch_bounds__(kSegWaves * 64) void seq_bwd_rows_segment_prep_kernel(
+    SegRowsSeqBwd rows, const int32_t* __restrict__ order, const int32_t* __restrict__ seg_ptr,
+    const int32_t* __restrict__ seg_target, int U, int CH, const float4* out, const float* __restrict__ norm, DropCfg drop,
+    float4* __restrict__ gn, float4* __restrict__ g_loop, float* __restrict__ bound_part) {
+    __shared__ float redm[kSegWaves];
+    const SegRowsSeqBwd src[1] = {rows};
+    SegPrepEpi epi{out, norm, drop, gn, g_loop, 0.f};
+    segment_walk<1>(src, epi, order, seg_ptr, seg_target, U, CH, (int)gridDim.x);
+    if (bound_part) {
+        float mx = epi.mx;
+#pragma unroll
+        for (int off = 32; off >= 1; off >>= 1) mx = fmaxf(mx, __shfl_xor(mx, off));
+        if ((threadIdx.x & 63) == 0) redm[threadIdx.x >> 6] = mx;
         __syncthreads();
-        if (wave == 0) {
-            for (int ch = lane; ch < CH; ch += 64) {
-                float4 r = red[0][ch];
-#pragma unroll
-                for (int w = 1; w < kSegWaves; ++w) r = f4_add(r, red[w][ch]);
-                dst[tgt + ch] = f4_add(dst[tgt + ch], r);
-            }
-        }
-        __syncthreads();
+        if (threadIdx.x == 0) {
+            float m = redm[0];
+#pragma unroll
+            for (int w = 1; w < kSegWaves; ++w) m = fmaxf(m, redm[w]);
+            bound_part[blockIdx.x] = m;
+        }
+    }
+}
+__global__ __launch_bounds__(256) void rgcn_bwd_prep_zero_rows_kernel(const float* __restrict__ norm, DropCfg drop, int N, int CH,
+                                                                      float4* __restrict__ gn, float4* __restrict__ g_loop) {
+    const size_t total = (size_t)N * CH;
+    const float4 z = make_float4(0.f, 0.f, 0.f, 0.f);
+    for (size_t i = (size_t)blockIdx.x * blockDim.x + threadIdx.x; i < total; i += (size_t)gridDim.x * blockDim.x) {
+        gn[i] = f4_scale(z, norm[i / CH]);
+        g_loop[i] = f4_mul(z, renet_drop4(drop, i));
     }
 }
 
@@ -915,6 +1068,60 @@
     RENET_LAUNCH(segment_add_kernel, dim3(seg_grid(U), 2), dim3(kSegWaves * 64), 0,
                        (hipStream_t)stream, (const float4*)src0, (const float4*)src1, order, seg_ptr, seg_target, U, D / 4,
                        (float4*)dst0, (float4*)dst1);
+    RENET_LAUNCH_CHECK();
+    return RENET_OK;
+}
+
+int renet_segment_add_multi(const float* a0, const float* a0_plus, const float* b0, const int32_t* order0,
+                            const int32_t* seg_ptr0, const int32_t* target0, int U0, float* dst0, const float* a1,
+                            const float* a1_plus, const float* b1, const int32_t* order1, const int32_t* seg_ptr1,
+                            const int32_t* target1, int U1, float* dst1, int D, void* stream) {
+    if (U0 < 0 || U1 < 0 || D <= 0 || (D & 3)) return RENET_ERR_BADARG;
+    if ((U0 > 0 && (!a0 || !dst0)) || (U1 > 0 && (!a1 || !dst1))) return RENET_ERR_BADARG;
+    if (U0 == 0 && U1 == 0) return RENET_OK;
+    if (D > 512) return RENET_ERR_UNSUPPORTED;
+    const SegJob j0{(const float4*)a0, (const float4*)a0_plus, (const float4*)b0, order0, seg_ptr0, target0, (float4*)dst0, U0,
+                    U0 > 0 ? seg_grid(U0) : 0};
+    const SegJob j1{(const float4*)a1, (const float4*)a1_plus, (const float4*)b1, order1, seg_ptr1, target1, (float4*)dst1, U1,
+                    U1 > 0 ? seg_grid(U1) : 0};
+    RENET_LAUNCH(segment_add_multi_kernel, dim3(max(j0.nwg, j1.nwg), 2), dim3(kSegWaves * 64), 0, (hipStream_t)stream, j0, j1,
+                 D / 4);
+    RENET_LAUNCH_CHECK();
+    return RENET_OK;
+}
+
+int renet_seq_bwd_rows_segment_prep_parts(int U) { return U > 0 ? seg_grid(U) : 1; }
+
+int renet_seq_bwd_rows_segment_prep(const float* dX, const float* dXr, int S, float seq_drop_p, uint64_t seed_x,
+                                    uint64_t seed_xr, const int32_t* order, const int32_t* seg_ptr, const int32_t* seg_target,
+                                    int U, const float* out, const float* norm, int relu, float drop_p, uint64_t seed, int nA,
+                                    int D, float* gn, float* g_loop, float* bound_part, void* stream) {
+    if (S < 0 || U < 0 || nA < 0 || D <= 0 || (D & 3) || drop_p < 0.f || drop_p >= 1.f || seq_drop_p < 0.f ||
+        seq_drop_p >= 1.f || U > nA || (relu && !out))
+        return RENET_ERR_BADARG;
+    if (nA == 0) return bound_part ? RENET_ERR_BADARG : RENET_OK;
+    if (D > 512) return RENET_ERR_UNSUPPORTED;
+    if (bound_part && U > 0 && seg_grid(U) > 1024) return RENET_ERR_UNSUPPORTED;
+    hipStream_t st = (hipStream_t)stream;
+    const int CH = D / 4;
+    const DropCfg drop = make_drop(drop_p, seed);
+    if (U != nA) {
+        const size_t total = (size_t)nA * CH;
+        RENET_LAUNCH(rgcn_bwd_prep_zero_rows_kernel, dim3((int)min((size_t)2048, (total + 255) / 256)), dim3(256), 0, st, norm,
+                     drop, nA, CH, (float4*)gn, (float4*)g_loop);
+        RENET_LAUNCH_CHECK();
+    }
+    if (U == 0) {
+        if (bound_part) {
+            const hipError_t e = hipMemsetAsync(bound_part, 0, sizeof(float), st);
+            if (e != hipSuccess) return (int)e;
+        }
+        return RENET_OK;
+    }
+    const SegRowsSeqBwd rows{(const float4*)dX, (const float4*)dXr, make_drop(seq_drop_p, seed_x), make_drop(seq_drop_p, seed_xr)};
+    RENET_LAUNCH(seq_bwd_rows_segment_prep_kernel, dim3(seg_grid(U)), dim3(kSegWaves * 64), 0, st, rows, order, seg_ptr,
+                 seg_target, U, CH, relu ? (const float4*)out : (const float4*)nullptr, norm, drop, (float4*)gn,
+                 (float4*)g_loop, bound_part);
     RENET_LAUNCH_CHECK();
     return RENET_OK;
 }
diff --git a/re-net_amd/csrc/seq.hip b/re-net_amd/csrc/seq.hip
--- a/re-net_amd/csrc/seq.hip
+++ b/re-net_amd/csrc/seq.hip
@@ -126,6 +126,55 @@
     }
 }
 
+__device__ __forceinline__ float4 sq_fma4(float4 a, float4 b, float4 c) {
+    return make_float4(__builtin_fmaf(a.x, b.x, c.x), __builtin_fmaf(a.y, b.y, c.y), __builtin_fmaf(a.z, b.z, c.z),
+                       __builtin_fmaf(a.w, b.w, c.w));
+}
+__device__ __forceinline__ float4 sq_sel4(bool on, float4 a, float4 b) {
+    return make_float4(on ? a.x : b.x, on ? a.y : b.y, on ? a.z : b.z, on ? a.w : b.w);
+}
+template <int LU>
+__global__ __launch_bounds__(256) void seq_assemble_bwd_seq_unr_kernel(const float4* __restrict__ dX,
+                                                                       const float4* __restrict__ dXr,
+                                                                       const int32_t* __restrict__ off, int L, int S,
+                                                                       int B, int CH, DropCfg dx, DropCfg dxr,
+                                                                       float4* __restrict__ dEntSeq,
+                                                                       float4* __restrict__ dRelSeq) {
+    const size_t total = (size_t)B * CH;
+    for (size_t t = (size_t)blockIdx.x * blockDim.x + threadIdx.x; t < total;
+         t += (size_t)gridDim.x * blockDim.x) {
+        const int i = (int)(t / CH), cc = (int)(t - (size_t)i * CH);
+        float4 ve[LU], vr[LU], vl[LU];
+        int pj[LU];
+        bool on[LU];
+        bool alive = true;
+#pragma unroll
+        for (int j = 0; j < LU; ++j) {
+            const int jj = min(j, L - 1);
+            const int o0 = off[jj], o1 = off[jj + 1];
+            alive = alive && j < L && i < o1 - o0;
+            on[j] = alive;
+            pj[j] = max(0, min(min(o0 + i, o1 - 1), S - 1));
+            const size_t bx = (size_t)pj[j] * 4 * CH + CH + cc, br = (size_t)pj[j] * 3 * CH + CH + cc;
+            ve[j] = dX[bx];
+            vr[j] = dXr[br];
+            vl[j] = dX[bx + CH];
+        }
+        __builtin_amdgcn_sched_barrier(0);
+        float4 se = make_float4(0.f, 0.f, 0.f, 0.f), sr = se;
+#pragma unroll
+        for (int j = 0; j < LU; ++j) {
+            const size_t bx = (size_t)pj[j] * 4 * CH + CH + cc, br = (size_t)pj[j] * 3 * CH + CH + cc;
+            float4 e = sq_fma4(ve[j], renet_drop4(dx, bx), se);
+            e = sq_fma4(vr[j], renet_drop4(dxr, br), e);
+            se = sq_sel4(on[j], e, se);
+            sr = sq_sel4(on[j], sq_fma4(vl[j], renet_drop4(dx, bx + CH), sr), sr);
+        }
+        dEntSeq[t] = se;
+        dRelSeq[t] = sr;
+    }
+}
+
 __global__ __launch_bounds__(256) void concat3_fwd_kernel(const float4* __restrict__ a,
                                                           const int32_t* __restrict__ ia,
                                                           const float4* __restrict__ hmid,
@@ -759,16 +808,22 @@
     if (S < 0 || B < 0 || L < 0 || D <= 0 || (D & 3) || drop_p < 0.f || drop_p >= 1.f) return RENET_ERR_BADARG;
     const int CH = D / 4;
     const DropCfg dx = make_drop(drop_p, seed_x), dxr = make_drop(drop_p, seed_xr);
-    if (S > 0) {
+    if (S > 0 && dRows) {
         RENET_LAUNCH(seq_assemble_bwd_rows_kernel, dim3(grid_for((size_t)S * CH)), dim3(256), 0,
                            (hipStream_t)stream, (const float4*)dX, (const float4*)dXr, S, CH, dx, dxr,
                            (float4*)dRows);
         RENET_LAUNCH_CHECK();
     }
     if (B > 0) {
-        RENET_LAUNCH(seq_assemble_bwd_seq_kernel, dim3(grid_for((size_t)B * CH)), dim3(256), 0,
-                           (hipStream_t)stream, (const float4*)dX, (const float4*)dXr, step_off, L, B, CH, dx,
-                           dxr, (float4*)dEntSeq, (float4*)dRelSeq);
+        const dim3 grid(grid_for((size_t)B * CH)), blk(256);
+        hipStream_t st = (hipStream_t)stream;
+        const float4 *x4 = (const float4*)dX, *xr4 = (const float4*)dXr;
+        float4 *de = (float4*)dEntSeq, *dr = (float4*)dRelSeq;
+        if (L < 1 || L > 16 || S < 1) RENET_LAUNCH(seq_assemble_bwd_seq_kernel, grid, blk, 0, st, x4, xr4, step_off, L, B, CH, dx, dxr, de, dr);
+        else if (L <= 4) RENET_LAUNCH((seq_assemble_bwd_seq_unr_kernel<4>), grid, blk, 0, st, x4, xr4, step_off, L, S, B, CH, dx, dxr, de, dr);
+        else if (L <= 8) RENET_LAUNCH((seq_assemble_bwd_seq_unr_kernel<8>), grid, blk, 0, st, x4, xr4, step_off, L, S, B, CH, dx, dxr, de, dr);
+        else if (L <= 12) RENET_LAUNCH((seq_assemble_bwd_seq_unr_kernel<12>), grid, blk, 0, st, x4, xr4, step_off, L, S, B, CH, dx, dxr, de, dr);
+        else RENET_LAUNCH((seq_assemble_bwd_seq_unr_kernel<16>), grid, blk, 0, st, x4, xr4, step_off, L, S, B, CH, dx, dxr, de, dr);
         RENET_LAUNCH_CHECK();
     }
     return RENET_OK;
diff --git a/re-net_amd/csrc/step.cpp b/re-net_amd/csrc/step.cpp
--- a/re-net_amd/csrc/step.cpp
+++ b/re-net_amd/csrc/step.cpp
@@ -45,7 +45,7 @@
 struct Lay {
     size_t out1, out2, X, Xr, sv0, sv1, feat1, feat2, dl1, dl2, featp1;
     size_t ew, gi0, gi1, hs0, hs1, logits, featp;
-    size_t dfeat1, dfeat2, da1, da2, dh1, dh2, dc1, dgi0, dgi1, dgh0, dgh1, dX, dXr, d_rows, d_ent_seq, d_rel_seq, d_h2, gn2,
+    size_t dfeat1, dfeat2, da1, da2, dh1, dh2, dc1, dgi0, dgi1, dgh0, dgh1, dX, dXr, d_ent_seq, d_rel_seq, gn2,
         gl2, dhN, gn1, gl1, dh1N, gs;
     size_t gru_ws, gemm_ws_main, gemm_ws_side, bwdw_ws, colsum_ws;
     size_t gru_ws_bytes, gemm_ws_bytes, bwdw_ws_bytes, colsum_ws_bytes;
@@ -104,10 +104,8 @@
     L.dgh1 = take(fbytes(S, 3 * D));
     L.dX = take(fbytes(S, 4 * D));
     L.dXr = take(fbytes(S, 3 * D));
-    L.d_rows = take(fbytes(S, D));
     L.d_ent_seq = take(fbytes(B, D));
     L.d_rel_seq = take(fbytes(B, D));
-    L.d_h2 = take(fbytes(nA, D));
     L.gn2 = take(fbytes(nA, D));
     L.gl2 = take(fbytes(nA, D));
     L.dhN = take(fbytes(N, D));
@@ -319,9 +317,6 @@
         const hipError_t e = hipEventRecord((hipEvent_t)ev_head_done, s.main);
         if (e != hipSuccess) return (int)e;
     }
-    CK(renet_add_inplace(F(L.da1), F(L.da2), (size_t)B * D, s.main));
-    CK(renet_segment_add(F(L.da1), b.plan_s.order, b.plan_s.seg_ptr, b.plan_s.target, b.plan_s.num_segments, D, m.g_ent, s.main));
-    CK(renet_segment_add(F(L.dc1), b.plan_r.order, b.plan_r.seg_ptr, b.plan_r.target, b.plan_r.num_segments, D, m.g_rel, s.main));
 
     {
         const float* dhl[2] = {F(L.dh1), F(L.dh2)};
@@ -362,16 +357,16 @@
     CK(gemm(s.main, wsm, L.gemm_ws_bytes, 0, 0, S, 3 * D, 3 * D, F(L.dgi0), 3 * D, m.wih, 4 * D, 0.f, F(L.dX), 4 * D, nullptr));
     CK(gemm(s.main, wsm, L.gemm_ws_bytes, 0, 0, S, 2 * D, 3 * D, F(L.dgi1), 3 * D, m.wih_r, 3 * D, 0.f, F(L.dXr), 3 * D, nullptr));
 
-    CK(renet_seq_assemble_bwd(F(L.dX), F(L.dXr), b.step_off, b.L, S, B, D, p, r->seed_x, r->seed_xr, F(L.d_rows), F(L.d_ent_seq),
+    CK(renet_seq_bwd_rows_segment_prep(F(L.dX), F(L.dXr), S, p, r->seed_x, r->seed_xr, b.plan_subj_row.order,
+                                       b.plan_subj_row.seg_ptr, b.plan_subj_row.target, b.plan_subj_row.num_segments, nullptr,
+                                       b.norm, 0, p, r->seed_rgcn2, nA, D, F(L.gn2), F(L.gl2), nullptr, s.main));
+    CK(renet_seq_assemble_bwd(F(L.dX), F(L.dXr), b.step_off, b.L, S, B, D, p, r->seed_x, r->seed_xr, nullptr, F(L.d_ent_seq),
                               F(L.d_rel_seq), s.main));
-    CK(renet_zero(F(L.d_h2), (size_t)nA * D, s.main));
-    CK(renet_segment_add(F(L.d_rows), b.plan_subj_row.order, b.plan_subj_row.seg_ptr, b.plan_subj_row.target,
-                         b.plan_subj_row.num_segments, D, F(L.d_h2), s.main));
-    CK(renet_segment_add(F(L.d_ent_seq), b.plan_s.order, b.plan_s.seg_ptr, b.plan_s.target, b.plan_s.num_segments, D, m.g_ent, s.main));
-    CK(renet_segment_add(F(L.d_rel_seq), b.plan_r.order, b.plan_r.seg_ptr, b.plan_r.target, b.plan_r.num_segments, D, m.g_rel, s.main));
+    CK(renet_segment_add_multi(F(L.da1), F(L.da2), F(L.d_ent_seq), b.plan_s.order, b.plan_s.seg_ptr, b.plan_s.target,
+                               b.plan_s.num_segments, m.g_ent, F(L.dc1), nullptr, F(L.d_rel_seq), b.plan_r.order,
+                               b.plan_r.seg_ptr, b.plan_r.target, b.plan_r.num_segments, m.g_rel, D, s.main));
 
     const int pair_shift = (T / 2) % T;
-    CK(renet_rgcn_bwd_prep(F(L.d_h2), F(L.out2), b.norm, 0, p, r->seed_rgcn2, nA, D, F(L.gn2), F(L.gl2), s.main));
     CK(renet_rgcn_gather_items(F(L.gn2), D, b.it_src, b.it_type, b.grp_ptr, b.n_groups, b.row_ptr, b.col, b.etype, nullptr, m.w2, T,
                                pair_shift, 1, nullptr, 0.f, 0, 0, F(L.dhN), N, b.n_heavy ? b.heavy_rows : nullptr, b.n_heavy,
                                pruned ? nA : 0, 0, pruned ? 1 : 0, s.main));
diff --git a/re-net_amd/ops.py b/re-net_amd/ops.py
--- a/re-net_amd/ops.py
+++ b/re-net_amd/ops.py
@@ -196,6 +196,18 @@
     d = torch.zeros(shape, device=src.device, dtype=torch.float32)
     K.segment_add(src, plan, d)
     return d
+
+
+def _segment_grad_pair(job_a, job_c, a_shape, c_shape):
+    (ra, pa, plan_a, t_a), (rc, pc, plan_c, t_c) = job_a, job_c
+    if t_a is not None and t_c is not None and ra.is_cuda:
+        K.segment_add_multi((ra, pa, None, plan_a, t_a), (rc, pc, None, plan_c, t_c))
+        return None, None
+    if pa is not None:
+        ra.add_(pa)
+    if pc is not None:
+        rc.add_(pc)
+    return _segment_grad(ra, plan_a, t_a, a_shape), _segment_grad(rc, plan_c, t_c, c_shape)
 
 
 class GatherRowsFn(Function):
@@ -365,8 +377,8 @@
         d_rows, d_ent_seq, d_rel_seq = K.seq_assemble_bwd(_c(dx), _c(dxr), g.step_off, g.L, g.B, d, ctx.drop_p,
                                                           *ctx.seeds)
         d_h2 = _segment_grad(d_rows, g.plan_subj_row, None, ctx.shapes[0])
-        d_ent = _segment_grad(d_ent_seq, g.plan_s, tgt_ent, ctx.shapes[1])
-        d_rel = _segment_grad(d_rel_seq, g.plan_r, tgt_rel, ctx.shapes[2])
+        d_ent, d_rel = _segment_grad_pair((d_ent_seq, None, g.plan_s, tgt_ent),
+                                          (d_rel_seq, None, g.plan_r, tgt_rel), ctx.shapes[1], ctx.shapes[2])
         return d_h2, d_ent, d_rel, None, None, None, None, None, None
 
 
@@ -707,8 +719,7 @@
         if t_w2 is not None and t_b2 is not None:
             grad_done(ctx.srcs[4])
             grad_done(ctx.srcs[5])
-        da1.add_(da2)
-        d_a, d_c = _scatter_head_rows(da1, dc1, plan_a, plan_c, t_a, t_c, a_shape, c_shape)
+        d_a, d_c = _segment_grad_pair((da1, da2, plan_a, t_a), (dc1, None, plan_c, t_c), a_shape, c_shape)
         return (d_a, None, dh1, d_c, None, d_w1, d_b1, None, dh2, d_w2, d_b2, None) + (None,) * 8
 
 
diff --git a/re-net_amd/renet_hip.py b/re-net_amd/renet_hip.py
--- a/re-net_amd/renet_hip.py
+++ b/re-net_amd/renet_hip.py
@@ -33,6 +33,13 @@
     'renet_segment_add': (c_int, [c_void_p, c_void_p, c_void_p, c_void_p, c_int, c_int, c_void_p, c_void_p]),
     'renet_segment_add2': (c_int, [c_void_p, c_void_p, c_void_p, c_void_p, c_void_p, c_int, c_int, c_void_p, c_void_p,
                                    c_void_p]),
+    'renet_segment_add_multi': (c_int, [c_void_p, c_void_p, c_void_p, c_void_p, c_void_p, c_void_p, c_int, c_void_p,
+                                        c_void_p, c_void_p, c_void_p, c_void_p, c_void_p, c_void_p, c_int, c_void_p,
+                                        c_int, c_void_p]),
+    'renet_seq_bwd_rows_segment_prep_parts': (c_int, [c_int]),
+    'renet_seq_bwd_rows_segment_prep': (c_int, [c_void_p, c_void_p, c_int, c_float, c_u64, c_u64, c_void_p, c_void_p,
+                                                c_void_p, c_int, c_void_p, c_void_p, c_int, c_float, c_u64, c_int, c_int,
+                                                c_void_p, c_void_p, c_void_p, c_void_p]),
     'renet_rgcn_gather': (c_int, [c_void_p, c_int, c_void_p, c_void_p, c_void_p, c_void_p, c_void_p, c_int,
                                   c_int, c_int, c_void_p, c_float, c_u64, c_int, c_void_p, c_int, c_void_p,
                                   c_int, c_int, c_int, c_int, c_void_p]),
@@ -285,7 +292,8 @@
     if t0 is not None:
         _timer.end(name, t0, flops=flops, nbytes=nbytes, tag=tag)
 
-GLUE = ('softmax_ce_planes', 'gather_rows', 'segment_add', 'segment_add2', 'compose_table_items', 'rgcn_bwd_prep', 'colsum',
+GLUE = ('softmax_ce_planes', 'gather_rows', 'segment_add', 'segment_add2', 'segment_add_multi',
+        'seq_bwd_rows_segment_prep', 'compose_table_items', 'rgcn_bwd_prep', 'colsum',
         'scale_by_device_scalar', 'seq_assemble_fwd', 'seq_assemble_fwd_bf16', 'softmax_ce_bf16', 'seq_assemble_bwd',
         'concat3_fwd', 'concat3_bwd', 'dropout', 'softmax_ce', 'adam_step', 'segment_pool_fwd', 'segment_pool_bwd',
         'pack_bf16_glue')
@@ -337,6 +345,31 @@
 def segment_add2(src0, src1, plan, dst0, dst1):
     _check(lib().renet_segment_add2(_f32(src0), _f32(src1), _i32(plan.order), _i32(plan.seg_ptr), _i32(plan.target),
                                     plan.num_segments, src0.shape[1], _f32(dst0), _f32(dst1), _stream()), 'segment_add2')
+
+
+def segment_add_multi(job0, job1):
+    args = []
+    for a, a_plus, b, plan, dst in (job0, job1):
+        args += [_f32(a), _f32(a_plus) if a_plus is not None else None, _f32(b) if b is not None else None,
+                 _i32(plan.order), _i32(plan.seg_ptr), _i32(plan.target), plan.num_segments, _f32(dst)]
+    _check(lib().renet_segment_add_multi(*args, job0[0].shape[1], _stream()), 'segment_add_multi')
+
+
+def seq_bwd_rows_segment_prep(dx, dxr, seq_drop_p, seed_x, seed_xr, plan, out, norm, relu, drop_p, seed, gn, g_loop,
+                              bounds=False):
+    n, d = gn.shape
+    part = None
+    if bounds:
+        nparts = lib().renet_seq_bwd_rows_segment_prep_parts(plan.num_segments)
+        part = torch.empty(nparts, device=gn.device, dtype=torch.float32)
+    _check(lib().renet_seq_bwd_rows_segment_prep(
+        _f32(dx), _f32(dxr), dx.shape[0], float(seq_drop_p), int(seed_x), int(seed_xr), _i32(plan.order),
+        _i32(plan.seg_ptr), _i32(plan.target), plan.num_segments, _f32(out) if out is not None else None, _f32(norm),
+        1 if relu else 0, float(drop_p), int(seed), n, d, _f32(gn), _f32(g_loop),
+        part.data_ptr() if part is not None else None, _stream()), 'seq_bwd_rows_segment_prep')
+    if part is not None:
+        _note_bound(g_loop, part, part.numel())
+    return part
 
 
 def rgcn_gather(x, row_ptr, col, etype, scale, weight, type_shift, transpose_w, addend, drop_p, seed,
```

After: 372,800 triples/s (median of 3 runs). About the same (+0.0%).
